# TAdeJong/pyGPA

Measured on AMD Instinct MI355X. Metric: Mpixels/s displacement-field extraction (3 peaks, 4096^2 img) + achieved HBM GB/s, higher is better.
Workload: dtype f32; 1 GPU; 4096x4096 synthetic hex moire, 3 Bragg peaks x 16 k-vectors, sigma=10, weighted DCT-PCG unwrap kmax=10, image resident in HBM, u downloaded to pinned host memory inside the step (BASELINE.json configs[2]); x_planes=12, d2h_of_u=included, overlapped with the next step (copy stream), images_in_flight=1

## Files before the change

### pygpa_amd/csrc/gpa_api.hip

```cpp
#include "gpa_plan.h"

static thread_local std::string g_err;
int gpa_fail(int code, const std::string& msg) {
  g_err = msg;
  return code;
}
namespace gpa {
static const char* const kOptNames[OPT_COUNT] = {
    "PBS_FULLBAND", "SERIAL_UNWRAP", "NO_WORKER", "NO_KSPLIT", "NO_COMPACT", "NO_SHARED",
    "NO_PAIR", "TRI_SMALL", "TRI_Q", "NO_MR", "MR_FORCE_BLUESTEIN", "NO_ROWPQ", "COLSOLVE", "NO_LAT",
    "F32_EPS_FLOOR", "COLSTREAM_CHUNK", "NO_ROWHALF", "PAIR_MAXSIDE", "ROWHALF_MINLG", "NO_PQDCT",
    "NO_REORDER", "NO_RAW", "NO_TILEFUSE", "NO_ROWPERS", "NO_LFTILE", "LF_ALL_ROUNDS", "DFT_ENGINE", "GAUSS_FFT_MINR", "NO_GAUSS2D", "NO_DFT_HALF", "F32_STALL", "PBS_LDS_PAD", "NO_SHARED_PHASES", "PA_STAG", "PA_STAG_TICKS", "PA_ROT", "LF_STACK_BYTES"};
static OptVal g_opts[OPT_COUNT];
static std::once_flag g_opts_once;
static void opt_assign(OptVal& o, const char* value) {
  o.set = value != nullptr;
  o.num = value ? atof(value) : 0.0;
  memset(o.str, 0, sizeof(o.str));
  if (value) strncpy(o.str, value, sizeof(o.str) - 1);
}
static void opts_from_env() {
  for (int k = 0; k < OPT_COUNT; ++k) opt_assign(g_opts[k], getenv((std::string("GPA_") + kOptNames[k]).c_str()));
}
const OptVal& opt(OptKey k) {
  std::call_once(g_opts_once, opts_from_env);
  return g_opts[k];
}
}

Axis make_axis(int n) {
  Axis a;
  a.n = n;
  int lg = 0;
  while ((1 << lg) < n) ++lg;
  if ((1 << lg) == n) {
    a.padded = false;
  } else {
    lg = 0;
    while ((1 << lg) < 2 * n - 1) ++lg;
    a.padded = true;
  }
  if (lg < 6) {
    lg = 6;
    a.padded = ((1 << lg) != n);
  }
  a.lg = lg;
  a.L = 1 << lg;
  a.extL = a.padded ? n - 1 : 0;
  a.extR = 0;
  return a;
}

Axis compact_axis(const Axis& full, int E) {
  if (!full.padded || E >= (full.n - 1) / 2) return full;
  int lg = 6;
  while ((1 << lg) < full.n + 2 * E) ++lg;
  if (lg >= full.lg) return full;
  Axis a = full;
  a.lg = lg;
  a.L = 1 << lg;
  a.extL = a.extR = E;
  return a;
}

int upload_real_table(gpa_plan* p, void* dst, const std::vector<double>& v) {
  if (p->dtype == GPA_F32) HIP_TRY(upload_as<float>(dst, v, p->stream));
  else HIP_TRY(upload_as<double>(dst, v, p->stream));
  return GPA_OK;
}

int dmalloc(gpa_plan* p, void** ptr, size_t bytes) {
  if (bytes == 0) bytes = 16;
  hipError_t e = hipMalloc(ptr, bytes);
  if (e != hipSuccess)
    return fail(GPA_ERR_HIP, std::string("hipMalloc(") + std::to_string(bytes) + "): " + hipGetErrorString(e));
  p->ws_bytes += bytes;
  return GPA_OK;
}
int plan_build(gpa_plan* p) {
  HIP_TRY(hipSetDevice(p->device));
  HIP_TRY(hipStreamCreateWithFlags(&p->stream, hipStreamNonBlocking));
  HIP_TRY(hipEventCreate(&p->ev0));
  HIP_TRY(hipEventCreate(&p->ev1));
  for (auto& e : p->stage_ev) HIP_TRY(hipEventCreate(&e));
  const size_t npx = (size_t)p->n0 * p->n1;
  const int B = p->max_batch;
  for (int ax = 0; ax < 2; ++ax) {
    const Axis& a = ax == 0 ? p->ax0 : p->ax1;
    std::vector<double> t((size_t)2 * a.L);
    for (int k = 0; k < a.L; ++k) {
      t[2 * k] = cos(-2.0 * M_PI * k / a.L);
      t[2 * k + 1] = sin(-2.0 * M_PI * k / a.L);
    }
    void** dst = ax == 0 ? &p->tw0 : &p->tw1;
    TRY(dmalloc(p, dst, (size_t)a.L * p->csz));
    TRY(upload_real_table(p, *dst, t));
  }
  TRY(dmalloc(p, &p->Hx, (size_t)p->ax0.L * p->csz));
  TRY(dmalloc(p, &p->Hy, (size_t)p->ax1.L * p->csz));
  p->tbuf_planes = B < 4 ? B : 4;
  TRY(dmalloc(p, &p->Tbuf, (size_t)p->tbuf_planes * npx * p->csz));
  TRY(dmalloc(p, &p->tb.cxb, (size_t)B * std::max(p->ax0.L / 16, 256) * p->csz));
  TRY(dmalloc(p, &p->tb.sx, (size_t)B * 16 * p->csz));
  TRY(dmalloc(p, &p->tb.wxw, (size_t)B * p->csz));
  TRY(dmalloc(p, &p->tb.wxr, (size_t)B * p->csz));
  TRY(dmalloc(p, &p->tb.cyb, (size_t)B * std::max(p->ax1.L / 16, 256) * p->csz));
  TRY(dmalloc(p, &p->tb.sy, (size_t)B * 16 * p->csz));
  TRY(dmalloc(p, &p->tb.wyw, (size_t)B * p->csz));
  TRY(dmalloc(p, &p->tb.wyr, (size_t)B * p->csz));
  TRY(dmalloc(p, (void**)&p->tb.planeof, (size_t)B * sizeof(int)));
  TRY(dmalloc(p, (void**)&p->d_pw, (size_t)B * sizeof(double)));
  TRY(dmalloc(p, &p->tb.dx, (size_t)B * p->n0 * p->csz));
  TRY(dmalloc(p, &p->tb.dy, (size_t)B * p->n1 * p->csz));
  TRY(dmalloc(p, (void**)&p->d_kl, (size_t)B * 2 * sizeof(double)));
  TRY(dmalloc(p, (void**)&p->d_kr, (size_t)B * 2 * sizeof(double)));
  HIP_TRY(hipHostMalloc((void**)&p->h_k, ((size_t)B * 6 + 32) * sizeof(double)));
  HIP_TRY(hipHostMalloc((void**)&p->h_iters, 8 * sizeof(int)));
  TRY(dmalloc(p, &p->d_image, npx * p->rsz));
  TRY(dmalloc(p, &p->d_mean, 16));
  TRY(dmalloc(p, &p->d_tile_mean, 16));
  TRY(dmalloc(p, (void**)&p->d_scratch, 16384 * sizeof(double)));
  TRY(dmalloc(p, &p->d_aux0, (size_t)p->n0 * 2 * sizeof(double)));
  TRY(dmalloc(p, &p->d_aux1, (size_t)p->n1 * 2 * sizeof(double)));
  p->max_peaks = B < 8 ? B : 8;
  TRY(dmalloc(p, &p->d_lockin, (size_t)p->max_peaks * npx * p->csz));
  TRY(dmalloc(p, (void**)&p->d_kidx, (size_t)p->max_peaks * npx * sizeof(int32_t)));
  TRY(dmalloc(p, &p->d_dudx, 2 * npx * p->rsz));
  TRY(dmalloc(p, &p->d_dudy, 2 * npx * p->rsz));
  TRY(dmalloc(p, &p->d_wnorm, npx * p->rsz));
  TRY(dmalloc(p, &p->d_u, 2 * npx * p->rsz));
  TRY(dmalloc(p, (void**)&p->d_kmat, (size_t)p->max_peaks * 2 * sizeof(double)));
  if (!p->spectral_only) {
    size_t before = 0;
    hipError_t e = unwrap_workspace_create(p->dtype, p->n0, p->n1, p->stream, &p->uw, &before);
    if (e != hipSuccess) return fail(GPA_ERR_HIP, std::string("unwrap workspace: ") + hipGetErrorString(e));
    p->ws_bytes += before;
  }
  return GPA_OK;
}


int upload_twiddles(gpa_plan* p, void* dst, int L) {
  std::vector<double> t((size_t)2 * L);
  for (int k = 0; k < L; ++k) {
    t[2 * k] = cos(-2.0 * M_PI * k / L);
    t[2 * k + 1] = sin(-2.0 * M_PI * k / L);
  }
  return upload_real_table(p, dst, t);
}

extern "C" {

int gpa_version(void) { return 100; }

int gpa_set_option(const char* name, const char* value) {
  if (!name) return fail(GPA_ERR_ARG, "gpa_set_option: null name");
  if (strncmp(name, "GPA_", 4) == 0) name += 4;
  (void)opt(OPT_NO_LAT);
  for (int k = 0; k < OPT_COUNT; ++k)
    if (strcmp(name, kOptNames[k]) == 0) {
      opt_assign(g_opts[k], value);
      return GPA_OK;
    }
  return fail(GPA_ERR_ARG, std::string("gpa_set_option: unknown option ") + name);
}
const char* gpa_last_error(void) { return g_err.c_str(); }

int gpa_device_count(void) {
  int n = 0;
  if (hipGetDeviceCount(&n) != hipSuccess) return 0;
  return n;
}

gpa_plan* gpa_plan_create(int device, int n0, int n1, int max_batch, int dtype) {
  if (n0 < 4 || n1 < 4 || max_batch < 1 || (dtype != GPA_F32 && dtype != GPA_F64)) {
    fail(GPA_ERR_ARG, "gpa_plan_create: need n0,n1 >= 4, max_batch >= 1, dtype in {GPA_F32, GPA_F64}");
    return nullptr;
  }
  int ndev = gpa_device_count();
  if (ndev <= 0 || device < 0 || device >= ndev) {
    fail(GPA_ERR_NODEV, "gpa_plan_create: no such GPU (device " + std::to_string(device) + " of " +
                            std::to_string(ndev) + ")");
    return nullptr;
  }
  gpa_plan* p = new gpa_plan();
  p->device = device;
  p->dtype = dtype;
  p->n0 = n0;
  p->n1 = n1;
  p->max_batch = max_batch;
  p->rsz = dtype == GPA_F32 ? 4 : 8;
  p->csz = 2 * p->rsz;
  p->ax0 = p->ax0_full = make_axis(n0);
  p->ax1 = p->ax1_full = make_axis(n1);
  p->serial_unwrap = opt_set(OPT_SERIAL_UNWRAP);
  p->use_worker = !opt_set(OPT_NO_WORKER);
  p->no_ksplit = opt_set(OPT_NO_KSPLIT);
  p->no_compact = opt_set(OPT_NO_COMPACT);
  p->use_shared = !opt_set(OPT_NO_SHARED);
  const int maxlg = dtype == GPA_F32 ? 14 : 13;
  if (n0 > 65536 || n1 > 65536) {
    fail(GPA_ERR_ARG, "gpa_plan_create: axis longer than 65536");
    delete p;
    return nullptr;
  }
  p->spectral_only = p->ax0.lg > maxlg || p->ax1.lg > maxlg;
  if (plan_build(p) != GPA_OK) {
    std::string keep = g_err;
    gpa_plan_destroy(p);
    g_err = keep;
    return nullptr;
  }
  return p;
}

void gpa_plan_destroy(gpa_plan* p) {
  if (!p) return;
  hipSetDevice(p->device);
  delete p->worker;
  p->worker = nullptr;
  if (p->stream) hipStreamSynchronize(p->stream);
  void* bufs[] = {p->tw0, p->tw1, p->Hx, p->Hy, p->Tbuf, p->tb.cxb, p->tb.sx, p->tb.wxw, p->tb.wxr, p->tb.cyb, p->tb.sy, p->tb.wyw, p->tb.wyr, p->tb.planeof, p->d_pw,
                  p->tb.dx, p->tb.dy, p->d_kl, p->d_kr, p->d_image, p->d_mean, p->d_tile_mean, p->d_scratch,
                  p->d_lockin, p->d_kidx, p->d_dudx, p->d_dudy, p->d_wnorm, p->d_u, p->d_kmat, p->d_sf, p->d_grad, p->d_grads, p->d_absw, p->d_aux0, p->d_aux1,
                  p->sh.Gb, p->sh.psi, p->sh.dyc, p->sh.gtab, p->sh.desc, p->sh.order, p->d_taps, p->tw1s,
                  p->sh.pre, p->sh.rot16, p->d_wys, p->d_shifts, p->d_ystep};
  for (void* b : bufs)
    if (b) hipFree(b);
  unwrap_workspace_destroy(&p->uw);
  unwrap_workspace_destroy(&p->uw2);
  if (p->uwb_images) unwrap_workspace_destroy(&p->uwb);
  if (p->have_uwp) unwrap_workspace_destroy(&p->uwp);
  if (p->d_wnorm_b) (void)hipFree(p->d_wnorm_b);
  if (p->h_iters_b) (void)hipHostFree(p->h_iters_b);
  for (void* b : {p->bT, p->bL, p->bMean, (void*)p->bScratch})
    if (b) (void)hipFree(b);
  if (p->stream2) { hipStreamSynchronize(p->stream2); hipStreamDestroy(p->stream2); }
  if (p->ev_fork) hipEventDestroy(p->ev_fork);
  if (p->ev_join) hipEventDestroy(p->ev_join);
  if (p->ev_x) hipEventDestroy(p->ev_x);
  if (p->d_tsum_part) (void)hipFree(p->d_tsum_part);
  warp_ws_free(&p->warp);
  ucell_ws_free(&p->ucell);
  dft_axis_destroy(&p->bx0);
  dft_axis_destroy(&p->bx1);
  dft_work_free(&p->dftw);
  for (auto& ax : p->gft)
    for (auto& g : ax) {
      if (g.H) (void)hipFree(g.H);
      if (g.tw) (void)hipFree(g.tw);
    }
  if (p->d_pertab) (void)hipFree(p->d_pertab);
  if (p->d_peakws) (void)hipFree(p->d_peakws);
  if (p->d_peaksmooth) (void)hipFree(p->d_peaksmooth);
  if (p->h_k) hipHostFree(p->h_k);
  if (p->h_iters) hipHostFree(p->h_iters);
  if (p->kprof) {
    for (int i = 0; i < p->kprof->npool; ++i) hipEventDestroy(p->kprof->pool[i]);
    delete p->kprof;
  }
  if (p->copy_stream) { hipStreamSynchronize(p->copy_stream); hipStreamDestroy(p->copy_stream); }
  if (p->ev_dl_ready) hipEventDestroy(p->ev_dl_ready);
  for (auto e : p->ev_dl_done)
    if (e) hipEventDestroy(e);
  if (p->ev0) hipEventDestroy(p->ev0);
  if (p->ev1) hipEventDestroy(p->ev1);
  for (auto e : p->stage_ev)
    if (e) hipEventDestroy(e);
  if (p->stream) hipStreamDestroy(p->stream);
  delete p;
}

int gpa_plan_sync(gpa_plan* p) {
  if (!p) return fail(GPA_ERR_ARG, "null plan");
  HIP_TRY(hipStreamSynchronize(p->stream));
  if (p->stream2) HIP_TRY(hipStreamSynchronize(p->stream2));
  if (p->copy_stream) HIP_TRY(hipStreamSynchronize(p->copy_stream));
  return GPA_OK;
}
size_t gpa_plan_workspace_bytes(const gpa_plan* p) { return p ? p->ws_bytes : 0; }
void* gpa_plan_stream(const gpa_plan* p) { return p ? (void*)p->stream : nullptr; }
int gpa_plan_fft_len(const gpa_plan* p, int axis) {
  if (!p) return 0;
  return axis == 0 ? p->ax0.L : p->ax1.L;
}

int gpa_timer_start(gpa_plan* p) {
  if (!p) return fail(GPA_ERR_ARG, "null plan");
  HIP_TRY(hipEventRecord(p->ev0, p->stream));
  return GPA_OK;
}
int gpa_timer_stop(gpa_plan* p, float* ms_out) {
  if (!p || !ms_out) return fail(GPA_ERR_ARG, "null argument");
  HIP_TRY(hipEventRecord(p->ev1, p->stream));
  HIP_TRY(hipEventSynchronize(p->ev1));
  HIP_TRY(hipEventElapsedTime(ms_out, p->ev0, p->ev1));
  return GPA_OK;
}
int gpa_set_profiling(gpa_plan* p, int on) {
  if (!p) return fail(GPA_ERR_ARG, "null plan");
  p->profiling = on != 0;
  return GPA_OK;
}
int gpa_last_kernel_profile(gpa_plan* p, char* out, size_t cap) {
  if (!p || !out || cap == 0) return fail(GPA_ERR_ARG, "null argument");
  if (p->kprof_table.size() + 1 > cap) return fail(GPA_ERR_STATE, "gpa_last_kernel_profile: buffer too small");
  memcpy(out, p->kprof_table.c_str(), p->kprof_table.size() + 1);
  return GPA_OK;
}

int gpa_download_async(gpa_plan* p, void* host_dst, const void* dev_src, size_t bytes, int slot) {
  if (!p || !host_dst || !dev_src) return fail(GPA_ERR_ARG, "gpa_download_async: null argument");
  if (slot < 0 || slot >= 4) return fail(GPA_ERR_ARG, "gpa_download_async: slot must be 0..3");
  HIP_TRY(hipSetDevice(p->device));
  if (!p->copy_stream) {
    HIP_TRY(hipStreamCreateWithFlags(&p->copy_stream, hipStreamNonBlocking));
    HIP_TRY(hipEventCreateWithFlags(&p->ev_dl_ready, hipEventDisableTiming));
    for (auto& e : p->ev_dl_done) HIP_TRY(hipEventCreateWithFlags(&e, hipEventDisableTiming));
  }
  HIP_TRY(hipEventRecord(p->ev_dl_ready, p->stream));
  HIP_TRY(hipStreamWaitEvent(p->copy_stream, p->ev_dl_ready, 0));
  HIP_TRY(hipMemcpyAsync(host_dst, dev_src, bytes, hipMemcpyDeviceToHost, p->copy_stream));
  HIP_TRY(hipEventRecord(p->ev_dl_done[slot], p->copy_stream));
  return GPA_OK;
}

int gpa_download_wait(gpa_plan* p, int slot) {
  if (!p) return fail(GPA_ERR_ARG, "null plan");
  if (slot < 0 || slot >= 4) return fail(GPA_ERR_ARG, "gpa_download_wait: slot must be 0..3");
  if (!p->copy_stream) return GPA_OK;
  HIP_TRY(hipEventSynchronize(p->ev_dl_done[slot]));
  return GPA_OK;
}

int gpa_last_stage_ms(gpa_plan* p, float* ms5) {
  if (!p || !ms5) return fail(GPA_ERR_ARG, "null argument");
  for (int i = 0; i < 5; ++i) ms5[i] = p->stage_ms[i];
  return GPA_OK;
}

}
```

### pygpa_amd/csrc/gpa_api_driver.hip

```cpp
#include "gpa_plan.h"

struct ExtractOut {
  void* lockins;
  int32_t* kidx;
  void* grads;
  void* absw;
  int grad_mode;
};

static int check_ranges(gpa_plan* p, const std::string& fn, int P, int K, int kmax) {
  if (P < 2 || P > p->max_peaks) return fail(GPA_ERR_STATE, fn + ": need 2 <= P <= 8");
  if (K < 1 || P * K > p->max_batch) return fail(GPA_ERR_STATE, fn + ": P*K exceeds max_batch");
  if (kmax < 1) return fail(GPA_ERR_ARG, "kmax must be >= 1");
  return GPA_OK;
}

static int extract_stage(gpa_plan* p, const double* kvecs, int P, const double* klists, int K, double sigma, int* Bx) {
  TRY(stage_sweep(p, kvecs, P, klists, K, sigma, Bx));
  TRY(stage_kmat(p, kvecs, P));
  {
    const size_t side = opt_set(OPT_PAIR_MAXSIDE) ? (size_t)opt(OPT_PAIR_MAXSIDE).num : 1024;
    p->use_pair = (size_t)p->n0 * p->n1 <= side * side && !opt_set(OPT_NO_PAIR);
  }
  if (p->use_pair && !p->have_uwp) {
    size_t bp = 0;
    hipError_t ep = unwrap_workspace_create(p->dtype, p->n0, p->n1, p->stream, &p->uwp, &bp, 2);
    if (ep != hipSuccess) {
      unwrap_workspace_destroy(&p->uwp);
      return fail(GPA_ERR_HIP, std::string("paired unwrap workspace: ") + hipGetErrorString(ep));
    }
    p->ws_bytes += bp;
    p->have_uwp = true;
  }
  if (p->use_pair && !unwrap_supports_batch(&p->uwp)) p->use_pair = false;
  if (!p->stream2) {
    HIP_TRY(hipStreamCreateWithFlags(&p->stream2, hipStreamNonBlocking));
    HIP_TRY(hipEventCreateWithFlags(&p->ev_fork, hipEventDisableTiming));
    HIP_TRY(hipEventCreateWithFlags(&p->ev_join, hipEventDisableTiming));
    size_t b2 = 0;
    hipError_t e2 = unwrap_workspace_create(p->dtype, p->n0, p->n1, p->stream2, &p->uw2, &b2);
    if (e2 != hipSuccess) return fail(GPA_ERR_HIP, std::string("second unwrap workspace: ") + hipGetErrorString(e2));
    p->ws_bytes += b2;
  }
  return GPA_OK;
}

static int extract_launch(gpa_plan* p, const void* image, int P, int K, int Bx, int mask_border, int kmax, void* u,
                          const ExtractOut& o) {
  const size_t npx = (size_t)p->n0 * p->n1;
  void* lk = o.lockins ? o.lockins : p->d_lockin;
  if (p->profiling) HIP_TRY(hipEventRecord(p->stage_ev[0], p->stream));
  HIP_TRY(launch_mean(p->dtype, image, npx, p->d_scratch, p->d_mean, p->stream));
  if (p->profiling) HIP_TRY(hipEventRecord(p->stage_ev[1], p->stream));
  TRY(run_passA(p, image, p->d_mean, p->Tbuf, Bx, 1));
  if (p->profiling) HIP_TRY(hipEventRecord(p->stage_ev[2], p->stream));
  if (o.grads) {
    int32_t* kidx = o.kidx ? o.kidx : p->d_kidx;
    bool shared = false;
    TRY(passB_phases(p, P, K, lk, kidx, p->d_sf, &shared));
    HIP_TRY(launch_phasegrad(p->dtype, p->d_sf, K, kidx, p->n0, p->n1, p->d_kl, p->d_kr, o.grad_mode, o.grads, p->stream,
                             shared ? p->d_ystep : nullptr, P));
  } else {
    TRY(passB_select(p, {p->Tbuf, 1, 0}, P, K, lk, o.kidx, !o.lockins && !o.absw));
  }
  if (o.absw) HIP_TRY(launch_cabs(p->dtype, lk, (size_t)P * npx, o.absw, p->stream));
  const double* ystep = p->lk_raw ? p->d_ystep : nullptr;
  if (p->profiling) HIP_TRY(hipEventRecord(p->stage_ev[3], p->stream));
  int nparts = 0;
  if (p->use_pair && p->have_uwp && !p->profiling && !p->serial_unwrap) {
    HIP_TRY(launch_reconstruct_setup(p->dtype, lk, p->d_kmat, P, p->n0, p->n1, mask_border, p->d_wnorm,
                                     unwrap_residual_buffer(&p->uwp, 0), unwrap_residual_buffer(&p->uwp, 1),
                                     unwrap_partials_buffer(&p->uwp, 0), unwrap_partials_buffer(&p->uwp, 1), &nparts,
                                     p->stream, 1, 0, 0, ystep));
    hipError_t ep = unwrap_enqueue_prepared(&p->uwp, p->d_wnorm, nparts, kmax, 1e-9, true, u, p->stream);
    if (ep == hipSuccess) ep = unwrap_fetch_iters(&p->uwp, p->h_iters, p->stream);
    if (ep != hipSuccess) return unwrap_fail(ep);
    p->iters_stride = 4;
    p->iters_off = unwrap_iters_slot(&p->uwp);
    return GPA_OK;
  }
  p->iters_stride = 1;
  p->iters_off = 0;
  HIP_TRY(launch_reconstruct_setup(p->dtype, lk, p->d_kmat, P, p->n0, p->n1, mask_border, p->d_wnorm,
                                   unwrap_residual_buffer(&p->uw), unwrap_residual_buffer(&p->uw2),
                                   unwrap_partials_buffer(&p->uw), unwrap_partials_buffer(&p->uw2), &nparts, p->stream, 1, 0,
                                   0, ystep));
  if (p->profiling) HIP_TRY(hipEventRecord(p->stage_ev[4], p->stream));
  HIP_TRY(hipEventRecord(p->ev_fork, p->stream));
  HIP_TRY(hipStreamWaitEvent(p->stream2, p->ev_fork, 0));
  hipStreamCaptureStatus cap = hipStreamCaptureStatusNone;
  (void)hipStreamIsCapturing(p->stream, &cap);
  const bool threaded = p->use_worker && !p->profiling && !p->serial_unwrap && cap == hipStreamCaptureStatusNone;
  hipError_t e2 = hipSuccess;
  void* u1 = (char*)u + npx * p->rsz;
  auto second = [&]() {
    e2 = unwrap_enqueue_prepared(&p->uw2, p->d_wnorm, nparts, kmax, 1e-9, true, u1, p->stream2);
    if (e2 == hipSuccess) e2 = unwrap_fetch_iters(&p->uw2, &p->h_iters[1], p->stream2);
  };
  if (threaded) {
    if (!p->worker) p->worker = new EnqueueWorker(p->device);
    p->worker->submit(second);
  }
  hipError_t e = unwrap_enqueue_prepared(&p->uw, p->d_wnorm, nparts, kmax, 1e-9, true, u, p->stream);
  if (p->profiling || p->serial_unwrap) {
    HIP_TRY(hipEventRecord(p->ev_fork, p->stream));
    HIP_TRY(hipStreamWaitEvent(p->stream2, p->ev_fork, 0));
  }
  if (e == hipSuccess) e = unwrap_fetch_iters(&p->uw, &p->h_iters[0], p->stream);
  if (threaded) p->worker->wait(); else second();
  if (e == hipSuccess) e = e2;
  if (e != hipSuccess) return unwrap_fail(e);
  HIP_TRY(hipEventRecord(p->ev_join, p->stream2));
  HIP_TRY(hipStreamWaitEvent(p->stream, p->ev_join, 0));
  if (p->profiling) HIP_TRY(hipEventRecord(p->stage_ev[5], p->stream));
  return GPA_OK;
}

static int extract_enqueue(gpa_plan* p, const char* what, const void* image, const double* kvecs, int P, const double* klists,
                           int K, double sigma, int mask_border, int kmax, void* u, const ExtractOut& o) {
  const std::string fn(what);
  if (!p || !image || !kvecs || !klists || !u) return fail(GPA_ERR_ARG, fn + ": null argument");
  TRY(check_ranges(p, fn, P, K, kmax));
  if (o.grads && (o.grad_mode < 0 || o.grad_mode > 2)) return fail(GPA_ERR_ARG, fn + ": grad_mode must be 0, 1 or 2");
  HIP_TRY(hipSetDevice(p->device));
  int Bx = 0;
  TRY(extract_stage(p, kvecs, P, klists, K, sigma, &Bx));
  if (o.grads) TRY(ensure_sf(p, (size_t)P * K * p->n0 * p->n1 * p->rsz));
  ProfInstall prof(p);
  return extract_launch(p, image, P, K, Bx, mask_border, kmax, u, o);
}

static void read_iters(const gpa_plan* p, int* iters2) {
  iters2[0] = p->h_iters[p->iters_off];
  iters2[1] = p->h_iters[p->iters_stride + p->iters_off];
}

int gpa_last_iters(gpa_plan* p, int* iters2) {
  if (!p || !iters2) return fail(GPA_ERR_ARG, "null argument");
  HIP_TRY(hipStreamSynchronize(p->stream));
  read_iters(p, iters2);
  return GPA_OK;
}

static int extract_finish(gpa_plan* p, int* iters_out) {
  HIP_TRY(hipStreamSynchronize(p->stream));
  if (p->profiling) {
    for (int i = 0; i < 5; ++i) hipEventElapsedTime(&p->stage_ms[i], p->stage_ev[i], p->stage_ev[i + 1]);
    collect_kernel_profile(p);
  }
  if (iters_out) read_iters(p, iters_out);
  return GPA_OK;
}

static int extract_host(gpa_plan* p, const char* what, const void* image, const double* kvecs, int P, const double* klists,
                        int K, double sigma, int mask_border, int kmax, void* u, const ExtractOut& o, int* iters_out) {
  if (!p || !image || !u) return fail(GPA_ERR_ARG, std::string(what) + ": null argument");
  HIP_TRY(hipSetDevice(p->device));
  const size_t npx = (size_t)p->n0 * p->n1;
  if (o.grads && !p->d_grads) TRY(dmalloc(p, &p->d_grads, (size_t)p->max_peaks * 2 * npx * p->rsz));
  if (o.absw && !p->d_absw) TRY(dmalloc(p, &p->d_absw, (size_t)p->max_peaks * npx * p->rsz));
  HIP_TRY(hipMemcpyAsync(p->d_image, image, npx * p->rsz, hipMemcpyHostToDevice, p->stream));
  const ExtractOut dev{o.lockins ? p->d_lockin : nullptr, o.kidx ? p->d_kidx : nullptr, o.grads ? p->d_grads : nullptr,
                       o.absw ? p->d_absw : nullptr, o.grad_mode};
  TRY(extract_enqueue(p, what, p->d_image, kvecs, P, klists, K, sigma, mask_border, kmax, p->d_u, dev));
  TRY(extract_finish(p, iters_out));
  HIP_TRY(hipMemcpyAsync(u, p->d_u, 2 * npx * p->rsz, hipMemcpyDeviceToHost, p->stream));
  if (o.lockins) HIP_TRY(hipMemcpyAsync(o.lockins, p->d_lockin, (size_t)P * npx * p->csz, hipMemcpyDeviceToHost, p->stream));
  if (o.kidx) HIP_TRY(hipMemcpyAsync(o.kidx, p->d_kidx, (size_t)P * npx * sizeof(int32_t), hipMemcpyDeviceToHost, p->stream));
  if (o.grads) HIP_TRY(hipMemcpyAsync(o.grads, p->d_grads, (size_t)P * 2 * npx * p->rsz, hipMemcpyDeviceToHost, p->stream));
  if (o.absw) HIP_TRY(hipMemcpyAsync(o.absw, p->d_absw, (size_t)P * npx * p->rsz, hipMemcpyDeviceToHost, p->stream));
  HIP_TRY(hipStreamSynchronize(p->stream));
  return GPA_OK;
}

int gpa_extract_displacement_field(gpa_plan* p, const void* image, const double* kvecs, int P,
                                   const double* klists, int K, double sigma, int mask_border, int kmax,
                                   void* u, void* lockins, int32_t* kidx, int* iters_out) {
  return extract_host(p, "gpa_extract_displacement_field", image, kvecs, P, klists, K, sigma, mask_border, kmax, u,
                      {lockins, kidx, nullptr, nullptr, 0}, iters_out);
}

int gpa_extract_displacement_field_grad(gpa_plan* p, const void* image, const double* kvecs, int P,
                                        const double* klists, int K, double sigma, int mask_border, int kmax,
                                        int grad_mode, void* u, void* lockins, int32_t* kidx, void* grads, void* absw,
                                        int* iters_out) {
  return extract_host(p, "gpa_extract_displacement_field_grad", image, kvecs, P, klists, K, sigma, mask_border, kmax, u,
                      {lockins, kidx, grads, absw, grad_mode}, iters_out);
}

int gpa_extract_displacement_field_dev(gpa_plan* p, const void* image, const double* kvecs, int P,
                                       const double* klists, int K, double sigma, int mask_border, int kmax,
                                       void* u, void* lockins, int32_t* kidx, int* iters_out) {
  TRY(extract_enqueue(p, "gpa_extract_displacement_field", image, kvecs, P, klists, K, sigma, mask_border, kmax, u,
                      {lockins, kidx, nullptr, nullptr, 0}));
  return extract_finish(p, iters_out);
}

int gpa_extract_displacement_field_grad_dev(gpa_plan* p, const void* image, const double* kvecs, int P,
                                            const double* klists, int K, double sigma, int mask_border, int kmax,
                                            int grad_mode, void* u, void* lockins, int32_t* kidx, void* grads, void* absw,
                                            int* iters_out) {
  TRY(extract_enqueue(p, "gpa_extract_displacement_field_grad_dev", image, kvecs, P, klists, K, sigma, mask_border, kmax, u,
                      {lockins, kidx, grads, absw, grad_mode}));
  return extract_finish(p, iters_out);
}

int gpa_extract_displacement_field_async(gpa_plan* p, const void* image, const double* kvecs, int P,
                                         const double* klists, int K, double sigma, int mask_border, int kmax,
                                         void* u, void* lockins, int32_t* kidx) {
  return extract_enqueue(p, "gpa_extract_displacement_field", image, kvecs, P, klists, K, sigma, mask_border, kmax, u,
                         {lockins, kidx, nullptr, nullptr, 0});
}

int gpa_extract_displacement_field_grad_async(gpa_plan* p, const void* image, const double* kvecs, int P,
                                              const double* klists, int K, double sigma, int mask_border, int kmax,
                                              int grad_mode, void* u, void* lockins, int32_t* kidx, void* grads, void* absw) {
  return extract_enqueue(p, "gpa_extract_displacement_field_grad_async", image, kvecs, P, klists, K, sigma, mask_border, kmax, u,
                         {lockins, kidx, grads, absw, grad_mode});
}

static int ensure_batch_unwrap(gpa_plan* p, int B) {
  if (B <= p->uwb_images) {
    if (!unwrap_set_active(&p->uwb, 2 * B)) return fail(GPA_ERR_STATE, "batched unwrap workspace: bad active count");
    return GPA_OK;
  }
  const size_t npx = (size_t)p->n0 * p->n1;
  HIP_TRY(hipStreamSynchronize(p->stream));
  if (p->uwb_images) {
    unwrap_workspace_destroy(&p->uwb);
    (void)hipFree(p->d_wnorm_b);
    (void)hipHostFree(p->h_iters_b);
    p->uwb_images = 0;
    p->d_wnorm_b = nullptr;
    p->h_iters_b = nullptr;
  }
  size_t bb = 0;
  hipError_t e = unwrap_workspace_create(p->dtype, p->n0, p->n1, p->stream, &p->uwb, &bb, 2 * B);
  if (e != hipSuccess) {
    unwrap_workspace_destroy(&p->uwb);
    return fail(GPA_ERR_HIP, std::string("batched unwrap workspace: ") + hipGetErrorString(e));
  }
  if (!unwrap_supports_batch(&p->uwb)) {
    unwrap_workspace_destroy(&p->uwb);
    return fail(GPA_ERR_STATE, "gpa_extract_displacement_field_batch: this image shape has no batched unwrap");
  }
  e = hipMalloc(&p->d_wnorm_b, (size_t)B * npx * p->rsz);
  if (e == hipSuccess) e = hipHostMalloc((void**)&p->h_iters_b, (size_t)8 * B * sizeof(int));
  if (e != hipSuccess) {
    unwrap_workspace_destroy(&p->uwb);
    if (p->d_wnorm_b) (void)hipFree(p->d_wnorm_b);
    p->d_wnorm_b = nullptr;
    return fail(GPA_ERR_HIP, std::string("batched driver buffers: ") + hipGetErrorString(e));
  }
  p->uwb_images = B;
  return GPA_OK;
}

static int ensure_batch_sweep(gpa_plan* p, int chunk, size_t t_img, size_t l_img) {
  if ((size_t)chunk * t_img <= p->bT_bytes && (size_t)chunk * l_img <= p->bL_bytes && chunk <= p->b_chunk) return GPA_OK;
  HIP_TRY(hipStreamSynchronize(p->stream));
  for (void* b : {p->bT, p->bL, p->bMean, (void*)p->bScratch})
    if (b) (void)hipFree(b);
  p->bT = p->bL = p->bMean = nullptr;
  p->bScratch = nullptr;
  p->bT_bytes = p->bL_bytes = 0;
  p->b_chunk = 0;
  hipError_t ea = hipMalloc(&p->bT, (size_t)chunk * t_img);
  if (ea == hipSuccess) ea = hipMalloc(&p->bL, (size_t)chunk * l_img);
  if (ea == hipSuccess) ea = hipMalloc(&p->bMean, (size_t)chunk * 8);
  if (ea == hipSuccess) ea = hipMalloc((void**)&p->bScratch, (size_t)chunk * 1024 * sizeof(double));
  if (ea != hipSuccess) return fail(GPA_ERR_HIP, std::string("batched sweep buffers: ") + hipGetErrorString(ea));
  p->bT_bytes = (size_t)chunk * t_img;
  p->bL_bytes = (size_t)chunk * l_img;
  p->b_chunk = chunk;
  return GPA_OK;
}

static int read_batch_iters(gpa_plan* p, int B, int* iters_out) {
  HIP_TRY(hipStreamSynchronize(p->stream));
  for (int j = 0; j < 2 * B; ++j) iters_out[j] = p->h_iters_b[4 * j + unwrap_iters_slot(&p->uwb)];
  return GPA_OK;
}

int gpa_extract_displacement_field_batch_dev(gpa_plan* p, const void* images, int B, const double* kvecs, int P,
                                             const double* klists, int K, double sigma, int mask_border, int kmax,
                                             void* u, int* iters_out) {
  const char* fn = "gpa_extract_displacement_field_batch";
  if (!p || !images || !kvecs || !klists || !u) return fail(GPA_ERR_ARG, std::string(fn) + ": null argument");
  if (B < 1 || B > 4096) return fail(GPA_ERR_ARG, std::string(fn) + ": need 1 <= images <= 4096");
  TRY(check_ranges(p, fn, P, K, kmax));
  HIP_TRY(hipSetDevice(p->device));
  int Bx = 0;
  TRY(extract_stage(p, kvecs, P, klists, K, sigma, &Bx));
  TRY(ensure_batch_unwrap(p, B));
  const size_t npx = (size_t)p->n0 * p->n1;
  const size_t t_img = (size_t)Bx * npx * p->csz, l_img = (size_t)P * npx * p->csz;
  const int chunk = (int)std::min<size_t>((size_t)B, std::max<size_t>(1, ((size_t)3 << 30) / t_img));
  TRY(ensure_batch_sweep(p, chunk, t_img, l_img));
  int nparts = 0;
  const size_t rstride = 2 * npx;
  const size_t pstride = (size_t)(unwrap_partials_buffer(&p->uwb, 2) - unwrap_partials_buffer(&p->uwb, 0));
  for (int c0 = 0; c0 < B; c0 += chunk) {
    const int nimg = std::min(chunk, B - c0);
    const void* image = (const char*)images + (size_t)c0 * npx * p->rsz;
    HIP_TRY(launch_mean(p->dtype, image, npx, p->bScratch, p->bMean, p->stream, nimg));
    TRY(run_passA(p, image, p->bMean, p->bT, Bx, nimg));
    TRY(passB_select(p, {p->bT, nimg, Bx}, P, K, p->bL, nullptr, true));
    HIP_TRY(launch_reconstruct_setup(p->dtype, p->bL, p->d_kmat, P, p->n0, p->n1, mask_border,
                                     (char*)p->d_wnorm_b + (size_t)c0 * npx * p->rsz,
                                     unwrap_residual_buffer(&p->uwb, 2 * c0), unwrap_residual_buffer(&p->uwb, 2 * c0 + 1),
                                     unwrap_partials_buffer(&p->uwb, 2 * c0), unwrap_partials_buffer(&p->uwb, 2 * c0 + 1),
                                     &nparts, p->stream, nimg, rstride, pstride, p->lk_raw ? p->d_ystep : nullptr));
  }
  hipError_t e = unwrap_enqueue_prepared(&p->uwb, p->d_wnorm_b, nparts, kmax, 1e-9, true, u, p->stream);
  if (e == hipSuccess) e = unwrap_fetch_iters(&p->uwb, p->h_iters_b, p->stream);
  if (e != hipSuccess) return fail(GPA_ERR_HIP, std::string("batched unwrap: ") + hipGetErrorString(e));
  return iters_out ? read_batch_iters(p, B, iters_out) : GPA_OK;
}

int gpa_supports_batch(gpa_plan* p) {
  if (!p) return 0;
  return unwrap_supports_batch(&p->uw) ? 1 : 0;
}

int gpa_last_batch_iters(gpa_plan* p, int B, int* iters_out) {
  if (!p || !iters_out || B < 1 || B > p->uwb_images) return fail(GPA_ERR_ARG, "gpa_last_batch_iters: bad argument");
  return read_batch_iters(p, B, iters_out);
}

int gpa_extract_gradients(gpa_plan* p, const void* image, const double* kvecs, int P, const double* klists, int K,
                          double sigma, int mask_border, void* dudx, void* dudy, void* wnorm) {
  if (!p || !image || !kvecs || !klists || !dudx || !dudy || !wnorm)
    return fail(GPA_ERR_ARG, "gpa_extract_gradients: null argument");
  TRY(check_ranges(p, "gpa_extract_gradients", P, K, 1));
  HIP_TRY(hipSetDevice(p->device));
  const size_t npx = (size_t)p->n0 * p->n1;
  HIP_TRY(hipMemcpyAsync(p->d_image, image, npx * p->rsz, hipMemcpyHostToDevice, p->stream));
  TRY(sweep_peaks_dev(p, p->d_image, nullptr, kvecs, P, klists, K, sigma, p->d_lockin, nullptr, true));
  TRY(stage_kmat(p, kvecs, P));
  HIP_TRY(launch_reconstruct(p->dtype, p->d_lockin, p->d_kmat, P, p->n0, p->n1, mask_border, p->d_dudx, p->d_dudy,
                             p->d_wnorm, p->stream, p->lk_raw ? p->d_ystep : nullptr));
  HIP_TRY(hipMemcpyAsync(dudx, p->d_dudx, (size_t)2 * p->n0 * (p->n1 - 1) * p->rsz, hipMemcpyDeviceToHost, p->stream));
  HIP_TRY(hipMemcpyAsync(dudy, p->d_dudy, (size_t)2 * (p->n0 - 1) * p->n1 * p->rsz, hipMemcpyDeviceToHost, p->stream));
  HIP_TRY(hipMemcpyAsync(wnorm, p->d_wnorm, npx * p->rsz, hipMemcpyDeviceToHost, p->stream));
  HIP_TRY(hipStreamSynchronize(p->stream));
  return GPA_OK;
}
```

### pygpa_amd/csrc/gpa_api_sweep.hip

```cpp
#include "gpa_plan.h"

int gpa_lockin_batch_dev(gpa_plan* p, const void* image, const double* kvecs, int B, double sigma,
                         void* out) {
  if (!p || !image || !kvecs || !out) return fail(GPA_ERR_ARG, "gpa_lockin_batch: null argument");
  if (B < 1 || B > p->max_batch) return fail(GPA_ERR_STATE, "gpa_lockin_batch: B exceeds the plan's max_batch");
  HIP_TRY(hipSetDevice(p->device));
  TRY(ensure_filters(p, sigma));
  int Bx = 0;
  TRY(stage_kvectors(p, kvecs, kvecs, B, &Bx));
  TRY(ensure_tbuf(p, Bx));
  TRY(run_passA(p, image, nullptr, p->Tbuf, Bx, 1));
  HIP_TRY(launch_passB(p->dtype, p->ax1, p->n0, p->Tbuf, p->Hy, p->tw1, p->tb, B, 1, false, out, nullptr,
                       p->stream));
  return GPA_OK;
}

int gpa_lockin_batch(gpa_plan* p, const void* image, const double* kvecs, int B, double sigma, void* out) {
  if (!p || !image || !kvecs || !out) return fail(GPA_ERR_ARG, "gpa_lockin_batch: null argument");
  if (B < 1 || B > p->max_batch) return fail(GPA_ERR_STATE, "gpa_lockin_batch: B exceeds the plan's max_batch");
  HIP_TRY(hipSetDevice(p->device));
  const size_t npx = (size_t)p->n0 * p->n1;
  HIP_TRY(hipMemcpyAsync(p->d_image, image, npx * p->rsz, hipMemcpyHostToDevice, p->stream));
  TRY(ensure_sf(p, (size_t)B * npx * p->csz));
  TRY(gpa_lockin_batch_dev(p, p->d_image, kvecs, B, sigma, p->d_sf));
  HIP_TRY(hipMemcpyAsync(out, p->d_sf, (size_t)B * npx * p->csz, hipMemcpyDeviceToHost, p->stream));
  HIP_TRY(hipStreamSynchronize(p->stream));
  return GPA_OK;
}

int stage_sweep(gpa_plan* p, const double* krefs, int P, const double* klists, int K, double sigma, int* Bx) {
  const int B = P * K;
  TRY(ensure_filters(p, sigma));
  std::vector<double> kr((size_t)B * 2);
  for (int pp = 0; pp < P; ++pp)
    for (int k = 0; k < K; ++k) {
      kr[2 * ((size_t)pp * K + k)] = krefs[2 * pp];
      kr[2 * ((size_t)pp * K + k) + 1] = krefs[2 * pp + 1];
    }
  TRY(stage_kvectors(p, klists, kr.data(), B, Bx));
  return ensure_tbuf(p, *Bx);
}

int run_passA(gpa_plan* p, const void* image, const void* mean, void* Tbuf, int Bx, int nimg) {
  HIP_TRY(launch_passA(p->dtype, p->ax0, p->n1, image, mean, p->tb, p->Hx, p->tw0, Tbuf, Bx, p->stream, nimg));
  return GPA_OK;
}

int passB_select(gpa_plan* p, const XPlanes& xp, int P, int K, void* lockin, int32_t* kidx, bool raw) {
  p->lk_raw = false;
  const int rows_wg = (p->n0 + 7) / 8 * P;
  int ksplit = 1;
  if (xp.stride == 0 && p->ax1.lg <= 10 && K >= 4 && !p->no_ksplit && rows_wg <= 256)
    while (ksplit < 4 && ksplit * 2 <= K && rows_wg * ksplit < 1024) ksplit *= 2;
  if (ksplit == 1) {
    TRY(shared_prepare(p, P, K));
    if (p->sh_use) {
      p->lk_raw = raw && !opt_set(OPT_NO_RAW) && p->sh_one_kref;
      HIP_TRY(launch_passB_shared(p->dtype, p->ax1s, p->n0, xp.T, p->ax1s.L == p->ax1.L ? p->tw1 : p->tw1s, p->tb,
                                  p->sh, p->sh_E, p->sh_Epad, P, K, lockin, kidx, p->stream, xp.nimg, xp.stride, p->sh_nbl,
                                  p->lk_raw));
    } else
      HIP_TRY(launch_passB(p->dtype, p->ax1, p->n0, xp.T, p->Hy, p->tw1, p->tb, P, K, true, lockin, kidx, p->stream, xp.nimg,
                           xp.stride));
    return GPA_OK;
  }
  const size_t npx = (size_t)p->n0 * p->n1, cnt = (size_t)ksplit * P * npx;
  TRY(ensure_sf(p, cnt * (p->csz + sizeof(int32_t))));
  void* part = p->d_sf;
  int32_t* pidx = reinterpret_cast<int32_t*>((char*)p->d_sf + cnt * p->csz);
  HIP_TRY(launch_passB_split(p->dtype, p->ax1, p->n0, xp.T, p->Hy, p->tw1, p->tb, P, K, ksplit, part, pidx, lockin, kidx,
                             p->stream));
  return GPA_OK;
}

int passB_phases(gpa_plan* p, int P, int K, void* lockin, int32_t* kidx, void* psi, bool* shared) {
  p->lk_raw = false;
  *shared = false;
  if (p->use_shared && !opt_set(OPT_NO_SHARED_PHASES)) {
    TRY(shared_prepare(p, P, K));
    if (p->sh_use && p->sh_one_kref) {
      const hipError_t e = launch_passB_shared_phases(p->dtype, p->ax1s, p->n0, p->Tbuf, p->ax1s.L == p->ax1.L ? p->tw1 : p->tw1s,
                                                      p->tb, p->sh, p->sh_E, p->sh_Epad, P, K, lockin, kidx, psi, p->stream, 0,
                                                      p->sh_nbl);
      if (e == hipSuccess) {
        *shared = true;
        return GPA_OK;
      }
      if (e != hipErrorInvalidValue) return fail(GPA_ERR_HIP, std::string("shared pass B (phases): ") + hipGetErrorString(e));
    }
  }
  HIP_TRY(launch_passB_ext(p->dtype, p->ax1, p->n0, p->Tbuf, p->Hy, p->tw1, p->tb, K, 3, lockin, kidx, nullptr, psi, p->stream, P));
  return GPA_OK;
}

void collect_kernel_profile(gpa_plan* p) {
  std::vector<std::string> names;
  std::vector<int> calls;
  std::vector<double> total;
  for (int i = 0; p->kprof && i < p->kprof->n; ++i) {
    const KernelProfiler::Rec& r = p->kprof->rec[i];
    float ms = 0.f;
    if (hipEventElapsedTime(&ms, r.a, r.b) != hipSuccess) continue;
    size_t j = 0;
    while (j < names.size() && names[j] != r.name) ++j;
    if (j == names.size()) { names.push_back(r.name); calls.push_back(0); total.push_back(0.0); }
    ++calls[j];
    total[j] += ms;
  }
  p->kprof_table.clear();
  char line[160];
  for (size_t j = 0; j < names.size(); ++j) {
    snprintf(line, sizeof(line), "%s %d %.6f\n", names[j].c_str(), calls[j], total[j]);
    p->kprof_table += line;
  }
}

int sweep_peaks_dev(gpa_plan* p, const void* image, const void* mean, const double* krefs, int P,
                           const double* klists, int K, double sigma, void* lockin, int32_t* kidx, bool raw) {
  if (P * K > p->max_batch) return fail(GPA_ERR_STATE, "sweep: P*K exceeds the plan's max_batch");
  int Bx = 0;
  TRY(stage_sweep(p, krefs, P, klists, K, sigma, &Bx));
  if (p->profiling) HIP_TRY(hipEventRecord(p->stage_ev[1], p->stream));
  TRY(run_passA(p, image, mean, p->Tbuf, Bx, 1));
  if (p->profiling) HIP_TRY(hipEventRecord(p->stage_ev[2], p->stream));
  TRY(passB_select(p, {p->Tbuf, 1, 0}, P, K, lockin, kidx, raw));
  if (p->profiling) HIP_TRY(hipEventRecord(p->stage_ev[3], p->stream));
  return GPA_OK;
}

static int sweep_one_peak(gpa_plan* p, const void* image, const double* kref, const double* klist, int K, double sigma,
                          int mode, void* lockin, int32_t* kidx, const uint8_t* d_gate, void* d_psi) {
  if (K > p->max_batch) return fail(GPA_ERR_STATE, "gpa_sweep: K exceeds the plan's max_batch");
  int Bx = 0;
  TRY(stage_sweep(p, kref, 1, klist, K, sigma, &Bx));
  TRY(run_passA(p, image, nullptr, p->Tbuf, Bx, 1));
  HIP_TRY(launch_passB_ext(p->dtype, p->ax1, p->n0, p->Tbuf, p->Hy, p->tw1, p->tb, K, mode, lockin, kidx, d_gate, d_psi,
                           p->stream));
  return GPA_OK;
}

int gpa_sweep_grad_dev(gpa_plan* p, const void* image, const double* kref, const double* klist, int K, double sigma,
                       int grad_mode, void* lockin, int32_t* kidx, void* grad) {
  if (!p || !image || !kref || !klist || !lockin || !grad) return fail(GPA_ERR_ARG, "gpa_sweep_grad: null argument");
  if (K < 1) return fail(GPA_ERR_ARG, "gpa_sweep_grad: K must be >= 1");
  if (grad_mode < 0 || grad_mode > 2) return fail(GPA_ERR_ARG, "gpa_sweep_grad: grad_mode must be 0, 1 or 2");
  if (K > p->max_batch) return fail(GPA_ERR_STATE, "gpa_sweep: K exceeds the plan's max_batch");
  HIP_TRY(hipSetDevice(p->device));
  const bool top = g_kprof == nullptr;
  ProfInstallIf prof(p, top);
  const size_t npx = (size_t)p->n0 * p->n1;
  TRY(ensure_sf(p, (size_t)K * npx * p->rsz));
  int32_t* ki = kidx ? kidx : p->d_kidx;
  int Bx = 0;
  TRY(stage_sweep(p, kref, 1, klist, K, sigma, &Bx));
  TRY(run_passA(p, image, nullptr, p->Tbuf, Bx, 1));
  bool shared = false;
  TRY(passB_phases(p, 1, K, lockin, ki, p->d_sf, &shared));
  HIP_TRY(launch_phasegrad(p->dtype, p->d_sf, K, ki, p->n0, p->n1, p->d_kl, p->d_kr, grad_mode, grad, p->stream,
                           shared ? p->d_ystep : nullptr));
  if (top && p->profiling) { HIP_TRY(hipStreamSynchronize(p->stream)); collect_kernel_profile(p); }
  return GPA_OK;
}

int gpa_sweep_dev(gpa_plan* p, const void* image, const double* kref, const double* klist, int K,
                  double sigma, void* lockin, int32_t* kidx, void* grad) {
  if (!p || !image || !kref || !klist || !lockin) return fail(GPA_ERR_ARG, "gpa_sweep: null argument");
  if (K < 1) return fail(GPA_ERR_ARG, "gpa_sweep: K must be >= 1");
  HIP_TRY(hipSetDevice(p->device));
  if (!grad) return sweep_peaks_dev(p, image, nullptr, kref, 1, klist, K, sigma, lockin, kidx, false);
  return gpa_sweep_grad_dev(p, image, kref, klist, K, sigma, 0, lockin, kidx, grad);
}

static int sweep_host(gpa_plan* p, const void* image, const double* kref, const double* klist, int K, double sigma,
                      int grad_mode, const uint8_t* gate, void* lockin, int32_t* kidx, void* grad) {
  if (!p || !image || !kref || !klist || !lockin) return fail(GPA_ERR_ARG, "gpa_sweep: null argument");
  if (K < 1) return fail(GPA_ERR_ARG, "gpa_sweep: K must be >= 1");
  HIP_TRY(hipSetDevice(p->device));
  ProfInstall prof(p);
  const size_t npx = (size_t)p->n0 * p->n1;
  HIP_TRY(hipMemcpyAsync(p->d_image, image, npx * p->rsz, hipMemcpyHostToDevice, p->stream));
  if (grad && !p->d_grad) TRY(dmalloc(p, &p->d_grad, 2 * npx * p->rsz));
  if (gate) {
    TRY(ensure_sf(p, (size_t)K * K));
    HIP_TRY(hipMemcpyAsync(p->d_sf, gate, (size_t)K * K, hipMemcpyHostToDevice, p->stream));
    TRY(sweep_one_peak(p, p->d_image, kref, klist, K, sigma, 2, p->d_lockin, p->d_kidx, (const uint8_t*)p->d_sf, nullptr));
  } else if (grad) {
    TRY(gpa_sweep_grad_dev(p, p->d_image, kref, klist, K, sigma, grad_mode, p->d_lockin, p->d_kidx, p->d_grad));
  } else {
    TRY(sweep_peaks_dev(p, p->d_image, nullptr, kref, 1, klist, K, sigma, p->d_lockin, p->d_kidx, false));
  }
  if (grad) HIP_TRY(hipMemcpyAsync(grad, p->d_grad, 2 * npx * p->rsz, hipMemcpyDeviceToHost, p->stream));
  HIP_TRY(hipMemcpyAsync(lockin, p->d_lockin, npx * p->csz, hipMemcpyDeviceToHost, p->stream));
  if (kidx) HIP_TRY(hipMemcpyAsync(kidx, p->d_kidx, npx * sizeof(int32_t), hipMemcpyDeviceToHost, p->stream));
  HIP_TRY(hipStreamSynchronize(p->stream));
  if (p->profiling) collect_kernel_profile(p);
  return GPA_OK;
}

int gpa_sweep(gpa_plan* p, const void* image, const double* kref, const double* klist, int K, double sigma,
              void* lockin, int32_t* kidx, void* grad) {
  return sweep_host(p, image, kref, klist, K, sigma, 0, nullptr, lockin, kidx, grad);
}

int gpa_sweep_grad(gpa_plan* p, const void* image, const double* kref, const double* klist, int K, double sigma,
                   int grad_mode, void* lockin, int32_t* kidx, void* grad) {
  if (!grad) return fail(GPA_ERR_ARG, "gpa_sweep_grad: null argument");
  if (grad_mode < 0 || grad_mode > 2) return fail(GPA_ERR_ARG, "gpa_sweep_grad: grad_mode must be 0, 1 or 2");
  return sweep_host(p, image, kref, klist, K, sigma, grad_mode, nullptr, lockin, kidx, grad);
}

int gpa_sweep_gated(gpa_plan* p, const void* image, const double* kref, const double* klist, int K, double sigma,
                    const uint8_t* gate, void* lockin, int32_t* kidx) {
  if (!gate) return fail(GPA_ERR_ARG, "gpa_sweep_gated: null argument");
  return sweep_host(p, image, kref, klist, K, sigma, 0, gate, lockin, kidx, nullptr);
}
```

### pygpa_amd/csrc/gpa_api_tables.hip

```cpp
#include "gpa_plan.h"

void host_fft_pow2(std::vector<std::complex<double>>& a, bool inverse) {
  const size_t n = a.size();
  int lg = 0;
  while ((size_t(1) << lg) < n) ++lg;
  for (size_t i = 0; i < n; ++i) {
    size_t r = 0;
    for (int b = 0; b < lg; ++b) r |= ((i >> b) & 1) << (lg - 1 - b);
    if (r > i) std::swap(a[i], a[r]);
  }
  for (size_t len = 2; len <= n; len <<= 1) {
    const double ang = (inverse ? 2 : -2) * M_PI / (double)len;
    for (size_t s = 0; s < n; s += len)
      for (size_t j = 0; j < len / 2; ++j) {
        std::complex<double> w(cos(ang * (double)j), sin(ang * (double)j));
        auto u = a[s + j], v = a[s + j + len / 2] * w;
        a[s + j] = u + v;
        a[s + j + len / 2] = u - v;
      }
  }
}

std::vector<double> gaussian_kspace(int n, double sigma) {
  std::vector<double> g(n);
  for (int k = 0; k < n; ++k) {
    const int kk = k < (n + 1) / 2 ? k : k - n;
    const double f = (double)kk / (double)n;
    const double e = 2.0 * M_PI * M_PI * sigma * sigma * f * f;
    g[k] = e > 50.0 ? 0.0 : exp(-e);
  }
  return g;
}

std::vector<double> spatial_kernel(int n, const std::vector<double>& g) {
  std::vector<double> h((size_t)n);
  std::vector<long double> cs((size_t)n);
  const long double w = 2.0L * 3.14159265358979323846264338327950288L / (long double)n;
  for (int j = 0; j < n; ++j) cs[j] = cosl(w * (long double)j);
  for (int m = 0; m < n; ++m) {
    long double acc = 0;
    for (int k = 0; k < n; ++k)
      if (g[k] != 0.0) acc += (long double)g[k] * cs[(size_t)((long long)k * m % n)];
    h[m] = (double)(acc / (long double)n);
  }
  return h;
}

int kernel_support(const std::vector<double>& h, double tol) {
  const int n = (int)h.size();
  double total = 0;
  for (double v : h) total += fabs(v);
  double tail = 0;
  for (int m = n / 2; m >= 1; --m) {
    tail += fabs(h[m]) + (n - m != m ? fabs(h[n - m]) : 0.0);
    if (tail > tol * total) return m;
  }
  return 0;
}

std::vector<double> spatial_taps(int n, const std::vector<double>& g, int mmax) {
  std::vector<double> h((size_t)mmax + 1);
  std::vector<long double> cs((size_t)n);
  const long double w = 2.0L * 3.14159265358979323846264338327950288L / (long double)n;
  for (int j = 0; j < n; ++j) cs[j] = cosl(w * (long double)j);
  for (int m = 0; m <= mmax; ++m) {
    long double acc = 0;
    for (int k = 0; k < n; ++k)
      if (g[k] != 0.0) acc += (long double)g[k] * cs[(size_t)((long long)k * m % n)];
    h[m] = (double)(acc / (long double)n);
  }
  return h;
}

void build_filter_table(const Axis& ax, const std::vector<double>& g, const std::vector<double>& hsp,
                               std::vector<double>& out) {
  const int L = ax.L, tpf = L / 16;
  if (!ax.padded) {
    out.assign((size_t)L, 0.0);
    for (int i = 0; i < 16; ++i)
      for (int t = 0; t < tpf; ++t) out[(size_t)i * tpf + t] = g[spec_index_rt(ax.lg, t, i)] / (double)L;
    return;
  }
  const int n = ax.n;
  std::vector<std::complex<double>> h((size_t)L, 0.0);
  if (ax.extR == 0) {
    for (int m = 0; m < n; ++m) h[m] = hsp[m];
  } else {
    for (int m = 0; m <= ax.extL; ++m) h[m] = hsp[m];
    for (int m = 1; m <= ax.extR; ++m) h[(size_t)L - m] = hsp[n - m];
  }
  host_fft_pow2(h, false);
  out.assign((size_t)2 * L, 0.0);
  for (int i = 0; i < 16; ++i)
    for (int t = 0; t < tpf; ++t) {
      auto v = h[spec_index_rt(ax.lg, t, i)] / (double)L;
      out[2 * ((size_t)i * tpf + t)] = v.real();
      out[2 * ((size_t)i * tpf + t) + 1] = v.imag();
    }
}

int ensure_filters(gpa_plan* p, double sigma) {
  if (!(sigma > 0)) return fail(GPA_ERR_ARG, "sigma must be positive");
  NEED_UNWRAP(p, "lock-in sweep");
  if (sigma == p->sigma_cached) return GPA_OK;
  HIP_TRY(hipStreamSynchronize(p->stream));
  p->sigma_cached = -1.0;
  for (int axis = 0; axis < 2; ++axis) {
    const Axis& full = axis == 0 ? p->ax0_full : p->ax1_full;
    Axis& cur = axis == 0 ? p->ax0 : p->ax1;
    std::vector<double> g = gaussian_kspace(full.n, sigma), hsp, table;
    Axis want = full;
    if (full.padded) {
      hsp = spatial_kernel(full.n, g);
      if (!p->no_compact) want = compact_axis(full, kernel_support(hsp, p->dtype == 0 ? 1e-9 : 1e-14));
    }
    if (want.lg != cur.lg || want.extR != cur.extR || want.extL != cur.extL) {
      TRY(upload_twiddles(p, axis == 0 ? p->tw0 : p->tw1, want.L));
      p->staged_kl.clear();
      p->staged_kr.clear();
      cur = want;
    }
    build_filter_table(cur, g, hsp, table);
    TRY(upload_real_table(p, axis == 0 ? p->Hx : p->Hy, table));
    if (axis == 1) {
      p->sh_ok = false;
      ++p->sh_epoch;
      const int n = cur.n;
      int mmax = (int)ceil(10.0 * sigma) + 16;
      if (p->use_shared && mmax < n / 2 && mmax <= 1024) {
        std::vector<double> taps = spatial_taps(n, g, mmax);
        double total = fabs(taps[0]), tail = 0;
        for (int m = 1; m <= mmax; ++m) total += 2 * fabs(taps[m]);
        int E = 1;
        const double tol = p->dtype == 0 ? 1e-9 : 1e-14;
        for (int m = mmax; m >= 1; --m) {
          tail += 2 * fabs(taps[m]);
          if (tail > tol * total) { E = m; break; }
        }
        Axis sa = cur;
        if (cur.padded) {
          sa.lg = 6;
          while ((1 << sa.lg) < n + E) ++sa.lg;
          sa.L = 1 << sa.lg;
          sa.extL = sa.extR = 0;
        }
        if (passB_shared_supports(p->dtype, sa, E)) {
          const int Epad = (E + 15) & ~15;
          if (sa.L != cur.L && p->tw1s_L != sa.L) {
            if (!p->tw1s) TRY(dmalloc(p, &p->tw1s, (size_t)8192 * p->csz));
            TRY(upload_twiddles(p, p->tw1s, sa.L));
            p->tw1s_L = sa.L;
          }
          p->ax1s = sa;
          if (!p->d_taps) TRY(dmalloc(p, (void**)&p->d_taps, 1025 * sizeof(double)));
          if (!p->sh.gtab) TRY(dmalloc(p, &p->sh.gtab, (2 * 256 + 16) * p->rsz));
          HIP_TRY(hipMemcpyAsync(p->d_taps, taps.data(), ((size_t)mmax + 1) * sizeof(double), hipMemcpyHostToDevice, p->stream));
          HIP_TRY(hipStreamSynchronize(p->stream));
          std::vector<double> gt((size_t)2 * Epad + 16, 0.0);
          for (int m = 1; m <= E; ++m) gt[m] = taps[m];
          TRY(upload_real_table(p, p->sh.gtab, gt));
          p->sh_etab = mmax;
          p->sh_E = E;
          p->sh_Epad = Epad;
          p->sh_sigma = sigma;
          p->sh_ok = true;
        }
      }
    }
  }
  p->sigma_cached = sigma;
  return GPA_OK;
}

int shared_prepare(gpa_plan* p, int P, int K) {
  p->sh_use = false;
  const int B = P * K;
  if (!p->sh_ok || !p->use_shared || K < 2 || (int)p->staged_planeof.size() < B) return GPA_OK;
  const bool reorder = !opt_set(OPT_NO_REORDER);
  if (p->sh_built_epoch == p->sh_epoch && p->sh_built_K == K && p->sh_built_B == B && p->sh_built_reorder == reorder) {
    p->sh_use = p->sh_built_ok;
    return GPA_OK;
  }
  p->sh_built_reorder = reorder;
  p->sh_built_epoch = -1;
  p->sh_built_ok = false;
  std::vector<int> order((size_t)B);
  for (int pp = 0; pp < P; ++pp) {
    bool aliased = false;
    for (int a = 0; a < K && !aliased; ++a)
      for (int b2 = a + 1; b2 < K && !aliased; ++b2) {
        const double *ka = &p->staged_kl[2 * ((size_t)pp * K + a)], *kb = &p->staged_kl[2 * ((size_t)pp * K + b2)];
        const bool same = ka[0] == kb[0] && ka[1] == kb[1];
        aliased = !same && ka[0] - floor(ka[0]) == kb[0] - floor(kb[0]) && ka[1] - floor(ka[1]) == kb[1] - floor(kb[1]);
      }
    std::vector<double> d2((size_t)K), pmin;
    std::vector<int> pfirst;
    int nplanes = 0;
    for (int k = 0; k < K; ++k) nplanes = std::max(nplanes, p->staged_planeof[pp * K + k] + 1);
    pmin.assign((size_t)nplanes, 1e300);
    pfirst.assign((size_t)nplanes, K);
    for (int k = 0; k < K; ++k) {
      const size_t b = (size_t)pp * K + k;
      const double ex = p->staged_kl[2 * b] - p->staged_kr[2 * b], ey = p->staged_kl[2 * b + 1] - p->staged_kr[2 * b + 1];
      d2[k] = ex * ex + ey * ey;
      const int pl = p->staged_planeof[b];
      pmin[pl] = std::min(pmin[pl], d2[k]);
      pfirst[pl] = std::min(pfirst[pl], k);
    }
    std::vector<int> idx((size_t)K);
    for (int k = 0; k < K; ++k) idx[k] = k;
    if (reorder && !aliased)
      std::stable_sort(idx.begin(), idx.end(), [&](int a, int b2) {
        const int pa = p->staged_planeof[pp * K + a], pb = p->staged_planeof[pp * K + b2];
        if (pa != pb) return pmin[pa] != pmin[pb] ? pmin[pa] < pmin[pb] : pfirst[pa] < pfirst[pb];
        return d2[a] < d2[b2];
      });
    for (int k = 0; k < K; ++k) order[(size_t)pp * K + k] = pp * K + idx[k];
  }
  const int NC = p->dtype == 0 ? 4 : 2;
  std::vector<int> desc((size_t)B, 0);
  int runs = 0;
  for (int pp = 0; pp < P; ++pp) {
    int k = 0, chunk = 0;
    while (k < K) {
      int e = k + 1;
      while (e < K && p->staged_planeof[order[pp * K + e]] == p->staged_planeof[order[pp * K + k]]) ++e;
      ++runs;
      for (int j = k; j < e; ++j) {
        const int r = j - k, slot = r % NC;
        int d = slot << 2;
        if (r == 0) d |= 1;
        if (slot == 0) { d |= 2 | (std::min(NC, e - j) << 4); ++chunk; }
        d |= (chunk & 1) << 7;
        desc[(size_t)pp * K + j] = d;
      }
      k = e;
    }
  }
  if (2 * runs > B) {
    p->sh_built_epoch = p->sh_epoch;
    p->sh_built_K = K;
    p->sh_built_B = B;
    return GPA_OK;
  }
  HIP_TRY(hipStreamSynchronize(p->stream));
  const int EEs = 16;
  const double fc = sqrt(log(p->dtype == 0 ? 1e9 : 1e17) / (2.0 * M_PI * M_PI * p->sh_sigma * p->sh_sigma));
  std::vector<int> shifts((size_t)P, 0);
  std::vector<double> wys((size_t)B);
  int need = 1;
  for (int pp = 0; pp < P; ++pp) {
    double wmin = p->staged_kl[2 * ((size_t)pp * K) + 1], wmax = wmin;
    for (int k = 1; k < K; ++k) {
      const double w = p->staged_kl[2 * ((size_t)pp * K + k) + 1];
      wmin = std::min(wmin, w);
      wmax = std::max(wmax, w);
    }
    const double lo = -wmax - fc, width = (wmax - wmin) + 2 * fc;
    const double flo = (lo - floor(lo)) * EEs;
    const int sft = (int)floor(flo) % EEs;
    const int blocks = width >= 1.0 ? EEs : (int)ceil((flo - floor(flo)) + width * EEs + 1e-9);
    shifts[pp] = blocks >= EEs ? 0 : sft;
    need = std::max(need, std::min(blocks, EEs));
    for (int k = 0; k < K; ++k)
      wys[(size_t)pp * K + k] = p->staged_kl[2 * (size_t)order[(size_t)pp * K + k] + 1] + (double)shifts[pp] / EEs;
  }
  p->sh_nbl = opt_set(OPT_PBS_FULLBAND) ? EEs : passB_shared_nbl(p->dtype, need);
  if (p->sh_nbl >= EEs) {
    for (int pp = 0; pp < P; ++pp) shifts[pp] = 0;
    for (int bq = 0; bq < B; ++bq) wys[bq] = p->staged_kl[2 * (size_t)order[bq] + 1];
    p->sh_nbl = EEs;
  }
  const size_t gb = (size_t)B * p->ax1s.L * p->rsz, ps = (size_t)B * p->sh_Epad * p->csz;
  if (gb > p->sh_gb_bytes) {
    if (p->sh.Gb) { (void)hipFree(p->sh.Gb); p->ws_bytes -= p->sh_gb_bytes; p->sh.Gb = nullptr; p->sh_gb_bytes = 0; }
    TRY(dmalloc(p, &p->sh.Gb, gb));
    p->sh_gb_bytes = gb;
  }
  if (ps > p->sh_psi_bytes) {
    if (p->sh.psi) { (void)hipFree(p->sh.psi); (void)hipFree(p->sh.pre); p->ws_bytes -= 2 * p->sh_psi_bytes; p->sh.psi = p->sh.pre = nullptr; p->sh_psi_bytes = 0; }
    TRY(dmalloc(p, &p->sh.psi, ps));
    TRY(dmalloc(p, &p->sh.pre, ps));
    p->sh_psi_bytes = ps;
  }
  if (!p->sh.rot16) TRY(dmalloc(p, &p->sh.rot16, (size_t)p->max_peaks * 16 * p->csz));
  if (!p->d_wys) TRY(dmalloc(p, (void**)&p->d_wys, (size_t)p->max_batch * sizeof(double)));
  if (!p->d_shifts) TRY(dmalloc(p, (void**)&p->d_shifts, (size_t)p->max_peaks * sizeof(int)));
  HIP_TRY(hipMemcpyAsync(p->d_wys, wys.data(), (size_t)B * sizeof(double), hipMemcpyHostToDevice, p->stream));
  HIP_TRY(hipMemcpyAsync(p->d_shifts, shifts.data(), (size_t)P * sizeof(int), hipMemcpyHostToDevice, p->stream));
  {
    std::vector<double> ys((size_t)P);
    p->sh_one_kref = true;
    for (int pp = 0; pp < P; ++pp) {
      const double c = p->staged_kr[2 * ((size_t)pp * K) + 1] + (double)shifts[pp] / EEs;
      ys[pp] = 2.0 * M_PI * (c - rint(c));
      for (int k = 1; k < K; ++k)
        if (p->staged_kr[2 * ((size_t)pp * K + k) + 1] != p->staged_kr[2 * ((size_t)pp * K) + 1]) p->sh_one_kref = false;
    }
    if (!p->d_ystep) TRY(dmalloc(p, (void**)&p->d_ystep, (size_t)p->max_peaks * sizeof(double)));
    HIP_TRY(hipMemcpyAsync(p->d_ystep, ys.data(), (size_t)P * sizeof(double), hipMemcpyHostToDevice, p->stream));
    HIP_TRY(hipStreamSynchronize(p->stream));
  }
  if (!p->sh.dyc) TRY(dmalloc(p, &p->sh.dyc, (size_t)p->max_peaks * p->n1 * p->csz));
  if (!p->sh.desc) TRY(dmalloc(p, (void**)&p->sh.desc, (size_t)p->max_batch * sizeof(int)));
  HIP_TRY(hipMemcpyAsync(p->sh.desc, desc.data(), (size_t)B * sizeof(int), hipMemcpyHostToDevice, p->stream));
  if (!p->sh.order) TRY(dmalloc(p, (void**)&p->sh.order, (size_t)p->max_batch * sizeof(int)));
  HIP_TRY(hipMemcpyAsync(p->sh.order, order.data(), (size_t)B * sizeof(int), hipMemcpyHostToDevice, p->stream));
  HIP_TRY(launch_shared_tables(p->dtype, p->ax1s, p->d_wys, p->d_kr, p->d_shifts, p->d_taps, p->sh_etab, p->sh_E, p->sh_Epad, B, K,
                               p->sh_nbl, p->sh, p->stream));
  HIP_TRY(hipStreamSynchronize(p->stream));
  p->sh_built_epoch = p->sh_epoch;
  p->sh_built_K = K;
  p->sh_built_B = B;
  p->sh_built_ok = true;
  p->sh_use = true;
  return GPA_OK;
}

int stage_kvectors(gpa_plan* p, const double* kl, const double* kr_per_b, int B, int* planes_out) {
  if ((int)p->staged_kl.size() == 2 * B && memcmp(p->staged_kl.data(), kl, (size_t)B * 2 * sizeof(double)) == 0 &&
      memcmp(p->staged_kr.data(), kr_per_b, (size_t)B * 2 * sizeof(double)) == 0) {
    *planes_out = p->last_planes;
    return GPA_OK;
  }
  HIP_TRY(hipStreamSynchronize(p->stream));
  p->staged_kl.assign(kl, kl + 2 * (size_t)B);
  p->staged_kr.assign(kr_per_b, kr_per_b + 2 * (size_t)B);
  double* h_kl = p->h_k;
  double* h_kr = p->h_k + 2 * (size_t)B;
  double* h_pw = p->h_k + 4 * (size_t)B;
  int* h_po = reinterpret_cast<int*>(p->h_k + 5 * (size_t)B);
  memcpy(h_kl, kl, (size_t)B * 2 * sizeof(double));
  memcpy(h_kr, kr_per_b, (size_t)B * 2 * sizeof(double));
  int Bx = 0;
  for (int b = 0; b < B; ++b) {
    int found = -1;
    for (int q = 0; q < Bx; ++q)
      if (memcmp(&h_pw[q], &kl[2 * b], sizeof(double)) == 0) { found = q; break; }
    if (found < 0) { h_pw[Bx] = kl[2 * b]; found = Bx++; }
    h_po[b] = found;
  }
  p->staged_planeof.assign(h_po, h_po + B);
  ++p->sh_epoch;
  HIP_TRY(hipMemcpyAsync(p->d_kl, h_kl, (size_t)B * 2 * sizeof(double), hipMemcpyHostToDevice, p->stream));
  HIP_TRY(hipMemcpyAsync(p->d_kr, h_kr, (size_t)B * 2 * sizeof(double), hipMemcpyHostToDevice, p->stream));
  HIP_TRY(hipMemcpyAsync(p->d_pw, h_pw, (size_t)Bx * sizeof(double), hipMemcpyHostToDevice, p->stream));
  HIP_TRY(hipMemcpyAsync(p->tb.planeof, h_po, (size_t)B * sizeof(int), hipMemcpyHostToDevice, p->stream));
  HIP_TRY(launch_tables(p->dtype, p->ax0, p->ax1, p->d_kl, p->d_kr, B, p->d_pw, Bx, p->tb, p->stream));
  HIP_TRY(hipStreamSynchronize(p->stream));
  p->last_planes = Bx;
  *planes_out = Bx;
  return GPA_OK;
}

int ensure_tbuf(gpa_plan* p, int planes) {
  if (planes <= p->tbuf_planes) return GPA_OK;
  const size_t npx = (size_t)p->n0 * p->n1;
  HIP_TRY(hipStreamSynchronize(p->stream));
  HIP_TRY(hipFree(p->Tbuf));
  p->ws_bytes -= (size_t)p->tbuf_planes * npx * p->csz;
  p->Tbuf = nullptr;
  p->tbuf_planes = 0;
  TRY(dmalloc(p, &p->Tbuf, (size_t)planes * npx * p->csz));
  p->tbuf_planes = planes;
  return GPA_OK;
}

int ensure_sf(gpa_plan* p, size_t bytes) {
  if (p->sf_bytes >= bytes) return GPA_OK;
  if (p->d_sf) {
    HIP_TRY(hipStreamSynchronize(p->stream));
    HIP_TRY(hipFree(p->d_sf));
    p->ws_bytes -= p->sf_bytes;
    p->d_sf = nullptr;
    p->sf_bytes = 0;
  }
  TRY(dmalloc(p, &p->d_sf, bytes));
  p->sf_bytes = bytes;
  return GPA_OK;
}

int stage_kmat(gpa_plan* p, const double* kvecs, int P) {
  std::vector<double> km((size_t)2 * P);
  for (int i = 0; i < 2 * P; ++i) km[i] = 2.0 * M_PI * kvecs[i];
  if (km == p->staged_kmat) return GPA_OK;
  HIP_TRY(hipStreamSynchronize(p->stream));
  p->staged_kmat = km;
  double* h = p->h_k + 6 * (size_t)p->max_batch;
  memcpy(h, km.data(), km.size() * sizeof(double));
  HIP_TRY(hipMemcpyAsync(p->d_kmat, h, km.size() * sizeof(double), hipMemcpyHostToDevice, p->stream));
  return GPA_OK;
}
```

### pygpa_amd/csrc/gpa_internal.h

```cpp
#pragma once
#include <hip/hip_runtime.h>
#include <stdint.h>

#include "gpa_fft.h"
#include "gpa_mrfft.h"

#ifndef GPA_F64_WAVES
#define GPA_F64_WAVES 2
#endif

namespace gpa {

struct KernelProfiler {
  struct Rec { const char* name; hipEvent_t a, b; };
  static constexpr int MAXREC = 4096;
  Rec rec[MAXREC];
  int n = 0;
  hipEvent_t pool[2 * MAXREC];
  int npool = 0;
};
extern thread_local KernelProfiler* g_kprof;
struct ProfScope {
  hipStream_t s;
  KernelProfiler::Rec* r = nullptr;
  ProfScope(const char* name, hipStream_t stream) : s(stream) {
    KernelProfiler* k = g_kprof;
    if (!k || k->n >= KernelProfiler::MAXREC) return;
    for (int j = 0; j < 2; ++j)
      if (k->npool < 2 * (k->n + 1)) { if (hipEventCreate(&k->pool[k->npool]) != hipSuccess) return; ++k->npool; }
    r = &k->rec[k->n];
    r->name = name;
    r->a = k->pool[2 * k->n];
    r->b = k->pool[2 * k->n + 1];
    ++k->n;
    (void)hipEventRecord(r->a, s);
  }
  ~ProfScope() { if (r) (void)hipEventRecord(r->b, s); }
};
#if defined(__HIPCC__)
__device__ __forceinline__ int xcd_tile(int b, int grid) {
  const int base = grid >> 3, rem = grid & 7, x = b & 7, idx = b >> 3;
  return x * base + (x < rem ? x : rem) + idx;
}
#endif

inline hipError_t set_dynamic_lds_once(const void* kern, int bytes, unsigned& done) {
  int dev = 0;
  (void)hipGetDevice(&dev);
  const unsigned bit = 1u << (dev & 31);
  if (done & bit) return hipSuccess;
  hipError_t e = hipFuncSetAttribute(kern, hipFuncAttributeMaxDynamicSharedMemorySize, bytes);
  if (e == hipSuccess) done |= bit;
  return e;
}

inline int device_cus() {
  static int n[32] = {};
  int dev = 0;
  (void)hipGetDevice(&dev);
  int& slot = n[dev & 31];
  if (!slot) {
    int cus = 0;
    if (hipDeviceGetAttribute(&cus, hipDeviceAttributeMultiprocessorCount, dev) != hipSuccess || cus <= 0) cus = 256;
    slot = cus;
  }
  return slot;
}

enum OptKey {
  OPT_PBS_FULLBAND, OPT_SERIAL_UNWRAP, OPT_NO_WORKER, OPT_NO_KSPLIT, OPT_NO_COMPACT, OPT_NO_SHARED,
  OPT_NO_PAIR, OPT_TRI_SMALL, OPT_TRI_Q, OPT_NO_MR, OPT_MR_FORCE_BLUESTEIN, OPT_NO_ROWPQ,
  OPT_COLSOLVE, OPT_NO_LAT, OPT_F32_EPS_FLOOR, OPT_COLSTREAM_CHUNK, OPT_NO_ROWHALF, OPT_PAIR_MAXSIDE, OPT_ROWHALF_MINLG, OPT_NO_PQDCT,
  OPT_NO_REORDER, OPT_NO_RAW, OPT_NO_TILEFUSE, OPT_NO_ROWPERS, OPT_NO_LFTILE, OPT_LF_ALL_ROUNDS, OPT_DFT_ENGINE, OPT_GAUSS_FFT_MINR, OPT_NO_GAUSS2D, OPT_NO_DFT_HALF, OPT_F32_STALL, OPT_PBS_LDS_PAD, OPT_NO_SHARED_PHASES, OPT_PA_STAG, OPT_PA_STAG_TICKS, OPT_PA_ROT, OPT_LF_STACK_BYTES, OPT_COUNT
};
struct OptVal {
  bool set;
  double num;
  char str[24];
};
const OptVal& opt(OptKey k);
inline bool opt_set(OptKey k) { return opt(k).set; }

#define GPA_PROF_CAT2(a, b) a##b
#define GPA_PROF_CAT(a, b) GPA_PROF_CAT2(a, b)
#define GPA_PROF(name, stream) ::gpa::ProfScope GPA_PROF_CAT(_gpa_prof_, __LINE__)(name, stream)

struct Axis {
  int n;
  int lg;
  int L;
  bool padded;
  int extL, extR;
};
inline int axis_tpf(const Axis& a) { return a.L / 16; }

GPA_HD int axis_src(int m, int n, int L, bool padded, int extL, int extR) {
  if (!padded) return m;
  if (m < n) return m;
  if (m < n + extR) return m - n;
  if (m >= L - extL) return m - L + n;
  return -1;
}

struct SweepTables {
  void* cxb;
  void* sx;
  void* wxw;
  void* wxr;
  void* cyb;
  void* sy;
  void* wyw;
  void* wyr;
  void* dx;
  void* dy;
  int* planeof;
};

hipError_t launch_tables(int dtype, const Axis& a0, const Axis& a1, const double* kl,
                         const double* kr, int B, const double* pw, int Bx, const SweepTables& tb,
                         hipStream_t s);
hipError_t launch_mean(int dtype, const void* image, size_t count, double* scratch,
                       void* mean_out, hipStream_t s, int nimg = 1);
hipError_t launch_passA(int dtype, const Axis& a0, int n1, const void* image, const void* mean,
                        const SweepTables& tb, const void* Hx, const void* tw0, void* Tbuf,
                        int Bx, hipStream_t s, int nimg = 1);
hipError_t launch_passB(int dtype, const Axis& a1, int n0, const void* Tbuf, const void* Hy,
                        const void* tw1, const SweepTables& tb, int P, int K, bool select,
                        void* out, int32_t* kidx, hipStream_t s, int nimg = 1, int Bx = 0);
hipError_t launch_passB_ext(int dtype, const Axis& a1, int n0, const void* Tbuf, const void* Hy, const void* tw1,
                            const SweepTables& tb, int K, int mode, void* out, int32_t* kidx, const uint8_t* gate,
                            void* psi, hipStream_t s, int P = 1);
hipError_t launch_passB_split(int dtype, const Axis& a1, int n0, const void* Tbuf, const void* Hy, const void* tw1,
                              const SweepTables& tb, int P, int K, int ksplit, void* part, int32_t* pidx, void* out,
                              int32_t* kidx, hipStream_t s);
hipError_t launch_phasegrad(int dtype, const void* psi, int K, const int32_t* kidx, int n0, int n1, const double* kl,
                            const double* kr, int mode, void* grad, hipStream_t s, const double* ystep = nullptr, int P = 1);
int passA_cols(int dtype, int lg);
int spec_index_rt(int lg, int tid, int reg, int elems = 16);

hipError_t launch_reconstruct(int dtype, const void* lockin, const double* kmat ,
                              int P, int n0, int n1, int border, void* dudx, void* dudy,
                              void* wnorm, hipStream_t s, const double* ystep = nullptr );

hipError_t launch_reconstruct_tile(int dtype, const void* lockin, const double* kmat, int P, int n0, int n1, int border,
                                   int i0, int j0, int t0, int t1, void* const dx[2], size_t dx_pitch, void* const dy[2],
                                   size_t dy_pitch, void* const wn[2], size_t wn_pitch, hipStream_t s,
                                   const double* ystep = nullptr);
hipError_t launch_reconstruct_setup(int dtype, const void* lockin, const double* kmat, int P, int n0, int n1,
                                    int border, void* wnorm, void* r0, void* r1, double* part0, double* part1,
                                    int* nparts, hipStream_t s, int nimg = 1, size_t rstride = 0, size_t pstride = 0,
                                    const double* ystep = nullptr );

hipError_t launch_prediff(int dtype, const void* grads, const void* w, const double* kmat, int P, int n0, int n1,
                          void* dudx, void* dudy, void* wnorm, hipStream_t s);

hipError_t launch_wlstsq(int dtype, const void* b, const void* w, const double* kmat, int P, size_t npx,
                         void* out, hipStream_t s);

hipError_t launch_jacobian(int dtype, const void* grads, const void* w, const double* kmat, int P, size_t npx,
                           double nmperpixel, const double* dks , void* J, hipStream_t s);
hipError_t launch_cabs(int dtype, const void* z, size_t count, void* out, hipStream_t s);
hipError_t launch_props(int dtype, const void* jac, size_t npx, int add_identity, double refangle, double refscale,
                        int diff, void* out, hipStream_t s);

int huber_sums_offset();
hipError_t launch_huber_moments(int dtype, const void* img, int n0, int n1, const double* coef, double cx, double cy,
                                double sx, double sy, double* scratch, hipStream_t s);

constexpr int PEAK_PARTS = 1024;
bool gauss2d_small_ok(int R);
hipError_t launch_gauss2d_small(int dtype, const void* in, void* out, int n0, int n1, const double* w, int R,
                                const void* minuend, hipStream_t s);
hipError_t launch_gauss1d(int dtype, const void* in, void* out, int n0, int n1, int axis, const double* w, int R,
                          const void* minuend, hipStream_t s);
hipError_t launch_localmax(int dtype, const void* smooth, int n0, int n1, double rel, double* part, double* thr,
                           int max_out, int* count, int32_t* coords, void* vals, hipStream_t s);

hipError_t launch_deconv_pack(int dtype, const void* data, int m0, int m1, int pad, void* Z, hipStream_t s);
hipError_t launch_deconv_filter(int dtype, void* Z, int n0, int n1, const double* gx, const double* gy, double balance,
                                hipStream_t s);
hipError_t launch_deconv_unpack(int dtype, const void* Z, int m0, int m1, int pad, void* out, hipStream_t s);

hipError_t launch_tile_sums(int dtype, const void* wins, size_t win_stride, size_t pitch, const int* rects_dev, int ntiles,
                            int max_rows, double* part, double* out, hipStream_t s);
int tile_sums_bands(int max_rows);
hipError_t launch_set_mean(int dtype, const double* sum, double scale, void* mean_out, hipStream_t s);
hipError_t launch_copy_fields(int dtype, const void* const* src, void* const* dst, const size_t* src_pitch,
                              const size_t* dst_pitch, const int* rows, const int* cols, int nf, hipStream_t s);
hipError_t launch_stitch(int dtype, const void* tiles, size_t slot_stride, size_t field_stride, size_t tile_pitch,
                         const int* table_dev, int ntiles, int t0, int t1, int nf, void* const* dst, const size_t* dst_pitch,
                         const int* dst_rows, const int* dst_cols, hipStream_t s);

struct WarpWs {
  void* buf = nullptr;
  size_t cap = 0;
  void* taps = nullptr;
  int taps_dtype = -1;
  size_t* counted = nullptr;
};
void warp_ws_free(WarpWs* ws);
hipError_t warp_reserve_undistort(int dtype, int n0, int n1, WarpWs* ws, hipStream_t s);
hipError_t warp_invert_u(int dtype, const void* d_u, int n0, int n1, double scale, int iters, int edge, int shift,
                         void* d_out, hipStream_t s, int mode, int nan_last, WarpWs* ws, const int* rects = nullptr, int nrect = 0);
hipError_t warp_image(int dtype, const void* d_img, const void* d_uinv, int n0, int n1, void* d_out, hipStream_t s, WarpWs* ws,
                      const int* rects = nullptr, int nrect = 0);
int warp_stack_chunk(int dtype, int n0, int n1, int B, int per_frame);
hipError_t warp_undistort_stack(int dtype, const void* d_frames, int B, const void* d_u, int per_frame, double scale, void* d_uinv,
                                int n0, int n1, void* d_out, hipStream_t s, WarpWs* ws);
hipError_t spline_coef_constant_f64(const double* d_in, int n0, int n1, double* d_tmp, double* d_out, hipStream_t s, WarpWs* ws);

struct UcellGeom {
  double ks[4], kinv[4], rmin[2], z;
  int rs0, rs1;
};
struct UcellWs {
  void* buf = nullptr;
  size_t cap = 0;
  WarpWs spline{};
  void* stage = nullptr;
  size_t stage_cap = 0;
  size_t* counted = nullptr;
};
void ucell_ws_free(UcellWs* ws);
hipError_t ucell_stage(UcellWs* ws, size_t bytes, hipStream_t s, void** out);
constexpr int UCELL_MAX_FRAMES = 65535;
constexpr long long UCELL_MAX_BINS = 1LL << 24;
hipError_t ucell_average(int dtype, const void* d_images, int B, const void* d_u, int n0, int n1, const UcellGeom& g,
                         double* d_res, double* d_weights, hipStream_t s, UcellWs* ws);
hipError_t ucell_expand(int dtype, const double* d_cell, const UcellGeom& g, double z2, const void* d_u, int n0, int n1,
                        void* d_out, hipStream_t s, UcellWs* ws);

}
```

### pygpa_amd/csrc/gpa_passb_shared.h

```cpp
#pragma once
#include "gpa_internal.h"

namespace gpa {

template <class T> struct PassBSharedNC { static constexpr int value = sizeof(T) == 4 ? 4 : 2; };

struct PassBSharedTables {
  void* Gb;
  void* psi;
  void* dyc;
  void* gtab;
  void* pre;
  void* rot16;
  int* order;
  int* desc;
};

bool passB_shared_supports(int dtype, const Axis& a1, int E);

hipError_t launch_shared_tables(int dtype, const Axis& a1, const double* wys, const double* kr, const int* shifts,
                                const double* taps, int Etab, int E, int Epad, int B, int K, int nbl, const PassBSharedTables& st,
                                hipStream_t s);
int passB_shared_nbl(int dtype, int need);

hipError_t launch_passB_shared(int dtype, const Axis& a1, int n0, const void* Tbuf, const void* tw1, const SweepTables& tb,
                               const PassBSharedTables& st, int E, int Epad, int P, int K, void* out, int32_t* kidx,
                               hipStream_t s, int nimg = 1, int Bx = 0, int nbl = 16, bool raw = false);
hipError_t launch_passB_shared_phases(int dtype, const Axis& a1, int n0, const void* Tbuf, const void* tw1, const SweepTables& tb,
                                      const PassBSharedTables& st, int E, int Epad, int P, int K, void* out, int32_t* kidx,
                                      void* psi_out, hipStream_t s, int Bx, int nbl);


}
```

### pygpa_amd/csrc/gpa_passb_shared.hip

```cpp
#include <stdlib.h>

#include "gpa_internal.h"
#include "gpa_passb_shared.h"

namespace gpa {

template <class T> struct MfmaVec;
template <> struct MfmaVec<float> { typedef float type __attribute__((ext_vector_type(4))); };
template <> struct MfmaVec<double> { typedef double type __attribute__((ext_vector_type(4))); };

__device__ __forceinline__ MfmaVec<float>::type mfma16(float a, float b, MfmaVec<float>::type c) {
  return __builtin_amdgcn_mfma_f32_16x16x4f32(a, b, c, 0, 0, 0);
}
__device__ __forceinline__ MfmaVec<double>::type mfma16(double a, double b, MfmaVec<double>::type c) {
  return __builtin_amdgcn_mfma_f64_16x16x4f64(a, b, c, 0, 0, 0);
}
template <class T> __device__ __forceinline__ int mfma_row(int kq, int r) {
  if constexpr (sizeof(T) == 8) return kq + 4 * r;
  else return 4 * kq + r;
}

template <class T> struct upair { T u, v; };

template <class T, int TPF, int EE>
__device__ __forceinline__ void load_gb(T (&h)[EE], const T* gbrow, int tid) {
  using gscalar = const __attribute__((address_space(1))) T;
  gscalar* gb = (gscalar*)gbrow;
#pragma unroll
  for (int i = 0; i < EE; ++i) h[i] = gb[i * TPF + tid];
}
template <class T> __device__ __forceinline__ cpx<T> load_cpx(__amdgpu_buffer_rsrc_t r, int voff, int soff, int aux = 16);
__device__ __forceinline__ cpx<float> load_once(const cpx<float>* p) {
  typedef float v2f_t __attribute__((ext_vector_type(2)));
  const v2f_t d = __builtin_nontemporal_load(reinterpret_cast<const v2f_t*>(p));
  return {d.x, d.y};
}
__device__ __forceinline__ cpx<double> load_once(const cpx<double>* p) {
  typedef double v2d_t __attribute__((ext_vector_type(2)));
  const v2d_t d = __builtin_nontemporal_load(reinterpret_cast<const v2d_t*>(p));
  return {d.x, d.y};
}

typedef int v2i_t __attribute__((ext_vector_type(2)));
typedef int v4i_t __attribute__((ext_vector_type(4)));
__device__ __forceinline__ void store_cpx(cpx<double> v, __amdgpu_buffer_rsrc_t r, int voff, int soff);
__device__ __forceinline__ void store_cpx(cpx<float> v, __amdgpu_buffer_rsrc_t r, int voff, int soff) {
  v2i_t d = {__float_as_int(v.x), __float_as_int(v.y)};
  __builtin_amdgcn_raw_buffer_store_b64(d, r, voff, soff, 0);
}
template <> __device__ __forceinline__ cpx<float> load_cpx<float>(__amdgpu_buffer_rsrc_t r, int voff, int soff, int aux) {
  v2i_t d = aux == 16 ? __builtin_amdgcn_raw_buffer_load_b64(r, voff, soff, 16) : aux == 2 ? __builtin_amdgcn_raw_buffer_load_b64(r, voff, soff, 2) : __builtin_amdgcn_raw_buffer_load_b64(r, voff, soff, 0);
  return {__int_as_float(d.x), __int_as_float(d.y)};
}
template <> __device__ __forceinline__ cpx<double> load_cpx<double>(__amdgpu_buffer_rsrc_t r, int voff, int soff, int aux) {
  v4i_t d = aux == 16 ? __builtin_amdgcn_raw_buffer_load_b128(r, voff, soff, 16) : aux == 2 ? __builtin_amdgcn_raw_buffer_load_b128(r, voff, soff, 2) : __builtin_amdgcn_raw_buffer_load_b128(r, voff, soff, 0);
  const long long a = ((long long)(unsigned)d.x) | ((long long)d.y << 32), b = ((long long)(unsigned)d.z) | ((long long)d.w << 32);
  return {__longlong_as_double(a), __longlong_as_double(b)};
}
__device__ __forceinline__ void store_pair(cpx<float> a, cpx<float> b, __amdgpu_buffer_rsrc_t r, int voff, int soff) {
  v4i_t d = {__float_as_int(a.x), __float_as_int(a.y), __float_as_int(b.x), __float_as_int(b.y)};
  __builtin_amdgcn_raw_buffer_store_b128(d, r, voff, soff, 0);
}
__device__ __forceinline__ void store_pair(cpx<double> a, cpx<double> b, __amdgpu_buffer_rsrc_t r, int voff, int soff) {
  store_cpx(a, r, voff, soff);
  store_cpx(b, r, voff + 16, soff);
}
__device__ __forceinline__ void store_cpx(cpx<double> v, __amdgpu_buffer_rsrc_t r, int voff, int soff) {
  const long long a = __double_as_longlong(v.x), b = __double_as_longlong(v.y);
  v4i_t d = {(int)a, (int)(a >> 32), (int)b, (int)(b >> 32)};
  __builtin_amdgcn_raw_buffer_store_b128(d, r, voff, soff, 0);
}

#ifndef GPA_PBS_MINTHREADS
#define GPA_PBS_MINTHREADS 128
#endif
template <class T, int LG, int EE = 16>
struct PassBSGeom {
  using F = WgFFT<T, LG, EE>;
  static_assert(F::P == 3 || F::P == 4, "three- or four-pass transforms");
  static constexpr int TPF = F::TPF;
  static_assert(TPF >= 64, "a row needs whole wavefronts");
  static constexpr int NF = TPF >= GPA_PBS_MINTHREADS ? 1 : GPA_PBS_MINTHREADS / TPF;
  static constexpr int THREADS = NF * TPF;
  static constexpr int NW = TPF / 64;
  static constexpr int NC = PassBSharedNC<T>::value;
  static constexpr int LOGNC = NC == 4 ? 2 : 1;
  static constexpr bool STAGE = sizeof(T) == 4;
  static constexpr bool TWL = F::P == 3;
  static constexpr int T1 = TWL ? F::P1_SETS * 6 : 0;
  static constexpr int SV = sizeof(T) == 4 ? 4 : 2;
  __host__ __device__ static size_t row_elems(int Epad) {
    const size_t ES = (size_t)Epad + 4;
    return (size_t)F::LDS_ELEMS + SV * ES + 2 * NC * ES + (STAGE ? 3 * NC * ES : 0);
  }
  __host__ __device__ static size_t lds_bytes(int Epad) {
    return (NF * row_elems(Epad) + T1) * sizeof(cpx<T>) + (2 * (size_t)Epad + 16) * sizeof(T);
  }
};

#ifndef GPA_PBS_F32_WAVES
#define GPA_PBS_F32_WAVES 3
#endif
#ifndef GPA_PBS_PAD_WAVES
#define GPA_PBS_PAD_WAVES 3
#endif
#ifndef GPA_PBS_F64_WAVES
#define GPA_PBS_F64_WAVES 2
#endif
#ifndef GPA_PBS_L13_WAVES
#define GPA_PBS_L13_WAVES 3
#endif
template <class T, int LG, bool PADDED, int EE, int NBL, bool PSI = false>
__global__ __launch_bounds__((PassBSGeom<T, LG, EE>::THREADS),
                             (sizeof(T) == 8 ? GPA_PBS_F64_WAVES : (LG >= 13 ? GPA_PBS_L13_WAVES : (PADDED ? GPA_PBS_PAD_WAVES : GPA_PBS_F32_WAVES)))) void passB_shared_kernel(
    const cpx<T>* __restrict__ Tin, int n0, int n1, const T* __restrict__ Gb, const cpx<T>* __restrict__ twtab,
    const int* __restrict__ planeof, const int* __restrict__ order, const int* __restrict__ desc, const cpx<T>* __restrict__ pre_g,
    const cpx<T>* __restrict__ psi, const T* __restrict__ gtab, const cpx<T>* __restrict__ dx,
    const cpx<T>* __restrict__ dyc, const cpx<T>* __restrict__ rot16, int K, int E, int Epad, cpx<T>* out,
    int32_t* kidx, int P, int Bx, int raw, T* __restrict__ psi_out) {
  using F = WgFFT<T, LG, EE>;
  using G = PassBSGeom<T, LG, EE>;
  using V4 = typename MfmaVec<T>::type;
  constexpr int TPF = F::TPF, L = F::L, NC = G::NC;
  constexpr bool STAGE = G::STAGE;
  extern __shared__ __attribute__((aligned(16))) char smem[];
  const int tid = threadIdx.x % TPF, f = __builtin_amdgcn_readfirstlane(threadIdx.x / TPF);
  cpx<T>* lds = reinterpret_cast<cpx<T>*>(smem) + (size_t)f * G::row_elems(Epad);
  upair<T>* strip = reinterpret_cast<upair<T>*>(lds + F::LDS_ELEMS);
  const int ES = Epad + 4;
  cpx<T>* fixb = lds + F::LDS_ELEMS + G::SV * ES;
  cpx<T>* pre_l = fixb + 2 * NC * ES;
  cpx<T>* psi_l = pre_l + NC * ES;
  cpx<T>* t1 = reinterpret_cast<cpx<T>*>(smem) + (size_t)G::NF * G::row_elems(Epad);
  T* glds = reinterpret_cast<T*>(t1 + G::T1);
  const int row = blockIdx.x * G::NF + f;
  const bool valid = row < n0;
  const int rr = valid ? row : 0;
  const int p = blockIdx.y, pt = p % P, img = p / P;
  const int lane = threadIdx.x & 63, wrow = tid >> 6;

  for (int i = threadIdx.x; i < 2 * Epad + 16; i += G::THREADS) glds[i] = gtab[i];
  constexpr bool TWLK = G::TWL && !(sizeof(T) == 4 && !PADDED);
  typename std::conditional<TWLK, typename F::TwiddlesP1Lds, typename F::Twiddles>::type tw;
  if constexpr (TWLK) {
    F::fill_pass1_table(t1, twtab, threadIdx.x, G::THREADS);
    __syncthreads();
    F::load_twiddles(tw, twtab, tid, t1);
  } else {
    F::load_twiddles(tw, twtab, tid);
  }

  T ab[EE];
#pragma unroll
  for (int i = 0; i < EE; ++i) ab[i] = T(0);
  const size_t obase = ((size_t)p * n0 + rr) * n1;
  const __amdgpu_buffer_rsrc_t orow = __builtin_amdgcn_make_buffer_rsrc((void*)(out + obase), 0, n1 * (int)sizeof(cpx<T>), 0x00020000);
  const __amdgpu_buffer_rsrc_t krow = __builtin_amdgcn_make_buffer_rsrc((void*)(kidx ? kidx + obase : nullptr), 0, kidx ? n1 * 4 : 0, 0x00020000);
  constexpr int OOB = (int)0x80000000;
  const int iA = PADDED ? (n1 - E) / TPF : EE - 1, iB = PADDED ? (n1 - 1) / TPF : EE - 1;

  cpx<T> X[NBL];
  T h[NBL];
  const cpx<T> rot = rot16[pt * EE + (tid & (EE - 1))];
  const cpx<T> rot_tail = rot16[pt * EE + ((n1 - 1 - (tid < E ? tid : 0)) & (EE - 1))];
  constexpr bool PREFETCH = NBL < EE && sizeof(T) == 4;
  for (int k = 0; k < K; ++k) {
    const int b = pt * K + k;
    const int ob = order[b];
    const int d = desc[b];
    if (d & 1) {
      const cpx<T>* src = Tin + (((size_t)img * Bx + planeof[ob]) * n0 + rr) * n1;
      const cpx<T> cs0 = dx[(size_t)ob * n0 + rr];
      const cpx<T> cs = cmul(cs0, rot);
      cpx<T> tail = {T(0), T(0)};
      if (tid < E) tail = src[n1 - 1 - tid];
      cpx<T> XX[EE];
      if constexpr (PADDED) {
        const __amdgpu_buffer_rsrc_t srow = __builtin_amdgcn_make_buffer_rsrc((void*)src, 0, n1 * (int)sizeof(cpx<T>), 0x00020000);
#pragma unroll
        for (int i = 0; i < EE; ++i)
          XX[i] = cmul(load_cpx<T>(srow, (tid + TPF * i) * (int)sizeof(cpx<T>), 0, 2), cs);
      } else {
#pragma unroll
        for (int i = 0; i < EE; ++i) XX[i] = cmul(load_once(src + tid + TPF * i), cs);
      }
      if (tid < Epad) {
        const bool in = tid < E;
        const cpx<T> s0 = in ? XX[0] : cpx<T>{T(0), T(0)};
        const cpx<T> s1 = in ? cmul(tail, cmul(cs0, rot_tail)) : cpx<T>{T(0), T(0)};
        if constexpr (G::SV == 4) {
          strip[0 * ES + tid] = {s0.x, -s0.y};
          strip[1 * ES + tid] = {s0.y, s0.x};
          strip[2 * ES + tid] = {s1.x, s1.y};
          strip[3 * ES + tid] = {s1.y, -s1.x};
        } else {
          strip[0 * ES + tid] = {s0.x, s0.y};
          strip[1 * ES + tid] = {s1.x, s1.y};
        }
      }
      F::forward(XX, lds, tid, tw);
#pragma unroll
      for (int i = 0; i < NBL; ++i) X[i] = XX[i];
    }
    const int par = (d >> 7) & 1;
    cpx<T> y[EE];
    {
      if (!PREFETCH || k == 0) load_gb<T, TPF, NBL>(h, Gb + (size_t)b * (NBL * TPF), tid);
      if constexpr (STAGE) {
        if (d & 2) {
          const int nc = (d >> 4) & 7;
          for (int e = tid; e < NC * Epad; e += TPF) {
            const int c = e / Epad, j = e - c * Epad, cc = c < nc ? c : nc - 1;
            pre_l[c * ES + j] = pre_g[(size_t)(b + cc) * Epad + j];
            psi_l[(par * NC + c) * ES + j] = psi[(size_t)(b + cc) * Epad + j];
          }
        }
      }
#pragma unroll
      for (int i = 0; i < EE; ++i) {
        if (i < NBL) y[i] = {X[i < NBL ? i : 0].x * h[i < NBL ? i : 0], X[i < NBL ? i : 0].y * h[i < NBL ? i : 0]};
        else y[i] = {T(0), T(0)};
      }
    }
    cpx<T> psL = {T(0), T(0)}, psR = {T(0), T(0)};
    const int a0R = PADDED ? 0 : TPF - 1 - tid;
    if constexpr (!STAGE) {
      psL = psi[(size_t)b * Epad + (tid < E ? tid : 0)];
      psR = psi[(size_t)b * Epad + (a0R < E ? a0R : 0)];
    }
    F::template inv_phase<0>(y, lds, tid, tw);
    __syncthreads();
    if (d & 2) {
      const int nc = (d >> 4) & 7;
      const int n = lane & 15, kq = lane >> 4;
      const int c = (n >> 1) & (NC - 1), end = (n >> (1 + G::LOGNC)) & 1, reim = n & 1;
      const cpx<T>* pre = STAGE ? pre_l + c * ES : pre_g + (size_t)(b + (c < nc ? c : nc - 1)) * Epad;
      const upair<T>* sp = strip + (G::SV == 4 ? end * 2 + reim : end) * ES;
      const bool swp = reim != 0;
      const T sgn = (end == 0) == swp ? T(1) : T(-1);
      const int Mt = (E + 15) >> 4;
      for (int mt = wrow; mt < Mt; mt += G::NW) {
        V4 acc0 = {T(0), T(0), T(0), T(0)}, acc1 = {T(0), T(0), T(0), T(0)};
        int ns = ((E - 16 * mt - 1) >> 2) + 1;
        if (ns > (Epad >> 2)) ns = Epad >> 2;
        const T* ga = glds + 16 * mt + (lane & 15) + kq + 1;
        for (int s = 0; s < ns; s += 4) {
          upair<T> q[4];
          cpx<T> pp[4];
          T av[4];
#pragma unroll
          for (int u = 0; u < 4; ++u) {
            int j = 4 * (s + u) + kq;
            j = j < Epad ? j : Epad - 1;
            q[u] = sp[j];
            if constexpr (G::SV == 2) q[u] = {swp ? q[u].v : q[u].u, sgn * (swp ? q[u].u : q[u].v)};
            pp[u] = pre[j];
            av[u] = ga[4 * (s + u)];
          }
#pragma unroll
          for (int u = 0; u < 4; ++u) {
            const T bv = q[u].u * pp[u].x + q[u].v * pp[u].y;
            if (u & 1) acc1 = mfma16(av[u], bv, acc1);
            else acc0 = mfma16(av[u], bv, acc0);
          }
        }
        if (n < 4 * NC) {
#pragma unroll
          for (int r = 0; r < 4; ++r) {
            const int a0 = 16 * mt + mfma_row<T>(kq, r);
            reinterpret_cast<T*>(fixb + (c * 2 + end) * ES + a0)[reim] = acc0[r] + acc1[r];
          }
        }
      }
    }
    F::template inv_phase<1>(y, lds, tid, tw);
    __syncthreads();
    F::template inv_phase<2>(y, lds, tid, tw);
    if constexpr (F::P == 4) {
      __syncthreads();
      F::template inv_phase<3>(y, lds, tid, tw);
    }
    {
      const int c = (d >> 2) & 3;
      const cpx<T>* pl = psi_l + (par * NC + c) * ES;
      if (tid < E) {
        const cpx<T> fx = fixb[(c * 2 + 1) * ES + tid];
        if constexpr (STAGE) psL = pl[tid];
        const cpx<T> t = cmulc(fx, psL);
        y[0].x += t.x;
        y[0].y += t.y;
      }
      if constexpr (!PADDED) {
        if (a0R < E) {
          const cpx<T> fx = fixb[(c * 2 + 0) * ES + a0R];
          if constexpr (STAGE) psR = pl[a0R];
          const cpx<T> t = cmul(fx, psR);
          y[EE - 1].x += t.x;
          y[EE - 1].y += t.y;
        }
      } else {
        cpx<T> fA = {T(0), T(0)}, fB = {T(0), T(0)};
        {
          const int aA = n1 - 1 - (tid + TPF * iA), aB = aA - TPF;
          const bool inA = aA >= 0 && aA < E, inB = aB >= 0 && aB < E && iB != iA;
          const int qa = inA ? aA : 0, qb = inB ? aB : 0;
          const cpx<T> xa = fixb[(c * 2 + 0) * ES + qa], xb = fixb[(c * 2 + 0) * ES + qb];
          const cpx<T> pa = STAGE ? pl[qa] : psi[(size_t)b * Epad + qa], pb = STAGE ? pl[qb] : psi[(size_t)b * Epad + qb];
          const cpx<T> ta = cmul(xa, pa), tb2 = cmul(xb, pb);
          fA = {inA ? ta.x : T(0), inA ? ta.y : T(0)};
          fB = {inB ? tb2.x : T(0), inB ? tb2.y : T(0)};
        }
#pragma unroll
        for (int i = 0; i < EE; ++i) {
          if (i == iA) { y[i].x += fA.x; y[i].y += fA.y; }
          if (i == iB && iB != iA) { y[i].x += fB.x; y[i].y += fB.y; }
        }
      }
    }
    if constexpr (PREFETCH) {
      if (k + 1 < K) load_gb<T, TPF, NBL>(h, Gb + (size_t)(b + 1) * (NBL * TPF), tid);
    }
    const int kout = ob - pt * K;
    if constexpr (PSI) {
      if (valid) {
        T* prow = psi_out + ((size_t)(p * K + kout) * n0 + rr) * n1;
#pragma unroll
        for (int i = 0; i < EE; ++i) {
          const int yy = tid + TPF * i;
          if (!PADDED || yy < n1) prow[yy] = -atan2(y[i].y, y[i].x);
        }
      }
    }
#pragma unroll
    for (int i = 0; i < EE; ++i) {
      const int yy = tid + TPF * i;
      const T a = y[i].x * y[i].x + y[i].y * y[i].y;
      const bool win = a > ab[i];
      ab[i] = win ? a : ab[i];
      if (__builtin_amdgcn_ballot_w64(win) == 0) continue;
      const int woff = (win && valid) ? (PADDED ? yy : tid) * (int)sizeof(cpx<T>) : OOB;
      constexpr int SOFF = PADDED ? 0 : 1;
      store_cpx(y[i], orow, woff, SOFF * i * TPF * (int)sizeof(cpx<T>));
      constexpr int SH = sizeof(cpx<T>) == 8 ? 1 : 2;
      if (kidx) __builtin_amdgcn_raw_buffer_store_b32(kout, krow, woff >> SH, SOFF * i * TPF * 4, 0);
    }
  }
  if (!valid) return;
  if (raw) {
#pragma unroll
    for (int i = 0; i < EE; ++i) {
      const int yy = tid + TPF * i;
      const bool never = !(ab[i] > T(0)) && (!PADDED || yy < n1);
      if (__builtin_amdgcn_ballot_w64(never) == 0) continue;
      if (never) {
        out[obase + yy] = cpx<T>{T(0), T(0)};
        if (kidx) kidx[obase + yy] = -1;
      }
    }
    return;
  }
  asm volatile("s_waitcnt vmcnt(0)" ::: "memory");
  const cpx<T>* dyp = dyc + (size_t)pt * n1;
  cpx<T> w[EE];
#pragma unroll
  for (int i = 0; i < EE; ++i) {
    const int yy = tid + TPF * i;
    w[i] = PADDED ? load_cpx<T>(orow, yy * (int)sizeof(cpx<T>), 0) : load_cpx<T>(orow, tid * (int)sizeof(cpx<T>), i * TPF * (int)sizeof(cpx<T>));
  }
#pragma unroll
  for (int i = 0; i < EE; ++i) {
    const int yy = tid + TPF * i;
    if (!PADDED || yy < n1) {
      cpx<T> v = {T(0), T(0)};
      if (ab[i] > T(0)) v = cmul(w[i], dyp[yy]);
      else if (kidx) kidx[obase + yy] = -1;
      out[obase + yy] = v;
    }
  }
}

template <class T>
__device__ __forceinline__ cpx<T> unit_phasor_s(double cycles) {
  double fr = cycles - rint(cycles);
  double s, c;
  sincospi(2.0 * fr, &s, &c);
  return {(T)c, (T)s};
}


template <class T, int LG, int EE>
__global__ __launch_bounds__(256) void shared_tables_kernel(const double* __restrict__ wys, const double* __restrict__ kr,
                                                           const int* __restrict__ shifts, const double* __restrict__ taps,
                                                           int Etab, int n1, int E, int Epad, int wrapped, int K, int nbl,
                                                           T* __restrict__ Gb, cpx<T>* __restrict__ psi,
                                                           cpx<T>* __restrict__ dyc, cpx<T>* __restrict__ pre,
                                                           cpx<T>* __restrict__ rot16) {
  using F = WgFFT<T, LG, EE>;
  constexpr int L = F::L, TPF = F::TPF;
  const int b = blockIdx.y;
  const int idx = blockIdx.x * 256 + threadIdx.x;
  const double wy = wys[b];
  if (idx < nbl * TPF) {
    const int i = idx / TPF, t = idx % TPF;
    const int kbin = F::spec_index(t, i);
    const double fq = wy + (double)kbin / (double)L;
    double acc = 0;
    for (int m = Etab; m >= 1; --m) {
      const double ph = fq * (double)m;
      acc += taps[m] * cospi(2.0 * (ph - rint(ph)));
    }
    Gb[(size_t)b * (nbl * TPF) + idx] = (T)((taps[0] + 2.0 * acc) / (double)L);
  }
  if (idx < Epad) {
    double ps, pc, qs, qc;
    const double c0 = -wy * (double)n1, c1 = wy * (double)(idx + 1);
    sincospi(2.0 * (c0 - rint(c0)), &ps, &pc);
    sincospi(2.0 * (c1 - rint(c1)), &qs, &qc);
    pc -= wrapped ? 1.0 : 0.0;
    cpx<T> v = {(T)(pc * qc - ps * qs), (T)(pc * qs + ps * qc)};
    if (idx >= E) v = {T(0), T(0)};
    psi[(size_t)b * Epad + idx] = v;
    pre[(size_t)b * Epad + idx] = unit_phasor_s<T>(wy * (double)idx);
  }
  if (b % K == 0) {
    const int p = b / K;
    const double sh = (double)shifts[p] / (double)EE;
    if (idx < n1) dyc[(size_t)p * n1 + idx] = unit_phasor_s<T>((kr[2 * b + 1] + sh) * (double)idx);
    if (idx < EE) rot16[p * EE + idx] = unit_phasor_s<T>(-sh * (double)idx);
  }
}

template <class T, int LG, int EE>
static hipError_t run_shared_tables(const Axis& a1, const double* wys, const double* kr, const int* shifts, const double* taps,
                                    int Etab, int E, int Epad, int B, int K, int nbl, const PassBSharedTables& st, hipStream_t s) {
  int len = a1.L > a1.n ? a1.L : a1.n;
  if (len < Epad) len = Epad;
  dim3 grid((len + 255) / 256, B);
  shared_tables_kernel<T, LG, EE><<<grid, 256, 0, s>>>(wys, kr, shifts, taps, Etab, a1.n, E, Epad, a1.padded ? 0 : 1, K, nbl,
                                                       (T*)st.Gb, (cpx<T>*)st.psi, (cpx<T>*)st.dyc, (cpx<T>*)st.pre,
                                                       (cpx<T>*)st.rot16);
  return hipGetLastError();
}

hipError_t launch_shared_tables(int dtype, const Axis& a1, const double* wys, const double* kr, const int* shifts,
                                const double* taps, int Etab, int E, int Epad, int B, int K, int nbl, const PassBSharedTables& st,
                                hipStream_t s) {
#define CASE_T(LG)                                                                                                      \
  if (a1.lg == LG)                                                                                                      \
    return dtype == 0 ? run_shared_tables<float, LG, 16>(a1, wys, kr, shifts, taps, Etab, E, Epad, B, K, nbl, st, s)    \
                      : run_shared_tables<double, LG, 16>(a1, wys, kr, shifts, taps, Etab, E, Epad, B, K, nbl, st, s);
  CASE_T(11) CASE_T(12) CASE_T(13)
#undef CASE_T
  return hipErrorInvalidValue;
}

template <class T, int LG, bool PADDED, int EE, int NBL, bool PSI = false>
static hipError_t run_passB_shared(const Axis& a1, int n0, const void* Tbuf, const void* tw1, const SweepTables& tb,
                                   const PassBSharedTables& st, int E, int Epad, int P, int K, void* out, int32_t* kidx,
                                   hipStream_t s, int nimg, int Bx, bool raw, void* psi_out = nullptr) {
  using G = PassBSGeom<T, LG, EE>;
  size_t lds = G::lds_bytes(Epad);
  if (lds > 160 * 1024 || E > G::TPF || Epad > G::TPF) return hipErrorInvalidValue;
  if (opt_set(OPT_PBS_LDS_PAD)) lds = std::min<size_t>(160 * 1024, lds + (size_t)opt(OPT_PBS_LDS_PAD).num);
  auto kern = passB_shared_kernel<T, LG, PADDED, EE, NBL, PSI>;
  static int lds_set[32] = {0};
  int dev = 0;
  (void)hipGetDevice(&dev);
  if (lds_set[dev & 31] < (int)lds) {
    hipError_t e = hipFuncSetAttribute(reinterpret_cast<const void*>(kern), hipFuncAttributeMaxDynamicSharedMemorySize, (int)lds);
    if (e != hipSuccess) return e;
    lds_set[dev & 31] = (int)lds;
  }
  dim3 grid((n0 + G::NF - 1) / G::NF, P * nimg);
  GPA_PROF(PSI ? "passB_shared_phases_kernel" : "passB_shared_kernel", s);
  kern<<<grid, G::THREADS, lds, s>>>((const cpx<T>*)Tbuf, n0, a1.n, (const T*)st.Gb, (const cpx<T>*)tw1, tb.planeof, st.order, st.desc,
                                     (const cpx<T>*)st.pre, (const cpx<T>*)st.psi, (const T*)st.gtab, (const cpx<T>*)tb.dx,
                                     (const cpx<T>*)st.dyc, (const cpx<T>*)st.rot16, K, E, Epad, (cpx<T>*)out, kidx, P, Bx, raw ? 1 : 0, (T*)psi_out);
  return hipGetLastError();
}

bool passB_shared_supports(int dtype, const Axis& a1, int E) {
  if (a1.lg < 11 || a1.lg > (dtype == 0 ? 13 : 12)) return false;
  const int tpf = a1.L / 16;
  const int Epad = (E + 15) & ~15;
  if (E < 1 || Epad > tpf || 2 * E > a1.n) return false;
  if (a1.padded && a1.n + E > a1.L) return false;
  const size_t csz = dtype == 0 ? 8 : 16;
  const int nf = tpf >= GPA_PBS_MINTHREADS ? 1 : GPA_PBS_MINTHREADS / tpf, nc = dtype == 0 ? 4 : 2;
  const size_t ES = (size_t)Epad + 4;
  const size_t stage = dtype == 0 ? 3 * nc * ES : 0;
  const size_t lds = (nf * ((size_t)(a1.L + a1.L / 16) + (dtype == 0 ? 4 : 2) * ES + 2 * nc * ES + stage) + 16 * 6) * csz +
                     (2 * (size_t)Epad + 16) * (csz / 2);
  return lds <= 160 * 1024;
}

int passB_shared_nbl(int dtype, int need) {
  if (dtype == 0 && need <= 6) return 6;
  if (need <= 8) return 8;
  return 16;
}

hipError_t launch_passB_shared_phases(int dtype, const Axis& a1, int n0, const void* Tbuf, const void* tw1, const SweepTables& tb,
                                      const PassBSharedTables& st, int E, int Epad, int P, int K, void* out, int32_t* kidx,
                                      void* psi_out, hipStream_t s, int Bx, int nbl) {
  if (!psi_out || !kidx) return hipErrorInvalidValue;
#define CALL_P(T, LG, NBL) \
  (a1.padded ? run_passB_shared<T, LG, true, 16, NBL, true>(a1, n0, Tbuf, tw1, tb, st, E, Epad, P, K, out, kidx, s, 1, Bx, false, psi_out) \
             : run_passB_shared<T, LG, false, 16, NBL, true>(a1, n0, Tbuf, tw1, tb, st, E, Epad, P, K, out, kidx, s, 1, Bx, false, psi_out))
#define CASE_P(LG, NBL) \
  if (a1.lg == LG && nbl == NBL) return dtype == 0 ? CALL_P(float, LG, NBL) : CALL_P(double, LG, NBL);
#define CASE_PF32(LG, NBL) \
  if (a1.lg == LG && nbl == NBL && dtype == 0) return CALL_P(float, LG, NBL);
  CASE_PF32(11, 6) CASE_PF32(12, 6) CASE_PF32(13, 6) CASE_PF32(13, 8) CASE_PF32(13, 16)
  CASE_P(11, 8) CASE_P(12, 8) CASE_P(11, 16) CASE_P(12, 16)
#undef CASE_PF32
#undef CASE_P
#undef CALL_P
  return hipErrorInvalidValue;
}

hipError_t launch_passB_shared(int dtype, const Axis& a1, int n0, const void* Tbuf, const void* tw1, const SweepTables& tb,
                               const PassBSharedTables& st, int E, int Epad, int P, int K, void* out, int32_t* kidx,
                               hipStream_t s, int nimg, int Bx, int nbl, bool raw) {
#define CALL_S(T, LG, NBL) \
  (a1.padded ? run_passB_shared<T, LG, true, 16, NBL>(a1, n0, Tbuf, tw1, tb, st, E, Epad, P, K, out, kidx, s, nimg, Bx, raw) \
             : run_passB_shared<T, LG, false, 16, NBL>(a1, n0, Tbuf, tw1, tb, st, E, Epad, P, K, out, kidx, s, nimg, Bx, raw))
#define CASE_S(LG, NBL) \
  if (a1.lg == LG && nbl == NBL) return dtype == 0 ? CALL_S(float, LG, NBL) : CALL_S(double, LG, NBL);
#define CASE_F32(LG, NBL) \
  if (a1.lg == LG && nbl == NBL && dtype == 0) return CALL_S(float, LG, NBL);
  CASE_F32(11, 6) CASE_F32(12, 6) CASE_F32(13, 6) CASE_F32(13, 8) CASE_F32(13, 16)
  CASE_S(11, 8) CASE_S(12, 8) CASE_S(11, 16) CASE_S(12, 16)
#undef CASE_F32
#undef CASE_S
#undef CALL_S
  return hipErrorInvalidValue;
}

}
```

### pygpa_amd/csrc/gpa_plan.h

```cpp
#pragma once
#include <math.h>
#include <stdio.h>
#include <stdlib.h>
#include <string.h>

#include <algorithm>
#include <complex>
#include <condition_variable>
#include <functional>
#include <mutex>
#include <thread>
#include <string>
#include <limits>
#include <vector>

#include "../../include/gpa_hip.h"
#include "gpa_internal.h"
#include "gpa_passb_shared.h"
#include "gpa_unwrap.h"
#include "gpa_dft.h"
#include "gpa_gaussfft.h"

using namespace gpa;

int gpa_fail(int code, const std::string& msg);
static inline int fail(int code, const std::string& msg) { return gpa_fail(code, msg); }

#define HIP_TRY(expr)                                                                         \
  do {                                                                                        \
    hipError_t _e = (expr);                                                                   \
    if (_e != hipSuccess)                                                                     \
      return fail(GPA_ERR_HIP, std::string(#expr) + ": " + hipGetErrorString(_e));            \
  } while (0)

#define NEED_UNWRAP(p, what)                                                                                     \
  do {                                                                                                             \
    if (!(p)->uw.impl)                                                                                             \
      return fail(GPA_ERR_STATE, std::string(what) + ": this plan's image is too large for the sweep / unwrap kernels " \
                                 "(an axis above 16384 pow2 / 8192 other in f32, 8192 / 4096 in f64); it serves per, "  \
                                 "find_peaks, gaussian_deconvolve and the per-pixel entry points only");                 \
  } while (0)

#define TRY(expr)            \
  do {                       \
    int _r = (expr);         \
    if (_r != GPA_OK) return _r; \
  } while (0)

struct EnqueueWorker {
  std::thread th;
  std::mutex m;
  std::condition_variable cv;
  std::function<void()> job;
  bool has_job = false, done = true, quit = false;
  explicit EnqueueWorker(int device) {
    th = std::thread([this, device] {
      (void)hipSetDevice(device);
      std::unique_lock<std::mutex> lk(m);
      for (;;) {
        cv.wait(lk, [this] { return has_job || quit; });
        if (quit) return;
        std::function<void()> j = std::move(job);
        has_job = false;
        lk.unlock();
        j();
        lk.lock();
        done = true;
        cv.notify_all();
      }
    });
  }
  void submit(std::function<void()> j) {
    std::lock_guard<std::mutex> lk(m);
    job = std::move(j);
    has_job = true;
    done = false;
    cv.notify_all();
  }
  void wait() {
    std::unique_lock<std::mutex> lk(m);
    cv.wait(lk, [this] { return done; });
  }
  ~EnqueueWorker() {
    {
      std::lock_guard<std::mutex> lk(m);
      quit = true;
      cv.notify_all();
    }
    if (th.joinable()) th.join();
  }
};

struct gpa_plan {
  int device = 0, dtype = 0, n0 = 0, n1 = 0, max_batch = 0;
  bool spectral_only = false;
  Axis ax0{}, ax1{};
  Axis ax0_full{}, ax1_full{};
  hipStream_t stream = nullptr;
  size_t rsz = 4, csz = 8;
  size_t ws_bytes = 0;
  void* tw0 = nullptr;
  void* tw1 = nullptr;
  void* Hx = nullptr;
  void* Hy = nullptr;
  double sigma_cached = -1.0;
  PassBSharedTables sh{};
  double* d_taps = nullptr;
  int sh_etab = 0, sh_E = 0, sh_Epad = 0;
  int sh_nbl = 16;
  double sh_sigma = 0.0;
  double* d_wys = nullptr;
  int* d_shifts = nullptr;
  Axis ax1s{};
  void* tw1s = nullptr;
  int tw1s_L = 0;
  bool sh_ok = false;
  bool use_shared = true;
  int sh_epoch = 0, sh_built_epoch = -1, sh_built_K = 0, sh_built_B = 0;
  bool sh_built_reorder = true;
  double* d_ystep = nullptr;
  bool sh_one_kref = true;
  bool lk_raw = false;
  bool sh_built_ok = false;
  bool sh_use = false;
  size_t sh_gb_bytes = 0, sh_psi_bytes = 0;
  std::vector<int> staged_planeof;
  void* Tbuf = nullptr;
  int tbuf_planes = 0;
  SweepTables tb{};
  double* d_kl = nullptr;
  double* d_kr = nullptr;
  double* d_pw = nullptr;
  int last_planes = 0;
  std::vector<double> staged_kl, staged_kr, staged_kmat;
  int* h_iters = nullptr;
  int iters_stride = 1;
  int iters_off = 0;
  UnwrapWorkspace uwp{};
  bool have_uwp = false, use_pair = false;
  double* h_k = nullptr;
  void* d_image = nullptr;
  void* d_mean = nullptr;
  void* d_tile_mean = nullptr;
  double* d_tsum_part = nullptr;
  size_t tsum_cap = 0;
  hipEvent_t ev_x = nullptr;
  double tile_mean = std::numeric_limits<double>::quiet_NaN();
  void* d_sf = nullptr;
  size_t sf_bytes = 0;
  void* d_grad = nullptr;
  void* d_grads = nullptr;
  void* d_absw = nullptr;
  double* d_scratch = nullptr;
  void* d_aux0 = nullptr;
  void* d_aux1 = nullptr;
  void* d_lockin = nullptr;
  int32_t* d_kidx = nullptr;
  int max_peaks = 0;
  void* d_dudx = nullptr;
  void* d_dudy = nullptr;
  void* d_wnorm = nullptr;
  void* d_u = nullptr;
  double* d_kmat = nullptr;
  UnwrapWorkspace uw{};
  UnwrapWorkspace uwb{};
  int uwb_images = 0;
  void* d_wnorm_b = nullptr;
  int* h_iters_b = nullptr;
  void *bT = nullptr, *bL = nullptr, *bMean = nullptr;
  double* bScratch = nullptr;
  size_t bT_bytes = 0, bL_bytes = 0;
  int b_chunk = 0;
  UnwrapWorkspace uw2{};
  hipStream_t stream2 = nullptr;
  hipEvent_t ev_fork = nullptr, ev_join = nullptr;
  DftAxis bx0{}, bx1{};
  DftWork dftw{};
  void* d_pertab = nullptr;
  struct GaussTab { double sigma = -1.0; int lg = 0; void* H = nullptr; void* tw = nullptr; int cap_lg = 0; unsigned stamp = 0; };
  GaussTab gft[2][2];
  unsigned gft_clock = 0;
  double* d_peakws = nullptr;
  void* d_peaksmooth = nullptr;
  bool peaks_smooth_valid = false;
  WarpWs warp{};
  UcellWs ucell{};
  hipEvent_t ev0 = nullptr, ev1 = nullptr;
  bool profiling = false;
  hipEvent_t stage_ev[6] = {nullptr, nullptr, nullptr, nullptr, nullptr, nullptr};
  float stage_ms[5] = {0, 0, 0, 0, 0};
  EnqueueWorker* worker = nullptr;
  bool use_worker = true, no_ksplit = false, no_compact = false;
  bool serial_unwrap = false;
  KernelProfiler* kprof = nullptr;
  std::string kprof_table;
  hipStream_t copy_stream = nullptr;
  hipEvent_t ev_dl_ready = nullptr, ev_dl_done[4] = {nullptr, nullptr, nullptr, nullptr};
};

template <class T>
static hipError_t upload_as(void* dst, const std::vector<double>& v, hipStream_t s) {
  std::vector<T> tmp(v.begin(), v.end());
  hipError_t e = hipMemcpyAsync(dst, tmp.data(), tmp.size() * sizeof(T), hipMemcpyHostToDevice, s);
  if (e != hipSuccess) return e;
  return hipStreamSynchronize(s);
}

void host_fft_pow2(std::vector<std::complex<double>>& a, bool inverse);
std::vector<double> gaussian_kspace(int n, double sigma);
std::vector<double> spatial_kernel(int n, const std::vector<double>& g);
int kernel_support(const std::vector<double>& h, double tol);
std::vector<double> spatial_taps(int n, const std::vector<double>& g, int mmax);
void build_filter_table(const Axis& ax, const std::vector<double>& g, const std::vector<double>& hsp,
                               std::vector<double>& out);
int ensure_filters(gpa_plan* p, double sigma);
int shared_prepare(gpa_plan* p, int P, int K);
int stage_kvectors(gpa_plan* p, const double* kl, const double* kr_per_b, int B, int* planes_out);
int ensure_tbuf(gpa_plan* p, int planes);
int ensure_sf(gpa_plan* p, size_t bytes);
int stage_kmat(gpa_plan* p, const double* kvecs, int P);
struct XPlanes { const void* T; int nimg, stride; };
int stage_sweep(gpa_plan* p, const double* krefs, int P, const double* klists, int K, double sigma, int* Bx);
int run_passA(gpa_plan* p, const void* image, const void* mean, void* Tbuf, int Bx, int nimg);
int passB_select(gpa_plan* p, const XPlanes& xp, int P, int K, void* lockin, int32_t* kidx, bool raw);
int passB_phases(gpa_plan* p, int P, int K, void* lockin, int32_t* kidx, void* psi, bool* shared);
void collect_kernel_profile(gpa_plan* p);
int sweep_peaks_dev(gpa_plan* p, const void* image, const void* mean, const double* krefs, int P,
                           const double* klists, int K, double sigma, void* lockin, int32_t* kidx, bool raw);
int tile_gradients_impl(gpa_plan* p, const void* image, size_t image_pitch, int r0, int c0, bool mean_on_device,
                               double mean, const double* kvecs, int P, const double* klists, int K, double sigma,
                               int mask_border, int i0, int j0, int t0, int t1, void* dx, size_t dx_pitch, size_t dx_plane,
                               void* dy, size_t dy_pitch, size_t dy_plane, void* wn, size_t wn_pitch, size_t wn_plane);
int plan_event(gpa_plan* p);
int dft_axes(gpa_plan* p);
int per_dft_staged(gpa_plan* p, const void* d_image, void* abs_out);
int gaussian_filter_dev(gpa_plan* p, const void* in, void* tmp, void* out, double sigma, const void* minuend);
int gaussian_weights(double sigma, std::vector<double>& w);
bool solve3(const double* m , const double* b, double* x);
Axis make_axis(int n);
Axis compact_axis(const Axis& full, int E);
int upload_real_table(gpa_plan* p, void* dst, const std::vector<double>& v);
int dmalloc(gpa_plan* p, void** ptr, size_t bytes);
inline int unwrap_fail(hipError_t e) {
  if (e == hipErrorNotSupported)
    return fail(GPA_ERR_STATE, "unwrap: no kernels for this shape -- an image with an axis that is not a power of two needs both axes <= 8192 "
                               "(f32) / 4096 (f64); powers of two go to 16384 / 8192 per axis (INTEGRATION.md, size limits)");
  return fail(GPA_ERR_HIP, std::string("unwrap: ") + hipGetErrorString(e));
}
int plan_build(gpa_plan* p);
int upload_twiddles(gpa_plan* p, void* dst, int L);

struct ProfInstallIf {
  bool own;
  ProfInstallIf(gpa_plan* p, bool own_) : own(own_ && p->profiling) {
    if (!own) return;
    if (!p->kprof) p->kprof = new KernelProfiler();
    p->kprof->n = 0;
    g_kprof = p->kprof;
  }
  ~ProfInstallIf() { if (own) g_kprof = nullptr; }
};
struct ProfInstall {
  explicit ProfInstall(gpa_plan* p) {
    if (!p->profiling) return;
    if (!p->kprof) p->kprof = new KernelProfiler();
    p->kprof->n = 0;
    g_kprof = p->kprof;
  }
  ~ProfInstall() { g_kprof = nullptr; }
};
```

### pygpa_amd/csrc/gpa_sweep.hip

```cpp
#include "gpa_internal.h"
#include "gpa_passb.h"

namespace gpa {

thread_local KernelProfiler* g_kprof = nullptr;

template <class T>
__device__ __forceinline__ cpx<T> unit_phasor(double cycles) {
  double fr = cycles - rint(cycles);
  double s, c;
  sincospi(2.0 * fr, &s, &c);
  return {(T)c, (T)s};
}

template <class T>
__global__ void tables_kernel(const double* __restrict__ kl, const double* __restrict__ kr,
                              const double* __restrict__ pw, int B, int Bx, int n0, int n1, int L0, int L1, int tpf0, int tpf1,
                              cpx<T>* cxb, cpx<T>* sx, cpx<T>* wxw, cpx<T>* wxr, cpx<T>* cyb, cpx<T>* sy, cpx<T>* wyw,
                              cpx<T>* wyr,
                              cpx<T>* dx, cpx<T>* dy) {
  const int b = blockIdx.y;
  const int j = blockIdx.x * blockDim.x + threadIdx.x;
  if (b < Bx) {
    const double wx = pw[b];
    const int tpf = tpf0;
    if (j < tpf) cxb[(size_t)b * tpf + j] = unit_phasor<T>(wx * j);
    if (j < 16) sx[b * 16 + j] = unit_phasor<T>(wx * (double)tpf * j);
    if (j == 0) wxw[b] = unit_phasor<T>(-wx * (double)(L0 - n0));
    if (j == 1) wxr[b] = unit_phasor<T>(-wx * (double)n0);
  }
  if (b < B) {
    const double wx = kl[2 * b], wy = kl[2 * b + 1], kx = kr[2 * b], ky = kr[2 * b + 1];
    const int tpf = tpf1;
    if (j < tpf) cyb[(size_t)b * tpf + j] = unit_phasor<T>(wy * j);
    if (j < 16) sy[b * 16 + j] = unit_phasor<T>(wy * (double)tpf * j);
    if (j == 0) wyw[b] = unit_phasor<T>(-wy * (double)(L1 - n1));
    if (j == 1) wyr[b] = unit_phasor<T>(-wy * (double)n1);
    if (j < n1) dy[(size_t)b * n1 + j] = unit_phasor<T>(-(wy - ky) * j);
    if (j < n0) dx[(size_t)b * n0 + j] = unit_phasor<T>(-(wx - kx) * j);
  }
}

hipError_t launch_tables(int dtype, const Axis& a0, const Axis& a1, const double* kl,
                         const double* kr, int B, const double* pw, int Bx, const SweepTables& tb,
                         hipStream_t s) {
  const int tpf0 = axis_tpf(a0), tpf1 = axis_tpf(a1);
  int len = a0.n > a1.n ? a0.n : a1.n;
  if (len < tpf0) len = tpf0;
  if (len < tpf1) len = tpf1;
  if (len < 16) len = 16;
  dim3 grid((len + 255) / 256, B > Bx ? B : Bx);
  if (dtype == 0)
    tables_kernel<float><<<grid, 256, 0, s>>>(kl, kr, pw, B, Bx, a0.n, a1.n, a0.L, a1.L, tpf0, tpf1, (cpx<float>*)tb.cxb,
                                              (cpx<float>*)tb.sx, (cpx<float>*)tb.wxw, (cpx<float>*)tb.wxr, (cpx<float>*)tb.cyb,
                                              (cpx<float>*)tb.sy, (cpx<float>*)tb.wyw, (cpx<float>*)tb.wyr, (cpx<float>*)tb.dx,
                                              (cpx<float>*)tb.dy);
  else
    tables_kernel<double><<<grid, 256, 0, s>>>(kl, kr, pw, B, Bx, a0.n, a1.n, a0.L, a1.L, tpf0, tpf1, (cpx<double>*)tb.cxb,
                                               (cpx<double>*)tb.sx, (cpx<double>*)tb.wxw, (cpx<double>*)tb.wxr, (cpx<double>*)tb.cyb,
                                               (cpx<double>*)tb.sy, (cpx<double>*)tb.wyw, (cpx<double>*)tb.wyr, (cpx<double>*)tb.dx,
                                               (cpx<double>*)tb.dy);
  return hipGetLastError();
}

template <class T> struct alignas(16) MeanVec4 { T v[4]; };
template <class T>
__global__ void mean_partial_kernel(const T* __restrict__ img, size_t count, double* partial) {
  img += (size_t)blockIdx.y * count;
  partial += (size_t)blockIdx.y * gridDim.x;
  __shared__ double sh[256];
  double acc = 0;
  if ((count & 3) == 0 && (reinterpret_cast<size_t>(img) & 15) == 0) {
    const MeanVec4<T>* v = reinterpret_cast<const MeanVec4<T>*>(img);
    const size_t c4 = count >> 2, step = (size_t)gridDim.x * 256;
    double a0 = 0, a1 = 0, a2 = 0, a3 = 0;
    size_t i = (size_t)blockIdx.x * 256 + threadIdx.x;
    for (; i + step < c4; i += 2 * step) {
      const MeanVec4<T> u = v[i], w = v[i + step];
      a0 += (double)u.v[0] + (double)w.v[0];
      a1 += (double)u.v[1] + (double)w.v[1];
      a2 += (double)u.v[2] + (double)w.v[2];
      a3 += (double)u.v[3] + (double)w.v[3];
    }
    if (i < c4) {
      const MeanVec4<T> u = v[i];
      a0 += (double)u.v[0]; a1 += (double)u.v[1]; a2 += (double)u.v[2]; a3 += (double)u.v[3];
    }
    acc = (a0 + a1) + (a2 + a3);
  } else {
    for (size_t i = (size_t)blockIdx.x * 256 + threadIdx.x; i < count; i += (size_t)gridDim.x * 256)
      acc += (double)img[i];
  }
  sh[threadIdx.x] = acc;
  __syncthreads();
  for (int s = 128; s > 0; s >>= 1) {
    if (threadIdx.x < s) sh[threadIdx.x] += sh[threadIdx.x + s];
    __syncthreads();
  }
  if (threadIdx.x == 0) partial[blockIdx.x] = sh[0];
}
template <class T>
__global__ void mean_final_kernel(const double* partial, int nparts, size_t count, T* mean_out) {
  partial += (size_t)blockIdx.y * nparts;
  mean_out += blockIdx.y;
  __shared__ double sh[256];
  double acc = 0;
  for (int i = threadIdx.x; i < nparts; i += 256) acc += partial[i];
  sh[threadIdx.x] = acc;
  __syncthreads();
  for (int s = 128; s > 0; s >>= 1) {
    if (threadIdx.x < s) sh[threadIdx.x] += sh[threadIdx.x + s];
    __syncthreads();
  }
  if (threadIdx.x == 0) *mean_out = (T)(sh[0] / (double)count);
}

hipError_t launch_mean(int dtype, const void* image, size_t count, double* scratch,
                       void* mean_out, hipStream_t s, int nimg) {
  const size_t want = count / 4096;
  const int nparts = want > 1024 ? 1024 : (want < 32 ? 32 : (int)want);
  GPA_PROF("mean_kernels", s);
  if (dtype == 0) {
    mean_partial_kernel<float><<<dim3(nparts, nimg), 256, 0, s>>>((const float*)image, count, scratch);
    mean_final_kernel<float><<<dim3(1, nimg), 256, 0, s>>>(scratch, nparts, count, (float*)mean_out);
  } else {
    mean_partial_kernel<double><<<dim3(nparts, nimg), 256, 0, s>>>((const double*)image, count, scratch);
    mean_final_kernel<double><<<dim3(1, nimg), 256, 0, s>>>(scratch, nparts, count, (double*)mean_out);
  }
  return hipGetLastError();
}

template <class T, int LG>
struct PassAGeom {
  using F = WgFFT<T, LG>;
  static constexpr int cols() {
#ifndef GPA_PA_C10
#define GPA_PA_C10 8
#endif
#ifndef GPA_PA_C9
#define GPA_PA_C9 16
#endif
#ifndef GPA_PA_C11
#define GPA_PA_C11 4
#endif
#ifndef GPA_PA_C12
#define GPA_PA_C12 16
#endif
    int c = LG == 10 ? GPA_PA_C10 : (LG == 9 ? GPA_PA_C9 : (LG == 11 ? GPA_PA_C11 : (LG == 12 ? GPA_PA_C12 : 16)));
    while (c > 1 && (c * F::TPF > 1024 || (size_t)c * (F::LDS_ELEMS + 32) * sizeof(cpx<T>) > 160 * 1024)) c /= 2;
    return c;
  }
  static constexpr int C = cols();
  static constexpr int NT = (sizeof(T) == 4 && C >= 2) ? 2 : 1;
  static constexpr int CT = C / NT;
  static constexpr int REGION = CT * F::LDS_ELEMS;
  static constexpr int THREADS = CT * F::TPF;
  static constexpr size_t LDS_BYTES = (size_t)NT * REGION * sizeof(cpx<T>);
  static constexpr bool FITS = (size_t)(F::LDS_ELEMS + 32) * sizeof(cpx<T>) <= 160 * 1024;
};

template <class T, int LG, bool PADDED>
__global__ __launch_bounds__((PassAGeom<T, LG>::THREADS)) void passA_kernel(
    const T* __restrict__ image, const T* __restrict__ mean, int n0, int n1,
    const cpx<T>* __restrict__ cxb, const cpx<T>* __restrict__ sx, const cpx<T>* __restrict__ wxw,
    const cpx<T>* __restrict__ wxr, int extL, int extR,
    const typename HType<PADDED, T>::type* __restrict__ H,
    const cpx<T>* __restrict__ twtab, cpx<T>* __restrict__ Tout, int B, int bchunk, int stag_phases, int stag_ticks,
    int stag_first, int rot_mul) {
  using F = WgFFT<T, LG>;
  using G = PassAGeom<T, LG>;
  constexpr int CT = G::CT, NT = G::NT, TPF = F::TPF, L = F::L;
  extern __shared__ __attribute__((aligned(16))) char smem[];
  const int c = threadIdx.x % CT, t = threadIdx.x / CT;
  cpx<T>* lds = reinterpret_cast<cpx<T>*>(smem) + c;
  constexpr int LDS_NSTRIDE = G::REGION;
  int tile = xcd_tile(blockIdx.x, gridDim.x);
  if (stag_phases < 0) {
    constexpr int TPL0 = (128 / (int)(G::C * sizeof(cpx<T>))) > 0 ? (128 / (int)(G::C * sizeof(cpx<T>))) : 1;
    const int g = TPL0 * -stag_phases, x = blockIdx.x & 7, idx = blockIdx.x >> 3;
    if (gridDim.x % (8 * g) == 0) tile = ((idx / g) * 8 + x) * g + idx % g;
  }
  const int y0 = tile * G::C + c * NT;
  image += (size_t)blockIdx.z * n0 * n1;
  Tout += (size_t)blockIdx.z * B * n0 * n1;
  const T m = mean ? mean[blockIdx.z] : T(0);

  T val[NT][16];
  unsigned wrapmask = 0, rightmask = 0;
#pragma unroll
  for (int n = 0; n < NT; ++n) {
    const int y = y0 + n;
#pragma unroll
    for (int i = 0; i < 16; ++i) {
      const int slot = t + TPF * i;
      const int xs = axis_src(slot, n0, L, PADDED, extL, extR);
      val[n][i] = (y < n1 && xs >= 0) ? image[(size_t)xs * n1 + y] - m : T(0);
      if (PADDED && slot >= n0) { if (slot < n0 + extR) rightmask |= 1u << i; else wrapmask |= 1u << i; }
    }
  }
  typename F::KTw tw;
  F::load_twiddles(tw, twtab, t);
  if (stag_phases > 1 && (int)blockIdx.x < stag_first) {
    constexpr int TPL = (128 / (int)(G::C * sizeof(cpx<T>))) > 0 ? (128 / (int)(G::C * sizeof(cpx<T>))) : 1;
    const int ph = (tile / TPL) % stag_phases;
    asm volatile("s_waitcnt vmcnt(0)" ::: "memory");
    if (ph) {
      const unsigned long long t0 = wall_clock64(), wait = (unsigned long long)ph * (unsigned)stag_ticks;
      while (wall_clock64() - t0 < wait) __builtin_amdgcn_s_sleep(4);
    }
    __syncthreads();
  }

  const int b0 = blockIdx.y * bchunk;
  const int b1 = (b0 + bchunk < B) ? b0 + bchunk : B;
  const int nb = b1 - b0;
  int b = b0 + (nb > 0 ? (int)(((unsigned)(tile * G::C * (int)sizeof(cpx<T>) / 128) * (unsigned)rot_mul) % (unsigned)nb) : 0);
  for (int j = 0; j < nb; ++j, b = (b + 1 < b1 ? b + 1 : b0)) {
    F::refresh(tw);
    const cpx<T> base = cxb[(size_t)b * TPF + t];
    cpx<T> x[NT][16];
#pragma unroll
    for (int i = 0; i < 16; ++i) {
      cpx<T> ph = cmul(base, sx[b * 16 + i]);
      if (PADDED && ((wrapmask >> i) & 1)) ph = cmul(ph, wxw[b]);
      if (PADDED && ((rightmask >> i) & 1)) ph = cmul(ph, wxr[b]);
#pragma unroll
      for (int n = 0; n < NT; ++n) x[n][i] = {val[n][i] * ph.x, val[n][i] * ph.y};
    }
    F::template forward_multi<NT, CT>(x, lds, LDS_NSTRIDE, t, tw);
    {
      const typename HType<PADDED, T>::type* Hb = H;
      asm volatile("" : "+s"(Hb));
#pragma unroll
      for (int i = 0; i < 16; ++i) {
        const auto h = hload<PADDED, T>(Hb, i * TPF + t);
#pragma unroll
        for (int n = 0; n < NT; ++n) x[n][i] = hmul(x[n][i], h);
      }
    }
    F::template inverse_multi<NT, CT>(x, lds, LDS_NSTRIDE, t, tw);
    bool paired = false;
    if constexpr (NT == 2) {
      if (y0 + 1 < n1 && (n1 & 1) == 0) {
        paired = true;
        struct alignas(2 * sizeof(cpx<T>)) Pair { cpx<T> a, b; };
        auto put = [&](int i) {
          const int slot = t + TPF * i;
          if (!PADDED || slot < n0) {
            Pair pr = {x[0][i], x[1][i]};
            *reinterpret_cast<Pair*>(&Tout[((size_t)b * n0 + slot) * n1 + y0]) = pr;
          }
        };
#pragma unroll
        for (int i = 0; i < 16; ++i) put(i);
      }
    }
    if (!paired) {
#pragma unroll
      for (int n = 0; n < NT; ++n) {
        const int y = y0 + n;
        if (y < n1) {
#pragma unroll
          for (int i = 0; i < 16; ++i) {
            const int slot = t + TPF * i;
            if (!PADDED || slot < n0) Tout[((size_t)b * n0 + slot) * n1 + y] = x[n][i];
          }
        }
      }
    }
  }
}

template <class T, int LG, bool PADDED>
static hipError_t run_passA(const Axis& a0, int n1, const void* image, const void* mean,
                            const SweepTables& tb, const void* Hx, const void* tw0, void* Tbuf,
                            int B, hipStream_t s, int nimg) {
  using G = PassAGeom<T, LG>;
  if constexpr (!G::FITS) {
    return hipErrorInvalidValue;
  } else {
    auto kern = passA_kernel<T, LG, PADDED>;
    static unsigned lds_set = 0;
    hipError_t e = set_dynamic_lds_once(reinterpret_cast<const void*>(kern), (int)G::LDS_BYTES, lds_set);
    if (e != hipSuccess) return e;
    const int tiles = (n1 + G::C - 1) / G::C;
    int ysplit = 1;
    while (tiles * ysplit < 512 && ysplit < B) ysplit *= 2;
    if (ysplit > B) ysplit = B;
    const int bchunk = (B + ysplit - 1) / ysplit;
    dim3 grid(tiles, (B + bchunk - 1) / bchunk, nimg);
    const int stag = opt_set(OPT_PA_STAG) ? (int)opt(OPT_PA_STAG).num : 0;
    const int stag_ticks = opt_set(OPT_PA_STAG_TICKS) ? (int)opt(OPT_PA_STAG_TICKS).num : 800 / (stag > 1 ? stag : 1);
    GPA_PROF("passA_kernel", s);
    kern<<<grid, G::THREADS, G::LDS_BYTES, s>>>(
        (const T*)image, (const T*)mean, a0.n, n1, (const cpx<T>*)tb.cxb, (const cpx<T>*)tb.sx,
        (const cpx<T>*)tb.wxw, (const cpx<T>*)tb.wxr, a0.extL, a0.extR,
        (const typename HType<PADDED, T>::type*)Hx, (const cpx<T>*)tw0, (cpx<T>*)Tbuf, B, bchunk, stag,
        stag_ticks, device_cus(), opt_set(OPT_PA_ROT) ? (int)opt(OPT_PA_ROT).num : (LG >= 12 ? 1 : 0));
    return hipGetLastError();
  }
}


hipError_t launch_passA(int dtype, const Axis& a0, int n1, const void* image, const void* mean,
                        const SweepTables& tb, const void* Hx, const void* tw0, void* Tbuf,
                        int B, hipStream_t s, int nimg) {
#define CASE_A(LG)                                                                                \
  case LG:                                                                                        \
    if (dtype == 0)                                                                               \
      return a0.padded ? run_passA<float, LG, true>(a0, n1, image, mean, tb, Hx, tw0, Tbuf, B, s, nimg) \
                       : run_passA<float, LG, false>(a0, n1, image, mean, tb, Hx, tw0, Tbuf, B, s, nimg); \
    else                                                                                          \
      return a0.padded ? run_passA<double, LG, true>(a0, n1, image, mean, tb, Hx, tw0, Tbuf, B, s, nimg) \
                       : run_passA<double, LG, false>(a0, n1, image, mean, tb, Hx, tw0, Tbuf, B, s, nimg);
  switch (a0.lg) { GPA_FOR_LG(CASE_A) }
#undef CASE_A
  return hipErrorInvalidValue;
}

hipError_t launch_passB(int dtype, const Axis& a1, int n0, const void* Tbuf, const void* Hy,
                        const void* tw1, const SweepTables& tb, int P, int K, bool select,
                        void* out, int32_t* kidx, hipStream_t s, int nimg, int Bx) {
#define CALL_B(T, LG, PD)                                                                                                   \
  (select ? run_passB<T, LG, PD, PB_SELECT>(a1, n0, Tbuf, Hy, tw1, tb, P, K, out, kidx, nullptr, nullptr, s, 1, nimg, Bx)    \
          : run_passB<T, LG, PD, PB_ALL>(a1, n0, Tbuf, Hy, tw1, tb, P, K, out, kidx, nullptr, nullptr, s, 1, nimg, Bx))
#define CASE_B(LG)                                                           \
  case LG:                                                                   \
    if (dtype == 0) return a1.padded ? CALL_B(float, LG, true) : CALL_B(float, LG, false); \
    else return a1.padded ? CALL_B(double, LG, true) : CALL_B(double, LG, false);
  switch (a1.lg) { GPA_FOR_LG(CASE_B) }
#undef CASE_B
#undef CALL_B
  return hipErrorInvalidValue;
}

int passA_cols(int dtype, int lg) {
#define CASE_C(LG) \
  case LG: return dtype == 0 ? PassAGeom<float, LG>::C : PassAGeom<double, LG>::C;
  switch (lg) { GPA_FOR_LG(CASE_C) }
#undef CASE_C
  return 0;
}

int spec_index_rt(int lg, int tid, int reg, int elems) {
  if (elems == 8) {
#define CASE_S8(LG) \
  case LG: return WgFFT<float, LG, 8>::spec_index(tid, reg);
    switch (lg) { CASE_S8(6) CASE_S8(7) CASE_S8(8) CASE_S8(9) CASE_S8(10) CASE_S8(11) CASE_S8(12) }
#undef CASE_S8
    return -1;
  }
#define CASE_S(LG) \
  case LG: return WgFFT<float, LG>::spec_index(tid, reg);
  switch (lg) { GPA_FOR_LG(CASE_S) }
#undef CASE_S
  return -1;
}

}
```

Baseline: 3212 Mpixels/s.

## Add y-spectral pass A: row FFT once, then x-filter only needed spectral blocks

Adds a y-spectral path for the sweep. A row FFT kernel transforms the image along y once and stores only the spectral blocks the peaks' bands need. Pass A then runs the x-direction filtering on those (plane, block) pairs, writes compact strips, and the shared pass B reads the strips with per-peak shifts instead of redoing the y transform on the full band. This aims to cut pass A/B FLOPs and HBM traffic on periodic 2048/4096 rows. The cost is extra Yhat and strip buffers, two more launches, host-side pair tables built with a synchronisation, and new failure paths when ksplit or the non-shared pass B would be chosen.

```diff
diff --git a/pygpa_amd/csrc/gpa_api.hip b/pygpa_amd/csrc/gpa_api.hip
--- a/pygpa_amd/csrc/gpa_api.hip
+++ b/pygpa_amd/csrc/gpa_api.hip
@@ -10,7 +10,7 @@
     "PBS_FULLBAND", "SERIAL_UNWRAP", "NO_WORKER", "NO_KSPLIT", "NO_COMPACT", "NO_SHARED",
     "NO_PAIR", "TRI_SMALL", "TRI_Q", "NO_MR", "MR_FORCE_BLUESTEIN", "NO_ROWPQ", "COLSOLVE", "NO_LAT",
     "F32_EPS_FLOOR", "COLSTREAM_CHUNK", "NO_ROWHALF", "PAIR_MAXSIDE", "ROWHALF_MINLG", "NO_PQDCT",
-    "NO_REORDER", "NO_RAW", "NO_TILEFUSE", "NO_ROWPERS", "NO_LFTILE", "LF_ALL_ROUNDS", "DFT_ENGINE", "GAUSS_FFT_MINR", "NO_GAUSS2D", "NO_DFT_HALF", "F32_STALL", "PBS_LDS_PAD", "NO_SHARED_PHASES", "PA_STAG", "PA_STAG_TICKS", "PA_ROT", "LF_STACK_BYTES"};
+    "NO_REORDER", "NO_RAW", "NO_TILEFUSE", "NO_ROWPERS", "NO_LFTILE", "LF_ALL_ROUNDS", "DFT_ENGINE", "GAUSS_FFT_MINR", "NO_GAUSS2D", "NO_DFT_HALF", "F32_STALL", "PBS_LDS_PAD", "NO_SHARED_PHASES", "PA_STAG", "PA_STAG_TICKS", "PA_ROT", "LF_STACK_BYTES", "NO_YSPEC"};
 static OptVal g_opts[OPT_COUNT];
 static std::once_flag g_opts_once;
 static void opt_assign(OptVal& o, const char* value) {
@@ -224,7 +224,7 @@
                   p->tb.dx, p->tb.dy, p->d_kl, p->d_kr, p->d_image, p->d_mean, p->d_tile_mean, p->d_scratch,
                   p->d_lockin, p->d_kidx, p->d_dudx, p->d_dudy, p->d_wnorm, p->d_u, p->d_kmat, p->d_sf, p->d_grad, p->d_grads, p->d_absw, p->d_aux0, p->d_aux1,
                   p->sh.Gb, p->sh.psi, p->sh.dyc, p->sh.gtab, p->sh.desc, p->sh.order, p->d_taps, p->tw1s,
-                  p->sh.pre, p->sh.rot16, p->d_wys, p->d_shifts, p->d_ystep};
+                  p->sh.pre, p->sh.rot16, p->d_wys, p->d_shifts, p->d_ystep, p->ys.Yhat, p->ys.strips, p->d_ys_pairs};
   for (void* b : bufs)
     if (b) hipFree(b);
   unwrap_workspace_destroy(&p->uw);
diff --git a/pygpa_amd/csrc/gpa_api_driver.hip b/pygpa_amd/csrc/gpa_api_driver.hip
--- a/pygpa_amd/csrc/gpa_api_driver.hip
+++ b/pygpa_amd/csrc/gpa_api_driver.hip
@@ -15,8 +15,8 @@
   return GPA_OK;
 }
 
-static int extract_stage(gpa_plan* p, const double* kvecs, int P, const double* klists, int K, double sigma, int* Bx) {
-  TRY(stage_sweep(p, kvecs, P, klists, K, sigma, Bx));
+static int extract_stage(gpa_plan* p, const double* kvecs, int P, const double* klists, int K, double sigma, int* Bx, int passb) {
+  TRY(stage_sweep(p, kvecs, P, klists, K, sigma, Bx, passb));
   TRY(stage_kmat(p, kvecs, P));
   {
     const size_t side = opt_set(OPT_PAIR_MAXSIDE) ? (size_t)opt(OPT_PAIR_MAXSIDE).num : 1024;
@@ -124,7 +124,7 @@
   if (o.grads && (o.grad_mode < 0 || o.grad_mode > 2)) return fail(GPA_ERR_ARG, fn + ": grad_mode must be 0, 1 or 2");
   HIP_TRY(hipSetDevice(p->device));
   int Bx = 0;
-  TRY(extract_stage(p, kvecs, P, klists, K, sigma, &Bx));
+  TRY(extract_stage(p, kvecs, P, klists, K, sigma, &Bx, o.grads ? SWEEP_PASSB_PHASES : SWEEP_PASSB_SELECT));
   if (o.grads) TRY(ensure_sf(p, (size_t)P * K * p->n0 * p->n1 * p->rsz));
   ProfInstall prof(p);
   return extract_launch(p, image, P, K, Bx, mask_border, kmax, u, o);
@@ -291,7 +291,7 @@
   TRY(check_ranges(p, fn, P, K, kmax));
   HIP_TRY(hipSetDevice(p->device));
   int Bx = 0;
-  TRY(extract_stage(p, kvecs, P, klists, K, sigma, &Bx));
+  TRY(extract_stage(p, kvecs, P, klists, K, sigma, &Bx, SWEEP_PASSB_SELECT));
   TRY(ensure_batch_unwrap(p, B));
   const size_t npx = (size_t)p->n0 * p->n1;
   const size_t t_img = (size_t)Bx * npx * p->csz, l_img = (size_t)P * npx * p->csz;
diff --git a/pygpa_amd/csrc/gpa_api_sweep.hip b/pygpa_amd/csrc/gpa_api_sweep.hip
--- a/pygpa_amd/csrc/gpa_api_sweep.hip
+++ b/pygpa_amd/csrc/gpa_api_sweep.hip
@@ -28,8 +28,16 @@
   return GPA_OK;
 }
 
-int stage_sweep(gpa_plan* p, const double* krefs, int P, const double* klists, int K, double sigma, int* Bx) {
+static bool shared_passB_runs(const gpa_plan* p, int passb) {
+  if (!p->sh_use) return false;
+  const bool phases_ok = p->use_shared && !opt_set(OPT_NO_SHARED_PHASES) && p->sh_one_kref;
+  if (passb == SWEEP_PASSB_SELECT) return true;
+  return passb == SWEEP_PASSB_PHASES && phases_ok;
+}
+
+int stage_sweep(gpa_plan* p, const double* krefs, int P, const double* klists, int K, double sigma, int* Bx, int passb) {
   const int B = P * K;
+  p->ys_use = false;
   TRY(ensure_filters(p, sigma));
   std::vector<double> kr((size_t)B * 2);
   for (int pp = 0; pp < P; ++pp)
@@ -38,10 +46,21 @@
       kr[2 * ((size_t)pp * K + k) + 1] = krefs[2 * pp + 1];
     }
   TRY(stage_kvectors(p, klists, kr.data(), B, Bx));
-  return ensure_tbuf(p, *Bx);
+  TRY(ensure_tbuf(p, *Bx));
+  if (passb != SWEEP_PASSB_OTHER) {
+    TRY(shared_prepare(p, P, K));
+    p->ys_use = shared_passB_runs(p, passb) && p->ys_ok && !opt_set(OPT_NO_YSPEC);
+    if (p->ys_use) TRY(ensure_yspec(p, 1, *Bx));
+  }
+  return GPA_OK;
 }
 
 int run_passA(gpa_plan* p, const void* image, const void* mean, void* Tbuf, int Bx, int nimg) {
+  if (p->ys_use) {
+    TRY(ensure_yspec(p, nimg, Bx));
+    HIP_TRY(launch_passA_yspec(p->dtype, p->ax0, p->ax1, image, mean, p->tb, p->Hx, p->tw0, p->tw1, Tbuf, Bx, p->ys, p->stream, nimg));
+    return GPA_OK;
+  }
   HIP_TRY(launch_passA(p->dtype, p->ax0, p->n1, image, mean, p->tb, p->Hx, p->tw0, Tbuf, Bx, p->stream, nimg));
   return GPA_OK;
 }
@@ -52,13 +71,18 @@
   int ksplit = 1;
   if (xp.stride == 0 && p->ax1.lg <= 10 && K >= 4 && !p->no_ksplit && rows_wg <= 256)
     while (ksplit < 4 && ksplit * 2 <= K && rows_wg * ksplit < 1024) ksplit *= 2;
+  const bool ys = p->ys_use;
+  if (ys && ksplit != 1) return fail(GPA_ERR_STATE, "pass B: the staged sweep took the y-spectral pass A");
   if (ksplit == 1) {
     TRY(shared_prepare(p, P, K));
+    p->ys_use = ys;
+    if (ys && !p->sh_use) return fail(GPA_ERR_STATE, "pass B: the staged sweep took the y-spectral pass A");
     if (p->sh_use) {
       p->lk_raw = raw && !opt_set(OPT_NO_RAW) && p->sh_one_kref;
+      const PassBYspec yb = {p->ys.strips, p->d_shifts};
       HIP_TRY(launch_passB_shared(p->dtype, p->ax1s, p->n0, xp.T, p->ax1s.L == p->ax1.L ? p->tw1 : p->tw1s, p->tb,
                                   p->sh, p->sh_E, p->sh_Epad, P, K, lockin, kidx, p->stream, xp.nimg, xp.stride, p->sh_nbl,
-                                  p->lk_raw));
+                                  p->lk_raw, ys ? &yb : nullptr));
     } else
       HIP_TRY(launch_passB(p->dtype, p->ax1, p->n0, xp.T, p->Hy, p->tw1, p->tb, P, K, true, lockin, kidx, p->stream, xp.nimg,
                            xp.stride));
@@ -76,19 +100,23 @@
 int passB_phases(gpa_plan* p, int P, int K, void* lockin, int32_t* kidx, void* psi, bool* shared) {
   p->lk_raw = false;
   *shared = false;
+  const bool ys = p->ys_use;
   if (p->use_shared && !opt_set(OPT_NO_SHARED_PHASES)) {
     TRY(shared_prepare(p, P, K));
+    p->ys_use = ys;
     if (p->sh_use && p->sh_one_kref) {
+      const PassBYspec yb = {p->ys.strips, p->d_shifts};
       const hipError_t e = launch_passB_shared_phases(p->dtype, p->ax1s, p->n0, p->Tbuf, p->ax1s.L == p->ax1.L ? p->tw1 : p->tw1s,
                                                       p->tb, p->sh, p->sh_E, p->sh_Epad, P, K, lockin, kidx, psi, p->stream, 0,
-                                                      p->sh_nbl);
+                                                      p->sh_nbl, ys ? &yb : nullptr);
       if (e == hipSuccess) {
         *shared = true;
         return GPA_OK;
       }
-      if (e != hipErrorInvalidValue) return fail(GPA_ERR_HIP, std::string("shared pass B (phases): ") + hipGetErrorString(e));
+      if (e != hipErrorInvalidValue || ys) return fail(GPA_ERR_HIP, std::string("shared pass B (phases): ") + hipGetErrorString(e));
     }
   }
+  if (ys) return fail(GPA_ERR_STATE, "pass B (phases): the staged sweep took the y-spectral pass A");
   HIP_TRY(launch_passB_ext(p->dtype, p->ax1, p->n0, p->Tbuf, p->Hy, p->tw1, p->tb, K, 3, lockin, kidx, nullptr, psi, p->stream, P));
   return GPA_OK;
 }
@@ -119,7 +147,7 @@
                            const double* klists, int K, double sigma, void* lockin, int32_t* kidx, bool raw) {
   if (P * K > p->max_batch) return fail(GPA_ERR_STATE, "sweep: P*K exceeds the plan's max_batch");
   int Bx = 0;
-  TRY(stage_sweep(p, krefs, P, klists, K, sigma, &Bx));
+  TRY(stage_sweep(p, krefs, P, klists, K, sigma, &Bx, SWEEP_PASSB_SELECT));
   if (p->profiling) HIP_TRY(hipEventRecord(p->stage_ev[1], p->stream));
   TRY(run_passA(p, image, mean, p->Tbuf, Bx, 1));
   if (p->profiling) HIP_TRY(hipEventRecord(p->stage_ev[2], p->stream));
@@ -152,7 +180,7 @@
   TRY(ensure_sf(p, (size_t)K * npx * p->rsz));
   int32_t* ki = kidx ? kidx : p->d_kidx;
   int Bx = 0;
-  TRY(stage_sweep(p, kref, 1, klist, K, sigma, &Bx));
+  TRY(stage_sweep(p, kref, 1, klist, K, sigma, &Bx, SWEEP_PASSB_PHASES));
   TRY(run_passA(p, image, nullptr, p->Tbuf, Bx, 1));
   bool shared = false;
   TRY(passB_phases(p, 1, K, lockin, ki, p->d_sf, &shared));
diff --git a/pygpa_amd/csrc/gpa_api_tables.hip b/pygpa_amd/csrc/gpa_api_tables.hip
--- a/pygpa_amd/csrc/gpa_api_tables.hip
+++ b/pygpa_amd/csrc/gpa_api_tables.hip
@@ -174,6 +174,7 @@
 
 int shared_prepare(gpa_plan* p, int P, int K) {
   p->sh_use = false;
+  p->ys_use = false;
   const int B = P * K;
   if (!p->sh_ok || !p->use_shared || K < 2 || (int)p->staged_planeof.size() < B) return GPA_OK;
   const bool reorder = !opt_set(OPT_NO_REORDER);
@@ -309,6 +310,32 @@
   HIP_TRY(launch_shared_tables(p->dtype, p->ax1s, p->d_wys, p->d_kr, p->d_shifts, p->d_taps, p->sh_etab, p->sh_E, p->sh_Epad, B, K,
                                p->sh_nbl, p->sh, p->stream));
   HIP_TRY(hipStreamSynchronize(p->stream));
+  p->ys_ok = false;
+  if (passB_yspec_supports(p->dtype, p->ax1s, p->sh_nbl) && p->ax1s.L == p->ax1.L && !p->ax1.padded) {
+    const int nplanes = p->last_planes;
+    std::vector<unsigned> mask((size_t)nplanes, 0u);
+    for (int b = 0; b < B; ++b) mask[p->staged_planeof[b]] |= yspec_blockmask(p->ax1s.lg, shifts[b / K], p->sh_nbl);
+    std::vector<int> pairs;
+    unsigned all = 0;
+    for (int slot = 0; slot < 16; ++slot)
+      for (int q = 0; q < nplanes; ++q) {
+        int seen = 0;
+        for (int blk = 0; blk < 16; ++blk)
+          if ((mask[q] >> blk) & 1) {
+            if (seen++ == slot) pairs.push_back(q | (blk << 16));
+          }
+        all |= mask[q];
+      }
+    if (!p->d_ys_pairs) TRY(dmalloc(p, (void**)&p->d_ys_pairs, (size_t)p->max_batch * 16 * sizeof(int)));
+    HIP_TRY(hipMemcpyAsync(p->d_ys_pairs, pairs.data(), pairs.size() * sizeof(int), hipMemcpyHostToDevice, p->stream));
+    HIP_TRY(hipStreamSynchronize(p->stream));
+    p->ys.pairs = p->d_ys_pairs;
+    p->ys.npairs = (int)pairs.size();
+    p->ys.blockmask = all;
+    p->ys.E = p->sh_E;
+    p->ys.Epad = p->sh_Epad;
+    p->ys_ok = !pairs.empty();
+  }
   p->sh_built_epoch = p->sh_epoch;
   p->sh_built_K = K;
   p->sh_built_B = B;
@@ -318,6 +345,7 @@
 }
 
 int stage_kvectors(gpa_plan* p, const double* kl, const double* kr_per_b, int B, int* planes_out) {
+  p->ys_use = false;
   if ((int)p->staged_kl.size() == 2 * B && memcmp(p->staged_kl.data(), kl, (size_t)B * 2 * sizeof(double)) == 0 &&
       memcmp(p->staged_kr.data(), kr_per_b, (size_t)B * 2 * sizeof(double)) == 0) {
     *planes_out = p->last_planes;
@@ -366,6 +394,23 @@
   return GPA_OK;
 }
 
+int ensure_yspec(gpa_plan* p, int nimg, int Bx) {
+  const size_t yb = (size_t)nimg * p->n0 * p->n1 * p->csz, sb = (size_t)nimg * Bx * p->n0 * 2 * p->sh_Epad * p->csz;
+  if (yb > p->ys_yhat_bytes) {
+    HIP_TRY(hipStreamSynchronize(p->stream));
+    if (p->ys.Yhat) { HIP_TRY(hipFree(p->ys.Yhat)); p->ws_bytes -= p->ys_yhat_bytes; p->ys.Yhat = nullptr; p->ys_yhat_bytes = 0; }
+    TRY(dmalloc(p, &p->ys.Yhat, yb));
+    p->ys_yhat_bytes = yb;
+  }
+  if (sb > p->ys_strips_bytes) {
+    HIP_TRY(hipStreamSynchronize(p->stream));
+    if (p->ys.strips) { HIP_TRY(hipFree(p->ys.strips)); p->ws_bytes -= p->ys_strips_bytes; p->ys.strips = nullptr; p->ys_strips_bytes = 0; }
+    TRY(dmalloc(p, &p->ys.strips, sb));
+    p->ys_strips_bytes = sb;
+  }
+  return GPA_OK;
+}
+
 int ensure_sf(gpa_plan* p, size_t bytes) {
   if (p->sf_bytes >= bytes) return GPA_OK;
   if (p->d_sf) {
diff --git a/pygpa_amd/csrc/gpa_internal.h b/pygpa_amd/csrc/gpa_internal.h
--- a/pygpa_amd/csrc/gpa_internal.h
+++ b/pygpa_amd/csrc/gpa_internal.h
@@ -71,7 +71,7 @@
   OPT_PBS_FULLBAND, OPT_SERIAL_UNWRAP, OPT_NO_WORKER, OPT_NO_KSPLIT, OPT_NO_COMPACT, OPT_NO_SHARED,
   OPT_NO_PAIR, OPT_TRI_SMALL, OPT_TRI_Q, OPT_NO_MR, OPT_MR_FORCE_BLUESTEIN, OPT_NO_ROWPQ,
   OPT_COLSOLVE, OPT_NO_LAT, OPT_F32_EPS_FLOOR, OPT_COLSTREAM_CHUNK, OPT_NO_ROWHALF, OPT_PAIR_MAXSIDE, OPT_ROWHALF_MINLG, OPT_NO_PQDCT,
-  OPT_NO_REORDER, OPT_NO_RAW, OPT_NO_TILEFUSE, OPT_NO_ROWPERS, OPT_NO_LFTILE, OPT_LF_ALL_ROUNDS, OPT_DFT_ENGINE, OPT_GAUSS_FFT_MINR, OPT_NO_GAUSS2D, OPT_NO_DFT_HALF, OPT_F32_STALL, OPT_PBS_LDS_PAD, OPT_NO_SHARED_PHASES, OPT_PA_STAG, OPT_PA_STAG_TICKS, OPT_PA_ROT, OPT_LF_STACK_BYTES, OPT_COUNT
+  OPT_NO_REORDER, OPT_NO_RAW, OPT_NO_TILEFUSE, OPT_NO_ROWPERS, OPT_NO_LFTILE, OPT_LF_ALL_ROUNDS, OPT_DFT_ENGINE, OPT_GAUSS_FFT_MINR, OPT_NO_GAUSS2D, OPT_NO_DFT_HALF, OPT_F32_STALL, OPT_PBS_LDS_PAD, OPT_NO_SHARED_PHASES, OPT_PA_STAG, OPT_PA_STAG_TICKS, OPT_PA_ROT, OPT_LF_STACK_BYTES, OPT_NO_YSPEC, OPT_COUNT
 };
 struct OptVal {
   bool set;
@@ -124,6 +124,17 @@
 hipError_t launch_passA(int dtype, const Axis& a0, int n1, const void* image, const void* mean,
                         const SweepTables& tb, const void* Hx, const void* tw0, void* Tbuf,
                         int Bx, hipStream_t s, int nimg = 1);
+struct PassAYspec {
+  void* Yhat;
+  void* strips;
+  const int* pairs;
+  int npairs;
+  unsigned blockmask;
+  int E, Epad;
+};
+hipError_t launch_passA_yspec(int dtype, const Axis& a0, const Axis& a1, const void* image, const void* mean,
+                              const SweepTables& tb, const void* Hx, const void* tw0, const void* tw1, void* Tbuf, int Bx,
+                              const PassAYspec& ys, hipStream_t s, int nimg = 1);
 hipError_t launch_passB(int dtype, const Axis& a1, int n0, const void* Tbuf, const void* Hy,
                         const void* tw1, const SweepTables& tb, int P, int K, bool select,
                         void* out, int32_t* kidx, hipStream_t s, int nimg = 1, int Bx = 0);
diff --git a/pygpa_amd/csrc/gpa_passb_shared.h b/pygpa_amd/csrc/gpa_passb_shared.h
--- a/pygpa_amd/csrc/gpa_passb_shared.h
+++ b/pygpa_amd/csrc/gpa_passb_shared.h
@@ -23,12 +23,16 @@
                                 hipStream_t s);
 int passB_shared_nbl(int dtype, int need);
 
+struct PassBYspec { const void* strips; const int* shifts; };
+bool passB_yspec_supports(int dtype, const Axis& a1, int nbl);
+
 hipError_t launch_passB_shared(int dtype, const Axis& a1, int n0, const void* Tbuf, const void* tw1, const SweepTables& tb,
                                const PassBSharedTables& st, int E, int Epad, int P, int K, void* out, int32_t* kidx,
-                               hipStream_t s, int nimg = 1, int Bx = 0, int nbl = 16, bool raw = false);
+                               hipStream_t s, int nimg = 1, int Bx = 0, int nbl = 16, bool raw = false,
+                               const PassBYspec* ys = nullptr);
 hipError_t launch_passB_shared_phases(int dtype, const Axis& a1, int n0, const void* Tbuf, const void* tw1, const SweepTables& tb,
                                       const PassBSharedTables& st, int E, int Epad, int P, int K, void* out, int32_t* kidx,
-                                      void* psi_out, hipStream_t s, int Bx, int nbl);
+                                      void* psi_out, hipStream_t s, int Bx, int nbl, const PassBYspec* ys = nullptr);
 
 
 }
diff --git a/pygpa_amd/csrc/gpa_passb_shared.hip b/pygpa_amd/csrc/gpa_passb_shared.hip
--- a/pygpa_amd/csrc/gpa_passb_shared.hip
+++ b/pygpa_amd/csrc/gpa_passb_shared.hip
@@ -2,6 +2,7 @@
 
 #include "gpa_internal.h"
 #include "gpa_passb_shared.h"
+#include "gpa_yspec.h"
 
 namespace gpa {
 
@@ -110,14 +111,16 @@
 #ifndef GPA_PBS_L13_WAVES
 #define GPA_PBS_L13_WAVES 3
 #endif
-template <class T, int LG, bool PADDED, int EE, int NBL, bool PSI = false>
+template <class T, int LG, bool PADDED, int EE, int NBL, bool PSI = false, bool YSPEC = false>
 __global__ __launch_bounds__((PassBSGeom<T, LG, EE>::THREADS),
                              (sizeof(T) == 8 ? GPA_PBS_F64_WAVES : (LG >= 13 ? GPA_PBS_L13_WAVES : (PADDED ? GPA_PBS_PAD_WAVES : GPA_PBS_F32_WAVES)))) void passB_shared_kernel(
     const cpx<T>* __restrict__ Tin, int n0, int n1, const T* __restrict__ Gb, const cpx<T>* __restrict__ twtab,
     const int* __restrict__ planeof, const int* __restrict__ order, const int* __restrict__ desc, const cpx<T>* __restrict__ pre_g,
     const cpx<T>* __restrict__ psi, const T* __restrict__ gtab, const cpx<T>* __restrict__ dx,
     const cpx<T>* __restrict__ dyc, const cpx<T>* __restrict__ rot16, int K, int E, int Epad, cpx<T>* out,
-    int32_t* kidx, int P, int Bx, int raw, T* __restrict__ psi_out) {
+    int32_t* kidx, int P, int Bx, int raw, T* __restrict__ psi_out, const cpx<T>* __restrict__ strips_in,
+    const int* __restrict__ shifts) {
+  static_assert(!YSPEC || (!PADDED && EE == 16 && NBL < EE), "y-spectral pass B: periodic rows, a rotated band");
   using F = WgFFT<T, LG, EE>;
   using G = PassBSGeom<T, LG, EE>;
   using V4 = typename MfmaVec<T>::type;
@@ -164,13 +167,42 @@
   const cpx<T> rot = rot16[pt * EE + (tid & (EE - 1))];
   const cpx<T> rot_tail = rot16[pt * EE + ((n1 - 1 - (tid < E ? tid : 0)) & (EE - 1))];
   constexpr bool PREFETCH = NBL < EE && sizeof(T) == 4;
+  int ytq = tid, ysh = 0;
+  if constexpr (YSPEC) {
+    const YspecSrc y0s = yspec_source(LG, shifts[pt], tid, 0);
+    ytq = y0s.tid;
+    ysh = y0s.reg;
+  }
+  auto put_strips = [&](cpx<T> s0, cpx<T> s1) {
+    if constexpr (G::SV == 4) {
+      strip[0 * ES + tid] = {s0.x, -s0.y};
+      strip[1 * ES + tid] = {s0.y, s0.x};
+      strip[2 * ES + tid] = {s1.x, s1.y};
+      strip[3 * ES + tid] = {s1.y, -s1.x};
+    } else {
+      strip[0 * ES + tid] = {s0.x, s0.y};
+      strip[1 * ES + tid] = {s1.x, s1.y};
+    }
+  };
   for (int k = 0; k < K; ++k) {
     const int b = pt * K + k;
     const int ob = order[b];
     const int d = desc[b];
     if (d & 1) {
-      const cpx<T>* src = Tin + (((size_t)img * Bx + planeof[ob]) * n0 + rr) * n1;
+      const size_t prow = ((size_t)img * Bx + planeof[ob]) * n0 + rr;
+      const cpx<T>* src = Tin + prow * n1;
       const cpx<T> cs0 = dx[(size_t)ob * n0 + rr];
+      if constexpr (YSPEC) {
+#pragma unroll
+        for (int i = 0; i < NBL; ++i) X[i] = cmul(load_once(src + ((i + ysh) & (EE - 1)) * TPF + ytq), cs0);
+        if (tid < Epad) {
+          const cpx<T>* sp = strips_in + prow * (2 * Epad);
+          const bool in = tid < E;
+          const cpx<T> s0 = in ? cmul(sp[tid], cmul(cs0, rot)) : cpx<T>{T(0), T(0)};
+          const cpx<T> s1 = in ? cmul(sp[2 * Epad - 1 - tid], cmul(cs0, rot_tail)) : cpx<T>{T(0), T(0)};
+          put_strips(s0, s1);
+        }
+      } else {
       const cpx<T> cs = cmul(cs0, rot);
       cpx<T> tail = {T(0), T(0)};
       if (tid < E) tail = src[n1 - 1 - tid];
@@ -188,19 +220,12 @@
         const bool in = tid < E;
         const cpx<T> s0 = in ? XX[0] : cpx<T>{T(0), T(0)};
         const cpx<T> s1 = in ? cmul(tail, cmul(cs0, rot_tail)) : cpx<T>{T(0), T(0)};
-        if constexpr (G::SV == 4) {
-          strip[0 * ES + tid] = {s0.x, -s0.y};
-          strip[1 * ES + tid] = {s0.y, s0.x};
-          strip[2 * ES + tid] = {s1.x, s1.y};
-          strip[3 * ES + tid] = {s1.y, -s1.x};
-        } else {
-          strip[0 * ES + tid] = {s0.x, s0.y};
-          strip[1 * ES + tid] = {s1.x, s1.y};
-        }
+        put_strips(s0, s1);
       }
       F::forward(XX, lds, tid, tw);
 #pragma unroll
       for (int i = 0; i < NBL; ++i) X[i] = XX[i];
+      }
     }
     const int par = (d >> 7) & 1;
     cpx<T> y[EE];
@@ -454,15 +479,17 @@
   return hipErrorInvalidValue;
 }
 
-template <class T, int LG, bool PADDED, int EE, int NBL, bool PSI = false>
+template <class T, int LG, bool PADDED, int EE, int NBL, bool PSI = false, bool YSPEC = false>
 static hipError_t run_passB_shared(const Axis& a1, int n0, const void* Tbuf, const void* tw1, const SweepTables& tb,
                                    const PassBSharedTables& st, int E, int Epad, int P, int K, void* out, int32_t* kidx,
-                                   hipStream_t s, int nimg, int Bx, bool raw, void* psi_out = nullptr) {
+                                   hipStream_t s, int nimg, int Bx, bool raw, void* psi_out = nullptr,
+                                   const PassBYspec* ys = nullptr) {
+  if (YSPEC && (!ys || !ys->strips || !ys->shifts)) return hipErrorInvalidValue;
   using G = PassBSGeom<T, LG, EE>;
   size_t lds = G::lds_bytes(Epad);
   if (lds > 160 * 1024 || E > G::TPF || Epad > G::TPF) return hipErrorInvalidValue;
   if (opt_set(OPT_PBS_LDS_PAD)) lds = std::min<size_t>(160 * 1024, lds + (size_t)opt(OPT_PBS_LDS_PAD).num);
-  auto kern = passB_shared_kernel<T, LG, PADDED, EE, NBL, PSI>;
+  auto kern = passB_shared_kernel<T, LG, PADDED, EE, NBL, PSI, YSPEC>;
   static int lds_set[32] = {0};
   int dev = 0;
   (void)hipGetDevice(&dev);
@@ -475,7 +502,8 @@
   GPA_PROF(PSI ? "passB_shared_phases_kernel" : "passB_shared_kernel", s);
   kern<<<grid, G::THREADS, lds, s>>>((const cpx<T>*)Tbuf, n0, a1.n, (const T*)st.Gb, (const cpx<T>*)tw1, tb.planeof, st.order, st.desc,
                                      (const cpx<T>*)st.pre, (const cpx<T>*)st.psi, (const T*)st.gtab, (const cpx<T>*)tb.dx,
-                                     (const cpx<T>*)st.dyc, (const cpx<T>*)st.rot16, K, E, Epad, (cpx<T>*)out, kidx, P, Bx, raw ? 1 : 0, (T*)psi_out);
+                                     (const cpx<T>*)st.dyc, (const cpx<T>*)st.rot16, K, E, Epad, (cpx<T>*)out, kidx, P, Bx, raw ? 1 : 0, (T*)psi_out,
+                                     (const cpx<T>*)(YSPEC ? ys->strips : nullptr), YSPEC ? ys->shifts : nullptr);
   return hipGetLastError();
 }
 
@@ -494,6 +522,10 @@
   return lds <= 160 * 1024;
 }
 
+bool passB_yspec_supports(int dtype, const Axis& a1, int nbl) {
+  return !a1.padded && a1.n == a1.L && yspec_lg_ok(a1.lg) && (nbl == 8 || (nbl == 6 && dtype == 0));
+}
+
 int passB_shared_nbl(int dtype, int need) {
   if (dtype == 0 && need <= 6) return 6;
   if (need <= 8) return 8;
@@ -502,8 +534,17 @@
 
 hipError_t launch_passB_shared_phases(int dtype, const Axis& a1, int n0, const void* Tbuf, const void* tw1, const SweepTables& tb,
                                       const PassBSharedTables& st, int E, int Epad, int P, int K, void* out, int32_t* kidx,
-                                      void* psi_out, hipStream_t s, int Bx, int nbl) {
+                                      void* psi_out, hipStream_t s, int Bx, int nbl, const PassBYspec* ys) {
   if (!psi_out || !kidx) return hipErrorInvalidValue;
+  if (ys) {
+    if (a1.padded) return hipErrorInvalidValue;
+#define CASE_Y(T, LG, NBL) \
+    if (a1.lg == LG && nbl == NBL && dtype == (sizeof(T) == 4 ? 0 : 1)) \
+      return run_passB_shared<T, LG, false, 16, NBL, true, true>(a1, n0, Tbuf, tw1, tb, st, E, Epad, P, K, out, kidx, s, 1, Bx, false, psi_out, ys);
+    CASE_Y(float, 11, 6) CASE_Y(float, 12, 6) CASE_Y(float, 11, 8) CASE_Y(float, 12, 8) CASE_Y(double, 11, 8) CASE_Y(double, 12, 8)
+#undef CASE_Y
+    return hipErrorInvalidValue;
+  }
 #define CALL_P(T, LG, NBL) \
   (a1.padded ? run_passB_shared<T, LG, true, 16, NBL, true>(a1, n0, Tbuf, tw1, tb, st, E, Epad, P, K, out, kidx, s, 1, Bx, false, psi_out) \
              : run_passB_shared<T, LG, false, 16, NBL, true>(a1, n0, Tbuf, tw1, tb, st, E, Epad, P, K, out, kidx, s, 1, Bx, false, psi_out))
@@ -521,7 +562,16 @@
 
 hipError_t launch_passB_shared(int dtype, const Axis& a1, int n0, const void* Tbuf, const void* tw1, const SweepTables& tb,
                                const PassBSharedTables& st, int E, int Epad, int P, int K, void* out, int32_t* kidx,
-                               hipStream_t s, int nimg, int Bx, int nbl, bool raw) {
+                               hipStream_t s, int nimg, int Bx, int nbl, bool raw, const PassBYspec* ys) {
+  if (ys) {
+    if (a1.padded) return hipErrorInvalidValue;
+#define CASE_Y(T, LG, NBL) \
+    if (a1.lg == LG && nbl == NBL && dtype == (sizeof(T) == 4 ? 0 : 1)) \
+      return run_passB_shared<T, LG, false, 16, NBL, false, true>(a1, n0, Tbuf, tw1, tb, st, E, Epad, P, K, out, kidx, s, nimg, Bx, raw, nullptr, ys);
+    CASE_Y(float, 11, 6) CASE_Y(float, 12, 6) CASE_Y(float, 11, 8) CASE_Y(float, 12, 8) CASE_Y(double, 11, 8) CASE_Y(double, 12, 8)
+#undef CASE_Y
+    return hipErrorInvalidValue;
+  }
 #define CALL_S(T, LG, NBL) \
   (a1.padded ? run_passB_shared<T, LG, true, 16, NBL>(a1, n0, Tbuf, tw1, tb, st, E, Epad, P, K, out, kidx, s, nimg, Bx, raw) \
              : run_passB_shared<T, LG, false, 16, NBL>(a1, n0, Tbuf, tw1, tb, st, E, Epad, P, K, out, kidx, s, nimg, Bx, raw))
diff --git a/pygpa_amd/csrc/gpa_plan.h b/pygpa_amd/csrc/gpa_plan.h
--- a/pygpa_amd/csrc/gpa_plan.h
+++ b/pygpa_amd/csrc/gpa_plan.h
@@ -17,6 +17,7 @@
 #include "../../include/gpa_hip.h"
 #include "gpa_internal.h"
 #include "gpa_passb_shared.h"
+#include "gpa_yspec.h"
 #include "gpa_unwrap.h"
 #include "gpa_dft.h"
 #include "gpa_gaussfft.h"
@@ -124,6 +125,11 @@
   bool sh_built_ok = false;
   bool sh_use = false;
   size_t sh_gb_bytes = 0, sh_psi_bytes = 0;
+  bool ys_ok = false;
+  bool ys_use = false;
+  PassAYspec ys{};
+  int* d_ys_pairs = nullptr;
+  size_t ys_yhat_bytes = 0, ys_strips_bytes = 0;
   std::vector<int> staged_planeof;
   void* Tbuf = nullptr;
   int tbuf_planes = 0;
@@ -220,7 +226,10 @@
 int ensure_sf(gpa_plan* p, size_t bytes);
 int stage_kmat(gpa_plan* p, const double* kvecs, int P);
 struct XPlanes { const void* T; int nimg, stride; };
-int stage_sweep(gpa_plan* p, const double* krefs, int P, const double* klists, int K, double sigma, int* Bx);
+enum { SWEEP_PASSB_OTHER = 0, SWEEP_PASSB_SELECT = 1, SWEEP_PASSB_PHASES = 2 };
+int stage_sweep(gpa_plan* p, const double* krefs, int P, const double* klists, int K, double sigma, int* Bx,
+                int passb = SWEEP_PASSB_OTHER);
+int ensure_yspec(gpa_plan* p, int nimg, int Bx);
 int run_passA(gpa_plan* p, const void* image, const void* mean, void* Tbuf, int Bx, int nimg);
 int passB_select(gpa_plan* p, const XPlanes& xp, int P, int K, void* lockin, int32_t* kidx, bool raw);
 int passB_phases(gpa_plan* p, int P, int K, void* lockin, int32_t* kidx, void* psi, bool* shared);
diff --git a/pygpa_amd/csrc/gpa_sweep.hip b/pygpa_amd/csrc/gpa_sweep.hip
--- a/pygpa_amd/csrc/gpa_sweep.hip
+++ b/pygpa_amd/csrc/gpa_sweep.hip
@@ -1,5 +1,6 @@
 #include "gpa_internal.h"
 #include "gpa_passb.h"
+#include "gpa_yspec.h"
 
 namespace gpa {
 
@@ -159,14 +160,16 @@
   static constexpr bool FITS = (size_t)(F::LDS_ELEMS + 32) * sizeof(cpx<T>) <= 160 * 1024;
 };
 
-template <class T, int LG, bool PADDED>
+enum { PA_SPATIAL = 0, PA_YSPEC = 1, PA_STRIPS = 2 };
+template <class T, int LG, bool PADDED, int MODE = PA_SPATIAL>
 __global__ __launch_bounds__((PassAGeom<T, LG>::THREADS)) void passA_kernel(
     const T* __restrict__ image, const T* __restrict__ mean, int n0, int n1,
     const cpx<T>* __restrict__ cxb, const cpx<T>* __restrict__ sx, const cpx<T>* __restrict__ wxw,
     const cpx<T>* __restrict__ wxr, int extL, int extR,
     const typename HType<PADDED, T>::type* __restrict__ H,
     const cpx<T>* __restrict__ twtab, cpx<T>* __restrict__ Tout, int B, int bchunk, int stag_phases, int stag_ticks,
-    int stag_first, int rot_mul) {
+    int stag_first, int rot_mul, const cpx<T>* __restrict__ Yin, const int* __restrict__ pairs, int npairs, int ntl,
+    int opitch) {
   using F = WgFFT<T, LG>;
   using G = PassAGeom<T, LG>;
   constexpr int CT = G::CT, NT = G::NT, TPF = F::TPF, L = F::L;
@@ -175,32 +178,58 @@
   cpx<T>* lds = reinterpret_cast<cpx<T>*>(smem) + c;
   constexpr int LDS_NSTRIDE = G::REGION;
   int tile = xcd_tile(blockIdx.x, gridDim.x);
-  if (stag_phases < 0) {
+  if (MODE == PA_SPATIAL && stag_phases < 0) {
     constexpr int TPL0 = (128 / (int)(G::C * sizeof(cpx<T>))) > 0 ? (128 / (int)(G::C * sizeof(cpx<T>))) : 1;
     const int g = TPL0 * -stag_phases, x = blockIdx.x & 7, idx = blockIdx.x >> 3;
     if (gridDim.x % (8 * g) == 0) tile = ((idx / g) * 8 + x) * g + idx % g;
   }
-  const int y0 = tile * G::C + c * NT;
-  image += (size_t)blockIdx.z * n0 * n1;
-  Tout += (size_t)blockIdx.z * B * n0 * n1;
-  const T m = mean ? mean[blockIdx.z] : T(0);
-
-  T val[NT][16];
+  int y0 = tile * G::C + c * NT;
+  int oy0 = y0;
+  int plane = 0;
+  const int op = MODE == PA_STRIPS ? opitch : n1;
+  if constexpr (MODE == PA_YSPEC) {
+    constexpr int TPL = (128 / (int)(G::C * sizeof(cpx<T>))) > 0 ? (128 / (int)(G::C * sizeof(cpx<T>))) : 1;
+    const int tl = tile % TPL, pr = (tile / TPL) % npairs, ln = tile / (TPL * npairs);
+    const int pe = pairs[pr];
+    plane = pe & 0xffff;
+    y0 = (pe >> 16) * (n1 >> 4) + (ln * TPL + tl) * G::C + c * NT;
+    oy0 = y0;
+  } else if constexpr (MODE == PA_STRIPS) {
+    y0 = (tile < ntl ? tile * G::C : n1 - (2 * ntl - tile) * G::C) + c * NT;
+    oy0 = tile < ntl ? y0 : y0 - (n1 - opitch);
+  }
+  if constexpr (MODE == PA_YSPEC) Yin += (size_t)blockIdx.z * n0 * n1;
+  else image += (size_t)blockIdx.z * n0 * n1;
+  Tout += (size_t)blockIdx.z * B * n0 * op;
+  const T m = (MODE != PA_YSPEC && mean) ? mean[blockIdx.z] : T(0);
+
+  T val[MODE == PA_YSPEC ? 1 : NT][16];
+  cpx<T> cval[MODE == PA_YSPEC ? NT : 1][16];
   unsigned wrapmask = 0, rightmask = 0;
 #pragma unroll
-  for (int n = 0; n < NT; ++n) {
-    const int y = y0 + n;
-#pragma unroll
-    for (int i = 0; i < 16; ++i) {
-      const int slot = t + TPF * i;
-      const int xs = axis_src(slot, n0, L, PADDED, extL, extR);
-      val[n][i] = (y < n1 && xs >= 0) ? image[(size_t)xs * n1 + y] - m : T(0);
-      if (PADDED && slot >= n0) { if (slot < n0 + extR) rightmask |= 1u << i; else wrapmask |= 1u << i; }
+  for (int i = 0; i < 16; ++i) {
+    const int slot = t + TPF * i;
+    const int xs = axis_src(slot, n0, L, PADDED, extL, extR);
+    if (PADDED && slot >= n0) { if (slot < n0 + extR) rightmask |= 1u << i; else wrapmask |= 1u << i; }
+    if constexpr (MODE == PA_YSPEC) {
+      struct alignas(NT * sizeof(cpx<T>)) Cols { cpx<T> v[NT]; };
+      Cols cc;
+#pragma unroll
+      for (int n = 0; n < NT; ++n) cc.v[n] = {T(0), T(0)};
+      if (xs >= 0) cc = *reinterpret_cast<const Cols*>(&Yin[(size_t)xs * n1 + y0]);
+#pragma unroll
+      for (int n = 0; n < NT; ++n) cval[n][i] = cc.v[n];
+    } else {
+#pragma unroll
+      for (int n = 0; n < NT; ++n) {
+        const int y = y0 + n;
+        val[n][i] = (y < n1 && xs >= 0) ? image[(size_t)xs * n1 + y] - m : T(0);
+      }
     }
   }
   typename F::KTw tw;
   F::load_twiddles(tw, twtab, t);
-  if (stag_phases > 1 && (int)blockIdx.x < stag_first) {
+  if (MODE == PA_SPATIAL && stag_phases > 1 && (int)blockIdx.x < stag_first) {
     constexpr int TPL = (128 / (int)(G::C * sizeof(cpx<T>))) > 0 ? (128 / (int)(G::C * sizeof(cpx<T>))) : 1;
     const int ph = (tile / TPL) % stag_phases;
     asm volatile("s_waitcnt vmcnt(0)" ::: "memory");
@@ -211,8 +240,8 @@
     __syncthreads();
   }
 
-  const int b0 = blockIdx.y * bchunk;
-  const int b1 = (b0 + bchunk < B) ? b0 + bchunk : B;
+  const int b0 = MODE == PA_YSPEC ? plane : blockIdx.y * bchunk;
+  const int b1 = MODE == PA_YSPEC ? plane + 1 : ((b0 + bchunk < B) ? b0 + bchunk : B);
   const int nb = b1 - b0;
   int b = b0 + (nb > 0 ? (int)(((unsigned)(tile * G::C * (int)sizeof(cpx<T>) / 128) * (unsigned)rot_mul) % (unsigned)nb) : 0);
   for (int j = 0; j < nb; ++j, b = (b + 1 < b1 ? b + 1 : b0)) {
@@ -225,7 +254,10 @@
       if (PADDED && ((wrapmask >> i) & 1)) ph = cmul(ph, wxw[b]);
       if (PADDED && ((rightmask >> i) & 1)) ph = cmul(ph, wxr[b]);
 #pragma unroll
-      for (int n = 0; n < NT; ++n) x[n][i] = {val[n][i] * ph.x, val[n][i] * ph.y};
+      for (int n = 0; n < NT; ++n) {
+        if constexpr (MODE == PA_YSPEC) x[n][i] = cmul(cval[n][i], ph);
+        else x[n][i] = {val[n][i] * ph.x, val[n][i] * ph.y};
+      }
     }
     F::template forward_multi<NT, CT>(x, lds, LDS_NSTRIDE, t, tw);
     {
@@ -241,14 +273,14 @@
     F::template inverse_multi<NT, CT>(x, lds, LDS_NSTRIDE, t, tw);
     bool paired = false;
     if constexpr (NT == 2) {
-      if (y0 + 1 < n1 && (n1 & 1) == 0) {
+      if (y0 + 1 < n1 && (op & 1) == 0) {
         paired = true;
         struct alignas(2 * sizeof(cpx<T>)) Pair { cpx<T> a, b; };
         auto put = [&](int i) {
           const int slot = t + TPF * i;
           if (!PADDED || slot < n0) {
             Pair pr = {x[0][i], x[1][i]};
-            *reinterpret_cast<Pair*>(&Tout[((size_t)b * n0 + slot) * n1 + y0]) = pr;
+            *reinterpret_cast<Pair*>(&Tout[((size_t)b * n0 + slot) * op + oy0]) = pr;
           }
         };
 #pragma unroll
@@ -263,7 +295,7 @@
 #pragma unroll
           for (int i = 0; i < 16; ++i) {
             const int slot = t + TPF * i;
-            if (!PADDED || slot < n0) Tout[((size_t)b * n0 + slot) * n1 + y] = x[n][i];
+            if (!PADDED || slot < n0) Tout[((size_t)b * n0 + slot) * op + oy0 + n] = x[n][i];
           }
         }
       }
@@ -271,51 +303,116 @@
   }
 }
 
-template <class T, int LG, bool PADDED>
+template <class T, int LG, bool PADDED, int MODE>
 static hipError_t run_passA(const Axis& a0, int n1, const void* image, const void* mean,
                             const SweepTables& tb, const void* Hx, const void* tw0, void* Tbuf,
-                            int B, hipStream_t s, int nimg) {
+                            int B, hipStream_t s, int nimg, const PassAYspec* ys) {
   using G = PassAGeom<T, LG>;
   if constexpr (!G::FITS) {
     return hipErrorInvalidValue;
   } else {
-    auto kern = passA_kernel<T, LG, PADDED>;
+    auto kern = passA_kernel<T, LG, PADDED, MODE>;
     static unsigned lds_set = 0;
     hipError_t e = set_dynamic_lds_once(reinterpret_cast<const void*>(kern), (int)G::LDS_BYTES, lds_set);
     if (e != hipSuccess) return e;
-    const int tiles = (n1 + G::C - 1) / G::C;
+    int tiles = (n1 + G::C - 1) / G::C, ntl = 0, opitch = n1;
+    if (MODE == PA_YSPEC) {
+      if (n1 % (16 * G::C) || ((size_t)(n1 / 16) * sizeof(cpx<T>)) % 128 || ys->npairs < 1) return hipErrorInvalidValue;
+      tiles = ys->npairs * (n1 / 16 / G::C);
+    } else if (MODE == PA_STRIPS) {
+      ntl = (ys->E + G::C - 1) / G::C;
+      opitch = 2 * ys->Epad;
+      if (n1 % G::C || ntl * G::C > ys->Epad || 2 * ntl * G::C > n1) return hipErrorInvalidValue;
+      tiles = 2 * ntl;
+    }
     int ysplit = 1;
-    while (tiles * ysplit < 512 && ysplit < B) ysplit *= 2;
+    while (MODE != PA_YSPEC && tiles * ysplit < 512 && ysplit < B) ysplit *= 2;
     if (ysplit > B) ysplit = B;
     const int bchunk = (B + ysplit - 1) / ysplit;
     dim3 grid(tiles, (B + bchunk - 1) / bchunk, nimg);
     const int stag = opt_set(OPT_PA_STAG) ? (int)opt(OPT_PA_STAG).num : 0;
     const int stag_ticks = opt_set(OPT_PA_STAG_TICKS) ? (int)opt(OPT_PA_STAG_TICKS).num : 800 / (stag > 1 ? stag : 1);
-    GPA_PROF("passA_kernel", s);
+    GPA_PROF(MODE == PA_STRIPS ? "passA_strips_kernel" : "passA_kernel", s);
     kern<<<grid, G::THREADS, G::LDS_BYTES, s>>>(
         (const T*)image, (const T*)mean, a0.n, n1, (const cpx<T>*)tb.cxb, (const cpx<T>*)tb.sx,
         (const cpx<T>*)tb.wxw, (const cpx<T>*)tb.wxr, a0.extL, a0.extR,
-        (const typename HType<PADDED, T>::type*)Hx, (const cpx<T>*)tw0, (cpx<T>*)Tbuf, B, bchunk, stag,
-        stag_ticks, device_cus(), opt_set(OPT_PA_ROT) ? (int)opt(OPT_PA_ROT).num : (LG >= 12 ? 1 : 0));
+        (const typename HType<PADDED, T>::type*)Hx, (const cpx<T>*)tw0, (cpx<T>*)(MODE == PA_STRIPS ? ys->strips : Tbuf), B, bchunk, stag,
+        stag_ticks, device_cus(), opt_set(OPT_PA_ROT) ? (int)opt(OPT_PA_ROT).num : (LG >= 12 ? 1 : 0),
+        (const cpx<T>*)(ys ? ys->Yhat : nullptr), ys ? ys->pairs : nullptr, ys ? ys->npairs : 0, ntl, opitch);
     return hipGetLastError();
   }
 }
 
+template <int MODE>
+static hipError_t dispatch_passA(int dtype, const Axis& a0, int n1, const void* image, const void* mean,
+                                 const SweepTables& tb, const void* Hx, const void* tw0, void* Tbuf,
+                                 int B, hipStream_t s, int nimg, const PassAYspec* ys) {
+#define CASE_A(LG)                                                                                \
+  case LG:                                                                                        \
+    if (dtype == 0)                                                                               \
+      return a0.padded ? run_passA<float, LG, true, MODE>(a0, n1, image, mean, tb, Hx, tw0, Tbuf, B, s, nimg, ys) \
+                       : run_passA<float, LG, false, MODE>(a0, n1, image, mean, tb, Hx, tw0, Tbuf, B, s, nimg, ys); \
+    else                                                                                          \
+      return a0.padded ? run_passA<double, LG, true, MODE>(a0, n1, image, mean, tb, Hx, tw0, Tbuf, B, s, nimg, ys) \
+                       : run_passA<double, LG, false, MODE>(a0, n1, image, mean, tb, Hx, tw0, Tbuf, B, s, nimg, ys);
+  switch (a0.lg) { GPA_FOR_LG(CASE_A) }
+#undef CASE_A
+  return hipErrorInvalidValue;
+}
 
 hipError_t launch_passA(int dtype, const Axis& a0, int n1, const void* image, const void* mean,
                         const SweepTables& tb, const void* Hx, const void* tw0, void* Tbuf,
                         int B, hipStream_t s, int nimg) {
-#define CASE_A(LG)                                                                                \
-  case LG:                                                                                        \
-    if (dtype == 0)                                                                               \
-      return a0.padded ? run_passA<float, LG, true>(a0, n1, image, mean, tb, Hx, tw0, Tbuf, B, s, nimg) \
-                       : run_passA<float, LG, false>(a0, n1, image, mean, tb, Hx, tw0, Tbuf, B, s, nimg); \
-    else                                                                                          \
-      return a0.padded ? run_passA<double, LG, true>(a0, n1, image, mean, tb, Hx, tw0, Tbuf, B, s, nimg) \
-                       : run_passA<double, LG, false>(a0, n1, image, mean, tb, Hx, tw0, Tbuf, B, s, nimg);
-  switch (a0.lg) { GPA_FOR_LG(CASE_A) }
-#undef CASE_A
-  return hipErrorInvalidValue;
+  return dispatch_passA<PA_SPATIAL>(dtype, a0, n1, image, mean, tb, Hx, tw0, Tbuf, B, s, nimg, nullptr);
+}
+
+template <class T, int LG>
+__global__ __launch_bounds__((WgFFT<T, LG, 16>::TPF)) void rowfft_kernel(const T* __restrict__ image, const T* __restrict__ mean,
+                                                                        int n0, const cpx<T>* __restrict__ twtab,
+                                                                        unsigned blockmask, cpx<T>* __restrict__ Yhat) {
+  using F = WgFFT<T, LG, 16>;
+  constexpr int TPF = F::TPF, L = F::L;
+  extern __shared__ __attribute__((aligned(16))) char smem[];
+  cpx<T>* lds = reinterpret_cast<cpx<T>*>(smem);
+  const int tid = threadIdx.x;
+  const size_t base = ((size_t)blockIdx.y * n0 + blockIdx.x) * L;
+  const T m = mean ? mean[blockIdx.y] : T(0);
+  cpx<T> x[16];
+#pragma unroll
+  for (int i = 0; i < 16; ++i) x[i] = {image[base + tid + TPF * i] - m, T(0)};
+  typename F::Twiddles tw;
+  F::load_twiddles(tw, twtab, tid);
+  F::forward(x, lds, tid, tw);
+#pragma unroll
+  for (int i = 0; i < 16; ++i)
+    if ((blockmask >> i) & 1) Yhat[base + i * TPF + tid] = x[i];
+}
+
+template <class T, int LG>
+static hipError_t run_rowfft(int n0, const void* image, const void* mean, const void* tw1, const PassAYspec& ys, hipStream_t s,
+                             int nimg) {
+  using F = WgFFT<T, LG, 16>;
+  auto kern = rowfft_kernel<T, LG>;
+  static unsigned lds_set = 0;
+  constexpr int lds = (int)(F::LDS_ELEMS * sizeof(cpx<T>));
+  hipError_t e = set_dynamic_lds_once(reinterpret_cast<const void*>(kern), lds, lds_set);
+  if (e != hipSuccess) return e;
+  GPA_PROF("rowfft_kernel", s);
+  kern<<<dim3(n0, nimg), F::TPF, lds, s>>>((const T*)image, (const T*)mean, n0, (const cpx<T>*)tw1, ys.blockmask, (cpx<T>*)ys.Yhat);
+  return hipGetLastError();
+}
+
+hipError_t launch_passA_yspec(int dtype, const Axis& a0, const Axis& a1, const void* image, const void* mean,
+                              const SweepTables& tb, const void* Hx, const void* tw0, const void* tw1, void* Tbuf, int B,
+                              const PassAYspec& ys, hipStream_t s, int nimg) {
+  if (a1.padded || !yspec_lg_ok(a1.lg) || a1.n != a1.L) return hipErrorInvalidValue;
+  hipError_t e;
+  if (a1.lg == 11) e = dtype == 0 ? run_rowfft<float, 11>(a0.n, image, mean, tw1, ys, s, nimg) : run_rowfft<double, 11>(a0.n, image, mean, tw1, ys, s, nimg);
+  else e = dtype == 0 ? run_rowfft<float, 12>(a0.n, image, mean, tw1, ys, s, nimg) : run_rowfft<double, 12>(a0.n, image, mean, tw1, ys, s, nimg);
+  if (e != hipSuccess) return e;
+  e = dispatch_passA<PA_YSPEC>(dtype, a0, a1.n, nullptr, nullptr, tb, Hx, tw0, Tbuf, B, s, nimg, &ys);
+  if (e != hipSuccess) return e;
+  return dispatch_passA<PA_STRIPS>(dtype, a0, a1.n, image, mean, tb, Hx, tw0, Tbuf, B, s, nimg, &ys);
 }
 
 hipError_t launch_passB(int dtype, const Axis& a1, int n0, const void* Tbuf, const void* Hy,
diff --git a/pygpa_amd/csrc/gpa_yspec.h b/pygpa_amd/csrc/gpa_yspec.h
--- /dev/null
+++ b/pygpa_amd/csrc/gpa_yspec.h
@@ -0,0 +1,27 @@
+#pragma once
+#include "gpa_fft.h"
+
+namespace gpa {
+
+GPA_HD bool yspec_lg_ok(int lg) { return lg == 11 || lg == 12; }
+
+struct YspecSrc { int tid, reg; };
+
+GPA_HD YspecSrc yspec_source(int lg, int s, int tid, int reg) {
+  const int odd = lg == 11 ? (s & 1) : 0;
+  YspecSrc r;
+  r.tid = odd ? (tid ^ 8) : tid;
+  r.reg = (reg + s - odd + ((odd && (tid & 8)) ? 2 : 0)) & 15;
+  return r;
+}
+
+GPA_HD unsigned yspec_blockmask(int lg, int s, int nbl) {
+  unsigned m = 0;
+  for (int i = 0; i < nbl; ++i) {
+    m |= 1u << yspec_source(lg, s, 0, i).reg;
+    m |= 1u << yspec_source(lg, s, 8, i).reg;
+  }
+  return m;
+}
+
+}
```

Result: faster. 3361 Mpixels/s, median of 6 (+4.6%).
